# JelleAalbers/blueice

Hardware: AMD Instinct MI355X
Metric: likelihood evals/sec (and GB/s vs HBM peak), 4-src 5^3-anchor 100^3-bin model (higher is better)
Workload: dtype f64; 1 GPU; C2: 4 sources, 3 shape params (5^3 anchors), 100^3 bins; step = one batched call (one kernel launch) of 8 independent dense evaluations, each against its own dataset, in grid cells that share no anchor (no byte re-used), tensor replicated per GPU; device=gfx950:sramecc+:xnack-, gather=none (one process), backend_requested=rccl, backend_explicit=False, gather_kind=none (one process)

## Files before the change

blueice_amd/_capi.py:

```python
import ctypes as C
import os

import numpy as np

from .exceptions import DeviceError

_HERE = os.path.dirname(os.path.abspath(__file__))
LIB_PATH = os.environ.get('BLUEICE_AMD_LIB') or os.path.join(_HERE, 'lib', 'libblueice_hip.so')

ST_OUT_OF_BOUNDS, ST_UNPHYSICAL, ST_BB_ROOT1, ST_BB_NEG, ST_BAD_DATASET, ST_INTERNAL = 1, 2, 4, 8, 16, 32
ERR_INVALID, ERR_HIP, ERR_STATE, ERR_NOMEM = -1, -2, -3, -4

_p = C.c_void_p
_i32, _i64, _f64 = C.c_int32, C.c_int64, C.c_double
_pd = C.POINTER(C.c_double)

SIGNATURES = {
    'bi_create': (C.c_int, [C.c_int, C.POINTER(_p)]),
    'bi_destroy': (None, [_p]),
    'bi_last_error': (C.c_char_p, [_p]),
    'bi_version': (C.c_char_p, []),
    'bi_device_info': (C.c_int, [_p, C.c_char_p, C.c_char_p, C.c_int, C.POINTER(C.c_int), C.POINTER(_i64)]),
    'bi_upload_model': (C.c_int, [_p, C.c_int, _p, _p, C.c_int, _i64, _p, _p, _p, C.c_int]),
    'bi_model_begin': (C.c_int, [_p, C.c_int, _p, _p, C.c_int, _i64, C.c_int]),
# ... 4 lines not shown
    'bi_set_allow_negative': (C.c_int, [_p, _p]),
    'bi_upload_counts': (C.c_int, [_p, _i64, _p]),
    'bi_set_analysis_space': (C.c_int, [_p, C.c_int, _p, _p]),
    'bi_upload_events': (C.c_int, [_p, _i64, _p]),
    'bi_histogram_events': (C.c_int, [_p, C.c_int, _p, _p, _i64, _p, _p]),
    'bi_score_events': (C.c_int, [_p, _p, C.c_int, C.c_int, _p, _p, _i64, _p, C.c_double]),
    'bi_set_unbinned': (C.c_int, [_p, _f64]),
    'bi_simulate_events': (C.c_int, [_p, _p, _p, _p, C.c_int, C.c_int, _p, _p, C.c_uint64, C.c_double, _p]),
    'bi_score_event_sets': (C.c_int, [_p, _p, C.c_int, C.c_int, _p, _p, _i64, _p, _p, C.c_double]),
    'bi_simulate_event_toys': (C.c_int, [_p, _p, _p, _p, C.c_int, C.c_int, _p, _p, _i64, C.c_uint64, C.c_double, _p]),
    'bi_set_event_sets': (C.c_int, [_p, _i64, _p]),
    'bi_event_set_offsets': (C.c_int, [_p, _p]),
    'bi_event_set_counts': (C.c_int, [_p, _p]),
    'bi_event_set_count': (_i64, [_p]),
    'bi_download_event_set': (C.c_int, [_p, _i64, _p]),
    'bi_download_events': (C.c_int, [_p, _p, _p]),
    'bi_simulated_event_count': (_i64, [_p]),
    'bi_generate_toys': (C.c_int, [_p, _p, _p, _i64, C.c_uint64]),
    'bi_generate_toys_points': (C.c_int, [_p, _i64, _p, _p, _p, C.c_uint64, _p]),
    'bi_download_counts': (C.c_int, [_p, _i64, _p]),
    'bi_eval': (C.c_int, [_p, _i64, _p, _p, _p, _p, _p]),
    'bi_eval_grad': (C.c_int, [_p, _i64, _p, _p, _p, _p, _p, _p]),
    'bi_eval_hess': (C.c_int, [_p, _i64, _p, _p, _p, _p, _p, _p, _p]),
    'bi_eval_gof': (C.c_int, [_p, _i64, _p, _p, _p, _p, _p, _p]),
    'bi_expected_counts': (C.c_int, [_p, _i64, _p, _p, C.c_int, _p]),
    'bi_set_coarse_binning': (C.c_int, [_p, C.c_int, _p, _p, _p, C.POINTER(_i64)]),
    'bi_expected_coarse': (C.c_int, [_p, _i64, _p, _p, C.c_int, _p, _p]),
    'bi_expected_coarse_jacobian': (C.c_int, [_p, _i64, _p, _p, _p, _p, _p]),
    'bi_coarse_counts': (C.c_int, [_p, _i64, _p, _p]),
    'bi_set_real_counts': (C.c_int, [_p, _i64, _p]),
    'bi_set_asimov_counts': (C.c_int, [_p, _i64, _p, _p]),
    'bi_real_count_sets': (_i64, [_p]),
    'bi_download_real_counts': (C.c_int, [_p, _i64, _p]),
    'bi_eval_real': (C.c_int, [_p, _i64, _p, _p, _p, _p, _p, _p]),
    'bi_eval_fisher': (C.c_int, [_p, _i64, _p, _p, _p, _p, _p, _p]),
    'bi_fisher_variant': (C.c_int, [C.c_int, C.POINTER(C.c_int), C.POINTER(C.c_int)]),
    'bi_minimize_batched': (C.c_int, [_p, _p, _i64, C.c_int, _p, _p, _p, _p, _p, C.c_double, C.c_int, _p, _p, _p, _p]),
    'bi_fit_batched': (C.c_int, [_p, _i64, C.c_int, _p, _p, _p, _p, _p, _p, _p, _p, _p, _p, _p, C.c_double, C.c_int, _p, _p, _p, _p]),
    'bi_fit_batched_gauss': (C.c_int, [_p, _i64, C.c_int, _p, _p, _p, _p, _p, _p, _p, _p, _p, _p, _p, C.c_double, C.c_int, _p, _p, _p,
                                       _p, _p, _p, _p]),
    'bi_fit_batched_real': (C.c_int, [_p, _i64, C.c_int, _p, _p, _p, _p, _p, _p, _p, _p, _p, _p, _p, C.c_double, C.c_int, _p, _p, _p,
                                      _p, _p, _p, _p]),
    'bi_factored_begin': (C.c_int, [_p, C.c_int, _p, _p, C.c_int, _i64, _p, _p]),
    'bi_factored_set_anchor': (C.c_int, [_p, C.c_int, _i64, _p, C.c_double]),
    'bi_factored_end': (C.c_int, [_p]),
    'bi_factored_set_counts': (C.c_int, [_p, _i64, _p]),
    'bi_eval_factored': (C.c_int, [_p, _i64, _p, _p, _p, _p, _p, _p]),
    'bi_eval_sourcewise_hess': (C.c_int, [_p, _i64, _p, _p, _p, _p, _p, _p, _p]),
    'bi_eval_sourcewise_fisher': (C.c_int, [_p, _i64, _p, _p, _p, _p, _p, _p]),
    'bi_fit_batched_factored': (C.c_int, [_p, _i64, C.c_int, _p, _p, _p, _p, _p, _p, _p, _p, _p, _p, _p, C.c_double, C.c_int, _p, _p, _p,
                                          _p, _p, _p, _p]),
    'bi_sample_stretch': (C.c_int, [_p, _i64, C.c_int, C.c_int, _p, _p, _p, _p, _p, _p, _p, _p, _p, _i64, C.c_double, C.c_uint64, _i64,
                                    _p, _p, _p, _p]),
    'bi_sample_stretch_gauss': (C.c_int, [_p, _i64, C.c_int, C.c_int, _p, _p, _p, _p, _p, _p, _p, _p, _p, _i64, C.c_double, C.c_uint64, _i64,
                                          _p, _p, _p, _p, _p, _p, _p]),
    'bi_grid_reduce': (C.c_int, [_p, _i64, _p, C.c_int, C.c_int, _p, _p, _p, _p, _p, _p, _p, _p, _p, _i64, _p, _p, _p, _p]),
    'bi_eval_datasets': (C.c_int, [_p, _p, _p, _i64, _i64, _p, _p]),
    'bi_eval_datasets_points': (C.c_int, [_p, _i64, _p, _p, _i64, _i64, _p, _p]),
    'bi_eval_datasets_points_device': (C.c_int, [_p, _i64, _p, _p, _i64, _i64, _p, _p]),
    'bi_interpolate': (C.c_int, [_p, C.c_int, _p, _p]),
    'bi_eval_full': (C.c_int, [_p, _p, _p, _i64, _p, _p, _p, _p]),
    'bi_plan_points': (C.c_int, [_p, _i64, _p, _p, _p, C.POINTER(_p)]),
    'bi_run_plan': (C.c_int, [_p, _p, _p]),
    'bi_plan_points_share': (C.c_int, [_p, _i64, _p, _p, _p, C.c_int, C.c_int, C.POINTER(_p)]),
    'bi_plan_points_resident': (C.c_int, [_p, _i64, _p, _p, _p, C.c_int, C.c_int, C.POINTER(_p)]),
    'bi_plan_share_info': (C.c_int, [_p, C.POINTER(_i64), C.POINTER(_i64), C.POINTER(_i64)]),
    'bi_plan_unsort': (C.c_int, [_p, _p, _p, _i64, _p]),
    'bi_plan_read': (C.c_int, [_p, _p, _p, _p]),
    'bi_plan_status': (C.c_int, [_p, _p, C.POINTER(_i32)]),
    'bi_plan_bytes': (_i64, [_p]),
    'bi_plan_launches': (_i64, [_p]),
    'bi_plan_destroy': (None, [_p, _p]),
    'bi_sync': (C.c_int, [_p]),
    'bi_stream': (_p, [_p]),
    'bi_eval_begin': (C.c_int, [_p, _p, _p, _i64]),
    'bi_eval_end': (C.c_int, [_p, _p, _p]),
    'bi_eval_datasets_device': (C.c_int, [_p, _p, _p, _i64, _i64, _p, _p]),
    'bi_counts_to_dense': (C.c_int, [_p]),
    'bi_device_alloc': (C.c_int, [_p, _i64, C.POINTER(_p)]),
    'bi_device_free': (C.c_int, [_p, _p]),
    'bi_memcpy_to_host': (C.c_int, [_p, _p, _p, _i64]),
    'bi_memcpy_to_device': (C.c_int, [_p, _p, _p, _i64]),
    'bi_selftest_log': (C.c_int, [_p, _i64, _p, _p]),
    'bi_selftest_sort': (C.c_int, [_p, C.c_int, _i64, _p, _p, C.c_int, C.c_int, _p, _p]),
    'bi_selftest_scan': (C.c_int, [_p, C.c_int, _i64, _p, _i64, _p]),
    'bi_selftest_grid_reduce': (C.c_int, [_p, _i64, _i64, _i64, _p, _p, _p, _p, _p]),
    'bi_measure_read_bandwidth': (C.c_int, [_p, C.c_int, C.c_int, C.c_int, _p]),
    'bi_measure_stream_bandwidth': (C.c_int, [_p, C.c_int, C.c_int, C.c_int, C.c_int, C.c_int, _p]),
    'bi_measure_copy_bandwidth': (C.c_int, [_p, _i64, C.c_int, _p]),
    'bi_profile_enable': (C.c_int, [_p, C.c_int]),
    'bi_profile_read': (C.c_int, [_p, C.POINTER(_i64), C.POINTER(_f64)]),
    'bi_set_param': (C.c_int, [_p, C.c_char_p, _i64]),
    'bi_get_param': (_i64, [_p, C.c_char_p]),
    'bi_list_params': (C.c_int, [C.c_char_p, C.c_int]),
}

OBJECTIVE_FN = C.CFUNCTYPE(C.c_int, _p, _i64, C.c_int, _pd, C.POINTER(_i64), _pd, _pd)

_lib = None


def load():
    global _lib
    if _lib is not None:
        return _lib
    if not os.path.exists(LIB_PATH):
        raise DeviceError("%s is missing: build it first (python -m blueice_amd.build). "
                          "blueice_amd has no CPU fallback." % LIB_PATH)
    try:
        lib = C.CDLL(LIB_PATH)
    except OSError as e:
        raise DeviceError("cannot load %s: %s" % (LIB_PATH, e))
    for name, (res, args) in SIGNATURES.items():
        try:
            fn = getattr(lib, name)
        except AttributeError:
            raise DeviceError("%s does not export %s (stale build?)" % (LIB_PATH, name))
        fn.restype = res
        fn.argtypes = args
    version = (lib.bi_version() or b'').decode()
    if not version.startswith('blueice_hip') or '(gfx950)' not in version or 'not the product' in version:
        raise DeviceError("%s is not a gfx950 build of libblueice_hip (bi_version: %r)" % (LIB_PATH, version))
    _lib = lib
    return lib


def ptr(a):
    if a is None:
        return None
    return a.ctypes.data_as(C.c_void_p)


def as_f64(a, shape=None):
    a = np.ascontiguousarray(a, dtype=np.float64)
    if shape is not None and tuple(a.shape) != tuple(shape):
        raise ValueError("expected array of shape %s, got %s" % (tuple(shape), a.shape))
    return a
```

blueice_amd/csrc/bi_context.h:

```cpp
#pragma once

struct bi_ctx;

constexpr int kThreads = 256;
constexpr int kBinsPerThread = 2;
constexpr int kTile = kThreads * kBinsPerThread;
constexpr int kMaxDim = 8;
constexpr int kMaxG = 16;
constexpr int kFacMaxDim = 32;
constexpr int kFacMaxSources = 8;
constexpr int kFacMaxOwn = 3;

inline thread_local std::string g_create_error;

struct DevBuf {
    void* p = nullptr;
    size_t bytes = 0;
    struct bi_ctx* owner = nullptr;
    bool view = false;
};

struct bi_plan {
    int64_t P = 0;
    struct Class {
// ... 2 lines not shown
        int nbx = 0;
        DevBuf rowoff, coef, aux, item_cnt, item_tiles, perm, slot_lg, partial, pflags;
        DevBuf rowoff_full;
    };
    std::vector<Class> classes;
    DevBuf bad_idx;
    int64_t n_bad = 0;
    DevBuf nan_idx;
    int64_t n_nan = 0;
    DevBuf out, status;
    std::vector<int32_t> h_status;
    int64_t epoch = 0;
    DevBuf slab;
    bool host_results = false;
    bool use_scan = false;
    int64_t n_groups = 0;
    int scan_cb = 4;
    DevBuf grp_first, grp_items;
    std::vector<int64_t> h_grp_first;
    std::vector<int32_t> h_grp_items;
    int bb_kgt = 0;
    bool valid = false;
    int valid_nslots = 0;
    DevBuf bad;
    bool shared = false;
    int share_world = 1;
    int64_t share_lo = 0, share_hi = 0, n_valid = 0;
    DevBuf sorted_idx;
    DevBuf keep_z, keep_rs;
    int64_t max_group_items = 0;
    int max_item_tiles = 0;
    bool device_planned = false;
    bool no_reuse = false;
    bool sparse = false;
    bool narrow = false;
    bool sorted = false;
    bool by_count = false;
    int64_t bytes = 0;
    int64_t launches = 0;
};

struct bi_ctx {
    int device = 0;
    hipStream_t stream = nullptr;
    hipDeviceProp_t prop{};
    std::string err;

    bool model_ready = false, model_open = false;
    int d = 0, S = 0;
    int64_t B = 0, Bp = 0, A = 0;
    std::vector<int> n_anchor;
    std::vector<std::vector<double>> grid;
    std::vector<int64_t> astride;
    std::vector<int> eff_axes;
    int bb_source = -1;
    std::vector<int32_t> allow_neg;
    DevBuf ps, nm, nm_tot;
    std::vector<double> h_mus;
    std::vector<double> h_nm_tot;
    std::vector<char> anchor_set;

    int space_k = 0;
    std::vector<int32_t> space_n_edges;
    DevBuf space_edges;

    bool unbinned = false;
    double outlier = 0.0;
    bool ps_finite = true;
    bool data_ready = false;
    bool dense_counts = false;
    int64_t T = 0;
    int64_t n_sets = 1;
    std::vector<int64_t> set_first, set_n;
    int64_t n_set_launches = 0;
    DevBuf counts, lgsum;
    std::vector<double> h_lgsum;
    DevBuf cnt8, cnt8_bad;
    std::vector<uint32_t> h_cnt8_bad;
    bool cnt8_valid = false;
    int cnt8_all = -1;
    int64_t narrow_counts = 1;
    int64_t last_streamed_bytes = 0;
    int64_t n_narrow_launches = 0;
    int64_t last_morph_nbx = 0, last_morph_items = 0, last_morph_fused = 0;

    DevBuf real_counts;
    int64_t real_T = 0;

    struct Factored {
        bool ready = false, open = false;
        int d = 0, S = 0;
        int64_t B = 0, Bp = 0;
        std::vector<std::vector<double>> grid;
        std::vector<int> n_own;
        std::vector<int> own;
        std::vector<int64_t> row_first;
        std::vector<int64_t> own_stride;
        std::vector<double> h_mus;
        std::vector<char> row_set;
        DevBuf ps;
        int64_t T = 0;
        DevBuf counts;
        std::vector<double> h_lgsum;
        int n_rows_point = 0;
        int max_own = 0;
    } fac;

    struct Coarse {
        bool set = false;
        int64_t C = 0, CR = 0, Cx = 0;
        int64_t L = 0, NR = 0;
        int64_t x_lo = 0, Lx = 0;
        int64_t max_rows = 0;
        int64_t max_width = 0;
        DevBuf row_off, row_list;
        DevBuf xb;
        DevBuf row_map, x_map;
    } coarse;

    std::vector<double> h_rowsum;
    std::vector<double> h_rowmin;
    bool ps_nonneg = false;

    bool csr_ready = false, compact_ready = false;
    bool compact_sorted = false;
    DevBuf nz_idx, nz_n, nz_off, ps_c, cnt_c;
    DevBuf tm_entries, tm_off;
    int64_t nz_tile_epoch = -1;
    bool tm_ok = false;
    DevBuf tmm_entries, tmm_off;
    int64_t tmm_epoch = -1;
    bool tmm_ok = false;
    int tmm_width = 4;
    int64_t toy_points_pp = 0;
    int64_t toy_points_lanes = 0;
    int64_t toy_points_overlap = 0;
    hipStream_t stream2 = nullptr;
    hipEvent_t tp_ev[7] = {nullptr, nullptr, nullptr, nullptr, nullptr, nullptr, nullptr};
    int64_t n_toy_points_passes = 0;
    int64_t dot_tiled = 1;
    int64_t score_sorted = 1;
    DevBuf ev_perm;
    bool ev_sorted = false;
    int64_t toy_fast_call = 7;
    DevBuf toy_blocks_done;
    bool toy_blocks_done_zeroed = false;
    unsigned long long toy_seq = 0;
    int64_t n_toy_polled = 0;
    int64_t dot_entry16 = 1;
    int tm_width = 4;
    int64_t dot_blocks_per_cu = 0;
    int64_t dot_lanes = 0;
    int64_t toy_events = 1;
    int64_t last_toy_method = 0;
    std::vector<int64_t> h_nz_off;
    std::vector<int64_t> h_c_off, h_cnt_off;
    std::vector<int64_t> h_c_np;
    std::vector<double> h_Tz;

    DevBuf slot_dev, slot_partial, slot_pflags, slot_counter;
    DevBuf mail, mail_flags;
    void* pack_host = nullptr;
    void* bounce_host = nullptr;
    size_t pack_host_bytes = 0;
    DevBuf pack_dev;
    void* plan_host = nullptr;
// ... 242 lines not shown
```

blueice_amd/csrc/bi_dev_common.h:

```cpp
#pragma once


constexpr long long kMailTicksPerMs = 100000;

struct LaunchArgs {
    const double* ps;
    const double* nm;
    const double* counts;
    const int64_t* rowoff;
    const double* coef;
    const double* aux;
    const int64_t* item_cnt;
    const int32_t* item_tiles;
    double* partial;
    unsigned* pflags;
    int64_t B, Bp;
    double outlier;
    int n0, n1, n2;
    int n_tiles;
    int chunks;
    int n_keep;
    double* fin_mail;
    unsigned* fin_flags;
    const int64_t* fin_perm;
    const double* fin_slot_lg;
    double* fin_out;
    int32_t* fin_status;
    int nan_S;
    long long mail_timeout = 2000 * kMailTicksPerMs;
    int skip_post = -1, late_post = -1;
    const uint8_t* cnt8 = nullptr;
};

constexpr int kMaxSingleStreams = 128;

struct SingleDesc {
    int64_t rowoff[kMaxSingleStreams];
    double coef[kMaxSingleStreams];
    double aux[2];
    double slot_lg;
    unsigned* flags;
    double* out;
    int32_t* status;
    unsigned long long* done;
    unsigned long long seq;
};

typedef double bi_double4 __attribute__((ext_vector_type(4)));

struct ScanArgs {
    const double* ps;
    const double* counts;
    const int64_t* rowoff;
    const double* coef;
    const int64_t* item_cnt;
    const int32_t* item_tiles;
    const int64_t* grp_first;
    const int32_t* grp_items;
    double* partial;
    int NS;
    int nslots;
    int n_groups;
    int xcd_mode;
    int share_slow;
};

struct ValidArgs {
    const double* ps;
    const int64_t* rowoff;
    const double* coef;
    const int64_t* grp_first;
    const int32_t* grp_items;
    unsigned* bad;
    int NS;
    int nslots;
    int n_strips;
};

struct BbScanArgs {
    const double* ps;
    const double* nm;
    const double* counts;
    const int64_t* rowoff;
    const double* coef;
    const double* aux;
    const int64_t* item_cnt;
    const int64_t* grp_first;
    const int32_t* grp_items;
    double* partial;
    unsigned* pflags;
    int64_t B;
    int n0, nc;
    int n_tiles;
};

struct GradMfmaArgs {
    const double* ps;
    const double* counts;
    const int64_t* rowoff;
    const double* coef;
    const int64_t* item_cnt;
    const int32_t* item_tiles;
    const int64_t* grp_first;
    const int32_t* grp_items;
    double* part_ll;
    double* part_g;
    int NS, n_slices;
};

struct HessArgs {
    const double* ps;
    const double* counts;
    const int64_t* rowoff;
    const double* coef;
    const int64_t* item_cnt;
// ... 228 lines not shown
    return v;
}

#define BI_SWAP_MUL(SWAP, a, b, out)                                                                               \
    do {                                                                                                           \
        const unsigned long long ua = __double_as_longlong(a), ub = __double_as_longlong(b);                       \
        const auto lo = SWAP((unsigned)ua, (unsigned)ub, false, false);                                            \
        const auto hi = SWAP((unsigned)(ua >> 32), (unsigned)(ub >> 32), false, false);                            \
        out = __longlong_as_double(((unsigned long long)hi[0] << 32) | lo[0]) *                                    \
              __longlong_as_double(((unsigned long long)hi[1] << 32) | lo[1]);                                     \
    } while (0)

__device__ __forceinline__ double lane_value(double v, int src_lane) {
    const unsigned long long u = __double_as_longlong(v);
    return __longlong_as_double(((unsigned long long)(unsigned)__builtin_amdgcn_readlane((int)(u >> 32), src_lane) << 32) |
                                (unsigned)__builtin_amdgcn_readlane((int)u, src_lane));
}

__device__ __forceinline__ unsigned wave_or(unsigned v) {
#pragma unroll
    for (int off = 32; off > 0; off >>= 1) v |= __shfl_down(v, off, 64);
    return v;
}

__shared__ double4 s_log_table[128];

__device__ __forceinline__ void log_table_load() {
    if (threadIdx.x < 128) s_log_table[threadIdx.x] = kLogTable[threadIdx.x];
    __syncthreads();
}

__device__ __forceinline__ bool pos_normal(double x) { return __builtin_amdgcn_class(x, 0x100); }
constexpr double kProdFloor = 0x1p-127;

__device__ __forceinline__ double log_core(double x, int k_adjust) {
    const unsigned long long ix = __double_as_longlong(x);
    const int hi = (int)(ix >> 32);
    const int t = hi - 0x3FE60000;
    const int k0 = t >> 20;
    const int k = k0 + k_adjust;
    int zhi;
    asm("v_mad_i32_i24 %0, %1, %2, %3" : "=v"(zhi) : "v"(k0), "s"(-(1 << 20)), "v"(hi));
    const double z = __longlong_as_double(((unsigned long long)(unsigned)zhi << 32) | (ix & 0xFFFFFFFFull));
    const double4 e = s_log_table[(t >> 13) & 127];
    const double kd = (double)k;
    const double r = fma(z, e.x, -1.0);
    const double w = fma(kd, kLn2Hi, e.y);
    const double tail = fma(kd, kLn2Lo, e.z);
    double p = fma(r, -1.0 / 8.0, e.w);
    p = fma(r, p, -1.0 / 6.0);
    p = fma(r, p, 1.0 / 5.0);
    p = fma(r, p, -1.0 / 4.0);
    p = fma(r, p, 1.0 / 3.0);
    p = fma(r, p, -0.5);
    const double q = fma(r * r, p, tail);
    const double h = w + r;
    const double err = (w - h) + r;
    return h + (err + q);
}

__device__ __forceinline__ double bin_log_fast(double x) { return log_core(x, 0); }

__device__ __forceinline__ double bin_log(double x) {
    const bool tiny = x < 2.2250738585072014e-308;
    double y = log_core(tiny ? x * 18014398509481984.0 : x, tiny ? -54 : 0);
    if (x == 0.0) y = -__builtin_inf();
    if (!(x >= 0.0)) y = __builtin_nan("");
    if (x == __builtin_inf()) y = x;
    return y;
}

template <bool NT>
__device__ __forceinline__ double2 stream_load(const double* p) {
    if constexpr (NT) {
        double2 v;
        v.x = __builtin_nontemporal_load(p);
        v.y = __builtin_nontemporal_load(p + 1);
        return v;
    } else {
        return *reinterpret_cast<const double2*>(p);
    }
}

__device__ __forceinline__ double poisson_term(double n, double mu) {
    double t;
    if (n > 0.0) {
        t = n * bin_log(mu) - mu;
    } else {
        t = -mu;
    }
    if (!(mu >= 0.0) || n != n) t = __builtin_nan("");
    else if (n < 0.0 || n != floor(n)) t = -__builtin_inf();
    return t;
}

__device__ __forceinline__ bool needs_checked_term(double n, double mu) { return n > 0.0 && !pos_normal(mu); }

__device__ __forceinline__ double poisson_term_fast(double n, double mu) {
    const double lg = bin_log_fast(mu);
    double t = (n > 0.0) ? n * lg - mu : -mu;
    if (!(mu >= 0.0) || n != n) t = __builtin_nan("");
    else if (n < 0.0 || n != floor(n)) t = -__builtin_inf();
    return t;
}

__device__ __forceinline__ double poisson_term_nolog(double n, double mu) {
    double t = -mu;
    if (!(mu >= 0.0) || n != n) t = __builtin_nan("");
    else if (n < 0.0 || n != floor(n)) t = -__builtin_inf();
    return t;
}

__device__ __forceinline__ void bb_roots(double a, double p, double U, double d, double& r1, double& r2) {
#pragma clang fp contract(off)
    double U2 = U * U, p2 = p * p, a2 = a * a, d2 = d * d;
    double disc = U2 * p2 + 2 * U2 * p + U2 + 2 * U * a * p2 + 2 * U * a * p - 2 * U * d * p2 - 2 * U * d * p +
                  a2 * p2 + 2 * a * d * p2 + d2 * p2;
    double lead = -U * p - U + a * p + d * p;
    double den = 2 * p * (p + 1);
    double sq = sqrt(disc);
    r1 = (lead - sq) / den;
    r2 = (lead + sq) / den;
}

constexpr unsigned long long kMailEmpty = 0x7FF4B10E1CE00001ull;

__device__ __forceinline__ void mail_post(double* slot, double v) {
    if (v != v) v = __builtin_nan("");
    __hip_atomic_store(slot, v, __ATOMIC_RELAXED, __HIP_MEMORY_SCOPE_SYSTEM);
}

__device__ __forceinline__ double mail_take(double* slot, long long deadline, bool* late) {
    unsigned long long bits;
    for (;;) {
        bits = __hip_atomic_load(reinterpret_cast<unsigned long long*>(slot), __ATOMIC_RELAXED, __HIP_MEMORY_SCOPE_SYSTEM);
        if (bits != kMailEmpty) break;
        if ((long long)wall_clock64() > deadline) { *late = true; return __builtin_nan(""); }
        __builtin_amdgcn_s_sleep(4);
    }
    __hip_atomic_store(reinterpret_cast<unsigned long long*>(slot), kMailEmpty, __ATOMIC_RELAXED, __HIP_MEMORY_SCOPE_SYSTEM);
    return __longlong_as_double(bits);
}

__device__ __forceinline__ double mail_take4(double* mail, int q0, int stride, int total, double s, long long deadline, bool* late) {
    unsigned long long bits[4];
#pragma unroll
    for (int u = 0; u < 4; ++u) {
        const int q = q0 + u * stride;
        bits[u] = q < total ? __hip_atomic_load(reinterpret_cast<unsigned long long*>(mail + q), __ATOMIC_RELAXED, __HIP_MEMORY_SCOPE_SYSTEM)
                            : 0ull;
    }
#pragma unroll
    for (int u = 0; u < 4; ++u) {
        const int q = q0 + u * stride;
        if (q >= total) break;
        if (bits[u] == kMailEmpty) {
            s += mail_take(mail + q, deadline, late);
        } else {
            __hip_atomic_store(reinterpret_cast<unsigned long long*>(mail + q), kMailEmpty, __ATOMIC_RELAXED, __HIP_MEMORY_SCOPE_SYSTEM);
            s += __longlong_as_double(bits[u]);
        }
    }
    return s;
}

__device__ __forceinline__ void flags_post(unsigned* word, unsigned f) {
// ... 35 lines not shown
```

blueice_amd/csrc/bi_events.h:

```cpp
#pragma once

namespace {


struct AxisWords {
    const char* with;
    const char* few;
    const char* values;
};
constexpr AxisWords kSpaceWords{"edges", "axis %d needs at least two edges", "bin edges"};
constexpr AxisWords kHistWords{"edges, and a counts buffer", "axis %d needs at least two edges", "bin edges"};
constexpr AxisWords kGridWords{"grid values", "axis %d needs at least two grid values", "grid values"};
constexpr AxisWords kSimWords{"bin edges", "axis %d has too few bin edges", "bin edges"};

struct AxisWalk {
    int k = 0;
    int flat = 0;
    int64_t bins = 1;
    int n[kMaxDim] = {}, off[kMaxDim] = {};
    int64_t stride[kMaxDim] = {};
    void put(int* n_out, int* off_out, int64_t* stride_out = nullptr) const {
        for (int i = 0; i < k; ++i) {
            n_out[i] = n[i];
            off_out[i] = off[i];
// ... 35 lines not shown
    return BI_OK;
}


int score_events_impl(bi_ctx* tp, bi_ctx* c, int method, int k, const int32_t* n_grid, const double* grid, int64_t N,
                      const double* coords, const double* coords_dev, double outlier_likelihood,
                      const std::vector<int64_t>* pad_cols = nullptr) {
    if (!c) return BI_ERR_INVALID;
    if (!tp || tp == c) return fail(c, BI_ERR_INVALID, "need a templates context different from the target");
    if (c->pending || tp->pending) return fail(c, BI_ERR_STATE, "a bi_eval_begin is outstanding: call bi_eval_end first");
    if (!tp->model_ready) return fail(c, BI_ERR_STATE, "the templates context holds no model");
    if (tp->device != c->device) return fail(c, BI_ERR_INVALID, "templates and target live on different devices");
    if (tp->bb_source >= 0) return fail(c, BI_ERR_INVALID, "Beeston-Barlow applies to binned likelihoods only");
    if (method != 0 && method != 1) return fail(c, BI_ERR_INVALID, "method must be 0 (piecewise) or 1 (linear)");
    AxisWalk ax;
    int rc = walk_axes(c, k, n_grid, grid, 2, method == 1, kGridWords, ax);
    if (rc) return rc;
    if (N < 0 || (N > 0 && !coords && !coords_dev)) return fail(c, BI_ERR_INVALID, "bad N / coords");
    if (ax.bins != tp->B) return fail(c, BI_ERR_INVALID, "the grid describes %lld bins, the templates have %lld", (long long)ax.bins, (long long)tp->B);
    ScoreArgs a{};
    a.k = k;
    a.method = method;
    a.clip = coords_dev ? 1 : 0;
    ax.put(a.n_grid, a.grid_off, a.stride);
    std::vector<int32_t> na(tp->n_anchor.begin(), tp->n_anchor.end());
    std::vector<double> az;
    for (int i = 0; i < tp->d; ++i) az.insert(az.end(), tp->grid[(size_t)i].begin(), tp->grid[(size_t)i].end());
    if ((rc = bi_model_begin(c, tp->d, na.data(), az.data(), tp->S, N, -1))) return rc;
    if (N > 0) {
        ScratchBuf d_ev, d_grid, d_base, d_t, d_keys, d_iota, d_tmp, d_pad;
        const bool sorted = !pad_cols && c->score_sorted && N >= 4096 && N < ((int64_t)1 << 31);
        if (pad_cols && !pad_cols->empty() && (rc = dev_upload(c, d_pad, *pad_cols))) return rc;
        size_t sort_bytes = 0;
        if (sorted) (void)prim_sort_pairs(nullptr, sort_bytes, (const int64_t*)nullptr, (int64_t*)nullptr, (const int32_t*)nullptr,
                                                    (int32_t*)nullptr, (size_t)N, 0u, 64u, c->stream);
        if ((!coords_dev && (rc = dev_alloc(c, d_ev, (size_t)N * k * sizeof(double)))) || (rc = dev_alloc(c, d_grid, (size_t)ax.flat * sizeof(double))) ||
            (rc = dev_alloc(c, d_base, (size_t)N * sizeof(int64_t))) || (method == 1 && (rc = dev_alloc(c, d_t, (size_t)N * k * sizeof(double)))) ||
            (sorted && ((rc = dev_alloc(c, d_keys, (size_t)N * sizeof(int64_t))) || (rc = dev_alloc(c, d_iota, (size_t)N * sizeof(int32_t))) ||
                        (rc = dev_alloc(c, d_tmp, std::max<size_t>(sort_bytes, 256))) || (rc = dev_alloc(c, c->ev_perm, (size_t)N * sizeof(int32_t))))))
            return rc;
        hipError_t e = coords_dev ? hipSuccess : hipMemcpyAsync(d_ev.p, coords, (size_t)N * k * sizeof(double), hipMemcpyHostToDevice, c->stream);
        if (e == hipSuccess) e = hipMemcpyAsync(d_grid.p, grid, (size_t)ax.flat * sizeof(double), hipMemcpyHostToDevice, c->stream);
        if (e == hipSuccess) e = hipStreamSynchronize(tp->stream);
        if (e == hipSuccess) {
            const int n_rows = (int)(tp->A * tp->S);
            hipLaunchKernelGGL(k_score_locate, dim3((unsigned)((N + kThreads - 1) / kThreads)), dim3(kThreads), 0, c->stream,
                               coords_dev ? coords_dev : (const double*)d_ev.p, N, a, (const double*)d_grid.p, (int64_t*)d_base.p, (double*)d_t.p);
            const int64_t* base_used = (const int64_t*)d_base.p;
            if (sorted) {
                hipLaunchKernelGGL(k_iota32, dim3((unsigned)((N + 255) / 256)), dim3(256), 0, c->stream, (int32_t*)d_iota.p, N);
                size_t tb = d_tmp.bytes;
                unsigned bits = 1;
                while (bits < 63 && ((int64_t)1 << bits) < tp->B) ++bits;
                e = prim_sort_pairs(d_tmp.p, tb, (const int64_t*)d_base.p, (int64_t*)d_keys.p, (const int32_t*)d_iota.p,
                                              (int32_t*)c->ev_perm.p, (size_t)N, 0u, bits, c->stream);
                base_used = (const int64_t*)d_keys.p;
            }
            const int per_block = kThreads * score_events_per_thread(method == 0 ? 0 : k);
            const unsigned bx = (unsigned)((N + per_block - 1) / per_block);
#define BI_ROWS(K)                                                                                                 \
    hipLaunchKernelGGL((k_score_rows<K>), dim3(bx, (unsigned)std::min(n_rows, 65535)), dim3(kThreads), 0, c->stream, \
                       base_used, (const double*)d_t.p, N, a, (const double*)tp->ps.p, tp->Bp, n_rows, (double*)c->ps.p, c->Bp,        \
                       sorted ? (const int32_t*)c->ev_perm.p : (const int32_t*)nullptr)
            if (e == hipSuccess) switch (method == 0 ? 0 : k) {
                case 0: BI_ROWS(0); break; case 1: BI_ROWS(1); break; case 2: BI_ROWS(2); break; case 3: BI_ROWS(3); break;
                case 4: BI_ROWS(4); break; case 5: BI_ROWS(5); break; case 6: BI_ROWS(6); break; case 7: BI_ROWS(7); break;
                default: BI_ROWS(8); break;
            }
#undef BI_ROWS
            if (e == hipSuccess && pad_cols && !pad_cols->empty()) {
                const int64_t n_fill = (int64_t)n_rows * (int64_t)pad_cols->size();
                hipLaunchKernelGGL(k_fill_columns, dim3((unsigned)((n_fill + 255) / 256)), dim3(256), 0, c->stream, (double*)c->ps.p, c->Bp,
                                   (int64_t)n_rows, (const int64_t*)d_pad.p, (int64_t)pad_cols->size(), 1.0);
            }
            if (e == hipSuccess) e = hipGetLastError();
        }
        if (e == hipSuccess) e = hipStreamSynchronize(c->stream);
        else (void)hipStreamSynchronize(c->stream);
        c->ev_sorted = e == hipSuccess && sorted;
        if (e != hipSuccess) return fail(c, BI_ERR_HIP, "bi_score_events: %s", hipGetErrorString(e));
    }
    c->h_mus = tp->h_mus;
    std::fill(c->anchor_set.begin(), c->anchor_set.end(), 1);
    if ((rc = bi_model_end(c))) return rc;
    c->allow_neg = tp->allow_neg;
    return bi_set_unbinned(c, outlier_likelihood);
}


struct SimSetup {
    SimArgs a{};
    PointGeom g;
    std::vector<double> r, h_edges;
    std::vector<int64_t> rowoff;
    ScratchBuf row, w, edges, rates, dens, cdf, tmp;
};

int sim_setup(bi_ctx* tp, bi_ctx* c, const double* z, const double* rate_scale, int method, int k, const int32_t* n_edges,
              const double* edges, size_t scan_items, const char* who, SimSetup& s) {
    if (!c) return BI_ERR_INVALID;
    if (!tp || tp == c) return fail(c, BI_ERR_INVALID, "need a templates context different from the target");
    if (c->pending || tp->pending) return fail(c, BI_ERR_STATE, "a bi_eval_begin is outstanding: call bi_eval_end first");
    if (!tp->model_ready) return fail(c, BI_ERR_STATE, "the templates context holds no model");
    if (tp->device != c->device) return fail(c, BI_ERR_INVALID, "templates and target live on different devices");
    if (method != 0 && method != 1) return fail(c, BI_ERR_INVALID, "method must be 0 (piecewise) or 1 (linear)");
    AxisWalk ax;
    int rc = walk_axes(c, k, n_edges, edges, method == 1 ? 3 : 2, false, kSimWords, ax);
    if (rc) return rc;
    if (tp->d > 0 && !z) return fail(c, BI_ERR_INVALID, "z is NULL");
    if (ax.bins != tp->B) return fail(c, BI_ERR_INVALID, "the edges describe %lld bins, the templates have %lld", (long long)ax.bins, (long long)tp->B);
    s.a.k = k; s.a.S = tp->S;
    ax.put(s.a.n_edges, s.a.edge_off, s.a.stride);
    HIP_TRY(c, hipSetDevice(c->device));
    PointGeom& g = s.g;
    std::vector<double>& r = s.r;
    if ((rc = rates_at(c, tp, z, rate_scale, "simulation", "event simulation", g, r))) return rc;
    const int S = tp->S;
    for (int q = 0; q < S; ++q)
        if (r[(size_t)q] >= kSimMaxRate)
            return fail(c, BI_ERR_INVALID, "event simulation draws at most 2^30 expected events per source: source %d has %g", q, r[(size_t)q]);
    const int nc = (int)g.w.size();
    const int64_t B = tp->B;
    s.rowoff.assign((size_t)S * nc, 0);
    for (int q = 0; q < S; ++q)
        for (int corner = 0; corner < nc; ++corner)
            s.rowoff[(size_t)q * nc + corner] = ((g.cell_anchor + corner_offset(tp, corner)) * S + q) * tp->Bp;
    size_t scan_bytes = 0, scan2 = 0;
    (void)prim_inclusive_scan_sum(nullptr, scan_bytes, (const double*)nullptr, (double*)nullptr, (size_t)B, c->stream);
    if (scan_items) (void)prim_exclusive_scan_sum(nullptr, scan2, (const int64_t*)nullptr, (int64_t*)nullptr, (int64_t)0, scan_items, c->stream);
    s.h_edges.assign(edges, edges + ax.flat);
    if ((rc = dev_upload(c, s.row, s.rowoff)) || (rc = dev_upload(c, s.w, g.w)) || (rc = dev_upload(c, s.edges, s.h_edges)) ||
        (rc = dev_upload(c, s.rates, r)) || (rc = dev_alloc(c, s.dens, (size_t)S * B * sizeof(double))) ||
        (rc = dev_alloc(c, s.cdf, (size_t)S * B * sizeof(double))) ||
        (rc = dev_alloc(c, s.tmp, std::max<size_t>(std::max(scan_bytes, scan2), 256)))) return rc;
    hipError_t e = hipStreamSynchronize(tp->stream);
    if (e == hipSuccess) {
        hipLaunchKernelGGL(k_morph_store, dim3((unsigned)((B + kThreads - 1) / kThreads), (unsigned)S), dim3(kThreads), 0, c->stream,
                           (const double*)tp->ps.p, (const int64_t*)s.row.p, (const double*)s.w.p, nc, B, (double*)s.dens.p);
        hipLaunchKernelGGL(k_sim_pmf, dim3((unsigned)((B + kThreads - 1) / kThreads), (unsigned)S), dim3(kThreads), 0, c->stream,
                           (const double*)s.dens.p, s.a, (const double*)s.edges.p, B, (double*)s.dens.p);
        e = hipGetLastError();
    }
    for (int q = 0; e == hipSuccess && q < S; ++q) {
        size_t tb = s.tmp.bytes;
        e = prim_inclusive_scan_sum(s.tmp.p, tb, (const double*)s.dens.p + (size_t)q * B, (double*)s.cdf.p + (size_t)q * B, (size_t)B, c->stream);
    }
    if (e != hipSuccess) return fail(c, BI_ERR_HIP, "%s: %s", who, hipGetErrorString(e));
    return BI_OK;
}

void lookup_grid(int method, int k, const int32_t* n_edges, const double* edges, std::vector<int32_t>& n_grid, std::vector<double>& grid) {
    n_grid.assign((size_t)k, 0);
    grid.clear();
    int eo = 0;
    for (int i = 0; i < k; ++i) {
        if (method == 0) {
            n_grid[(size_t)i] = n_edges[i];
            grid.insert(grid.end(), edges + eo, edges + eo + n_edges[i]);
        } else {
            n_grid[(size_t)i] = n_edges[i] - 1;
            for (int j = 0; j + 1 < n_edges[i]; ++j) grid.push_back(0.5 * (edges[eo + j] + edges[eo + j + 1]));
        }
        eo += n_edges[i];
    }
}


// ... 249 lines not shown
```

blueice_amd/csrc/bi_k_misc.h:

```cpp
#pragma once

#include "bi_philox.h"

namespace {

__global__ void k_selftest_log(const double* __restrict__ x, int64_t n, double* __restrict__ out) {
    log_table_load();
    const int64_t i = (int64_t)blockIdx.x * blockDim.x + threadIdx.x;
    if (i < n) out[i] = bin_log(x[i]);
}

template <bool NT>
__global__ __launch_bounds__(kThreads) void k_read_sum(const double* __restrict__ p, int64_t n2, double* __restrict__ sink) {
    double s = 0.0;
    const int64_t stride = (int64_t)gridDim.x * kThreads;
    int64_t i = (int64_t)blockIdx.x * kThreads + threadIdx.x;
    for (; i + 7 * stride < n2; i += 8 * stride) {
        double2 v[8];
#pragma unroll
        for (int u = 0; u < 8; ++u) v[u] = stream_load<NT>(p + 2 * (i + u * stride));
#pragma unroll
        for (int u = 0; u < 8; ++u) s += v[u].x + v[u].y;
    }
    for (; i < n2; i += stride) s += p[2 * i] + p[2 * i + 1];
// ... 83 lines not shown
    f = wave_or(f);
    if (lanes == 64) {
        if ((threadIdx.x & 63) == 0 && p >= 0) {
            out[p] = s - lg;
            if (status) status[p] |= (int32_t)f;
        }
        return;
    }
    if ((threadIdx.x & 63) == 0) { sh[threadIdx.x >> 6] = s; shf[threadIdx.x >> 6] = f; }
    __syncthreads();
    if (threadIdx.x == 0 && p >= 0) {
        double t = sh[0];
        unsigned ff = shf[0];
        for (int w = 1; w < kThreads / 64; ++w) { t += sh[w]; ff |= shf[w]; }
        out[p] = t - lg;
        if (status) status[p] |= (int32_t)ff;
    }
}

__global__ __launch_bounds__(kThreads) void k_status_or(const int32_t* __restrict__ status, int64_t n, int32_t* __restrict__ out) {
    unsigned f = 0u;
    for (int64_t i = (int64_t)blockIdx.x * kThreads + threadIdx.x; i < n; i += (int64_t)gridDim.x * kThreads) f |= (unsigned)status[i];
    f = wave_or(f);
    if ((threadIdx.x & 63) == 0 && f) atomicOr((unsigned*)out, f);
}

__global__ __launch_bounds__(kThreads) void k_status_clear(int32_t* __restrict__ status, int64_t n, int32_t mask) {
    for (int64_t i = (int64_t)blockIdx.x * kThreads + threadIdx.x; i < n; i += (int64_t)gridDim.x * kThreads)
        if (status[i] & mask) status[i] &= ~mask;
}

__global__ void k_fill_value(double* __restrict__ out, int64_t n, double v) {
    const int64_t i = (int64_t)blockIdx.x * blockDim.x + threadIdx.x;
    if (i < n) out[i] = v;
}

__global__ void k_fill_const(double* __restrict__ out, const int64_t* __restrict__ idx, int64_t n, double v) {
    const int64_t i = (int64_t)blockIdx.x * blockDim.x + threadIdx.x;
    if (i < n) out[idx[i]] = v;
}

__global__ __launch_bounds__(kThreads) void k_counts_lgamma(const double* __restrict__ counts, int64_t B, int64_t Bp,
                                                            double* __restrict__ partial, int nblk) {
    const int t = blockIdx.y;
    const double* __restrict__ c = counts + (int64_t)t * Bp;
    double s = 0.0;
    for (int64_t b = (int64_t)blockIdx.x * kThreads + threadIdx.x; b < B; b += (int64_t)nblk * kThreads) {
        const double n = c[b];
        if (n > 1.0 && n == floor(n)) s += lgamma(n + 1.0);
    }
    __shared__ double sh[kThreads / 64];
    s = wave_sum(s);
    if ((threadIdx.x & 63) == 0) sh[threadIdx.x >> 6] = s;
    __syncthreads();
    if (threadIdx.x == 0) {
        double r = sh[0];
        for (int w = 1; w < kThreads / 64; ++w) r += sh[w];
        partial[(int64_t)t * nblk + blockIdx.x] = r;
    }
}

constexpr int kNarrowPerThread = 8;
__global__ __launch_bounds__(kThreads) void k_counts_narrow(const double* __restrict__ counts, int64_t B, int64_t Bp,
                                                            uint8_t* __restrict__ narrow, unsigned* __restrict__ bad) {
    const int t = blockIdx.y;
    const int64_t b0 = ((int64_t)blockIdx.x * kThreads + threadIdx.x) * kNarrowPerThread;
    bool lossy = false;
    if (b0 < Bp) {
        const double* __restrict__ src = counts + (int64_t)t * Bp + b0;
        unsigned long long packed = 0ull;
#pragma unroll
        for (int j = 0; j < kNarrowPerThread; ++j) {
            const double v = b0 + j < B ? src[j] : 0.0;
            const bool in_range = v >= 0.0 && v <= 255.0;
            const unsigned q = in_range ? (unsigned)(int)v : 0u;
            lossy |= __double_as_longlong((double)q) != __double_as_longlong(v);
            packed |= (unsigned long long)q << (8 * j);
        }
        *reinterpret_cast<unsigned long long*>(narrow + (int64_t)t * Bp + b0) = packed;
    }
    if (__ballot(lossy) != 0ull && (threadIdx.x & 63) == 0) atomicOr(bad + t, 1u);
}

__global__ void k_rows_sum(const double* __restrict__ partial, int nblk, double* __restrict__ out, int64_t T) {
    const int64_t t = (int64_t)blockIdx.x * blockDim.x + threadIdx.x;
    if (t >= T) return;
    double s = 0.0;
    for (int b = 0; b < nblk; ++b) s += partial[t * nblk + b];
    out[t] = s;
}

__global__ __launch_bounds__(kThreads) void k_morph_store(const double* __restrict__ src,
                                                          const int64_t* __restrict__ rowoff,
                                                          const double* __restrict__ w,
                                                          int nc, int64_t B, double* __restrict__ out,
                                                          const int32_t* __restrict__ place = nullptr) {
    const int r = blockIdx.y;
    const int64_t b = (int64_t)blockIdx.x * kThreads + threadIdx.x;
    if (b >= B) return;
    double v = 0.0;
    for (int c = 0; c < nc; ++c) {
        const double term = __dmul_rn(src[rowoff[(int64_t)r * nc + c] + b], w[c]);
        v = __dadd_rn(v, term);
    }
    out[(int64_t)r * B + (place ? (int64_t)place[b] : b)] = v;
}

__global__ __launch_bounds__(kThreads) void k_row_total(const double* __restrict__ rows, int64_t B, int64_t Bp,
                                                        double* __restrict__ out) {
    const double* __restrict__ r = rows + (int64_t)blockIdx.x * Bp;
    double s = 0.0;
    for (int64_t b = threadIdx.x; b < B; b += kThreads) s += r[b];
    __shared__ double sh[kThreads / 64];
    s = wave_sum(s);
    if ((threadIdx.x & 63) == 0) sh[threadIdx.x >> 6] = s;
    __syncthreads();
    if (threadIdx.x == 0) {
        double t = sh[0];
        for (int w = 1; w < kThreads / 64; ++w) t += sh[w];
        out[blockIdx.x] = t;
    }
}

constexpr int kSumChunk = 8192;

__global__ __launch_bounds__(kThreads) void k_bb_chunk_sums(const double* __restrict__ nm, const int64_t* __restrict__ rowoff_all,
                                                            const double* __restrict__ w_all, int nc, int64_t B,
                                                            double* __restrict__ chunk_sum_all, double* __restrict__ tail_all) {
    __shared__ double a[kSumChunk / 2];
    __shared__ double r[256];
    __shared__ double leaf[64];
    const int64_t q = blockIdx.x;
    const int64_t* __restrict__ rowoff = rowoff_all + q * nc;
    const double* __restrict__ w = w_all + q * nc;
    double* __restrict__ chunk_sum = chunk_sum_all + q * (B / kSumChunk);
    double* __restrict__ tail = tail_all + q * (B % kSumChunk);
    const int64_t b0 = (int64_t)blockIdx.y * kSumChunk;
    const int n = (int)(B - b0 < (int64_t)kSumChunk ? B - b0 : (int64_t)kSumChunk);
    if (n < kSumChunk) {
        for (int i = threadIdx.x; i < n; i += kThreads) {
            double v = 0.0;
            for (int c = 0; c < nc; ++c) v = __dadd_rn(v, __dmul_rn(nm[rowoff[c] + b0 + i], w[c]));
            tail[i] = v;
        }
        return;
    }
    for (int half = 0; half < 2; ++half) {
        __syncthreads();
        for (int i = threadIdx.x; i < kSumChunk / 2; i += kThreads) {
            double v = 0.0;
            for (int c = 0; c < nc; ++c) v = __dadd_rn(v, __dmul_rn(nm[rowoff[c] + b0 + half * (kSumChunk / 2) + i], w[c]));
            a[i] = v;
        }
        __syncthreads();
        {
            const int blk = threadIdx.x >> 3, j = threadIdx.x & 7;
            double t = a[blk * 128 + j];
#pragma unroll
            for (int i = 1; i < 16; ++i) t = __dadd_rn(t, a[blk * 128 + 8 * i + j]);
            r[threadIdx.x] = t;
        }
        __syncthreads();
        if (threadIdx.x < 32) {
            const double* q = r + threadIdx.x * 8;
            leaf[half * 32 + threadIdx.x] = __dadd_rn(__dadd_rn(__dadd_rn(q[0], q[1]), __dadd_rn(q[2], q[3])),
                                                      __dadd_rn(__dadd_rn(q[4], q[5]), __dadd_rn(q[6], q[7])));
// ... 748 lines not shown
```

blueice_amd/csrc/bi_k_morph.h:

```cpp
#pragma once

#ifndef BI_CNT8_NT
#define BI_CNT8_NT 0
#endif

namespace {


template <int G, bool BB, bool NT, int MODE, bool CNT8 = false>
__device__ __forceinline__ void morph_tiles(const LaunchArgs& a, const int64_t* __restrict__ rowoff,
                                            const double* __restrict__ coef, const double* __restrict__ aux_base,
                                            const double* __restrict__ cnt, const uint8_t* __restrict__ cnt8, int n_tiles, int tile0,
                                            int tile_step, double (&sum)[G], unsigned (&flg)[G]) {
    double4 tab = {0.0, 0.0, 0.0, 0.0};
    if (threadIdx.x < 128) tab = kLogTable[threadIdx.x];
    bool tab_pending = true;
    const int chunks = (a.chunks > 1 && n_tiles >= 64 * a.chunks) ? a.chunks : 1;
    const int per_chunk = (n_tiles + chunks - 1) / chunks;
    for (int lt = tile0; lt < per_chunk * chunks; lt += tile_step) {
        const int tile = chunks > 1 ? (lt % chunks) * per_chunk + lt / chunks : lt;
        if (tile >= n_tiles) continue;
        const int64_t bin0 = (int64_t)tile * kTile + threadIdx.x * kBinsPerThread;
        double acc[G][2];
#pragma unroll
        for (int g = 0; g < G; ++g) { acc[g][0] = 0.0; acc[g][1] = 0.0; }
        double2 nv;
        if constexpr (MODE == 2 || MODE == 3) { nv.x = nv.y = 0.0; }
        else if constexpr (CNT8) {
#if BI_CNT8_NT
            const unsigned pair = __builtin_nontemporal_load(reinterpret_cast<const uint16_t*>(cnt8 + bin0));
#else
            const unsigned pair = *reinterpret_cast<const uint16_t*>(cnt8 + bin0);
#endif
            nv.x = (double)(pair & 0xffu);
            nv.y = (double)(pair >> 8);
        } else { nv = *reinterpret_cast<const double2*>(cnt + bin0); }

        int k0 = 0;
        if constexpr (NT && G == 1 && MODE != 2 && MODE != 3) {
            k0 = a.n_keep;
#pragma unroll 8
            for (int k = 0; k < k0; ++k) {
                const double2 v = stream_load<false>(a.ps + rowoff[k] + bin0);
                const double c = coef[k];
                acc[0][0] = fma(c, v.x, acc[0][0]);
                acc[0][1] = fma(c, v.y, acc[0][1]);
            }
        }
        if constexpr (MODE == 2 || MODE == 3) if (a.nan_S > 0) {
            const int S = a.nan_S, nc = a.n0 / S;
            for (int s = 0; s < S; ++s) {
                double part[G][2];
#pragma unroll
                for (int g = 0; g < G; ++g) { part[g][0] = 0.0; part[g][1] = 0.0; }
                for (int c = 0; c < nc; ++c) {
                    const int k = c * S + s;
                    const double2 v = stream_load<NT>(a.ps + rowoff[k] + bin0);
#pragma unroll
                    for (int g = 0; g < G; ++g) {
                        const double cf = coef[k * G + g];
                        part[g][0] = fma(cf, v.x, part[g][0]);
                        part[g][1] = fma(cf, v.y, part[g][1]);
                    }
                }
                if constexpr (MODE == 3) {
#pragma unroll
                    for (int j = 0; j < 2; ++j)
                        if (part[0][j] == part[0][j]) {
#pragma unroll
                            for (int g = 0; g < G; ++g) acc[g][j] += part[g][j];
                        }
                } else {
#pragma unroll
                    for (int g = 0; g < G; ++g) {
                        if (part[g][0] == part[g][0]) acc[g][0] += part[g][0];
                        if (part[g][1] == part[g][1]) acc[g][1] += part[g][1];
                    }
                }
            }
            k0 = a.n0;
        }
#pragma unroll 8
        for (int k = k0; k < a.n0; ++k) {
            const double2 v = stream_load<NT>(a.ps + rowoff[k] + bin0);
#pragma unroll
            for (int g = 0; g < G; ++g) {
                const double c = coef[k * G + g];
                acc[g][0] = fma(c, v.x, acc[g][0]);
                acc[g][1] = fma(c, v.y, acc[g][1]);
            }
        }
        if (tab_pending) {
            if (threadIdx.x < 128) s_log_table[threadIdx.x] = tab;
            __syncthreads();
            tab_pending = false;
        }

        if constexpr (MODE == 2) {
            bool checked = false;
#pragma unroll
            for (int g = 0; g < G; ++g) {
#pragma unroll
                for (int j = 0; j < 2; ++j) {
                    if (a.outlier != 0.0 && !(acc[g][j] > 0.0)) acc[g][j] = a.outlier;
                    checked |= bin0 + j < a.B && !pos_normal(acc[g][j]);
                }
            }
            const bool fast = __ballot(checked) == 0ull;
#pragma unroll
            for (int g = 0; g < G; ++g) {
#pragma unroll
                for (int j = 0; j < 2; ++j) {
                    const double lg = fast ? bin_log_fast(acc[g][j]) : bin_log(acc[g][j]);
                    if (bin0 + j < a.B) sum[g] += lg;
                }
            }
        } else if constexpr (MODE == 3) {
#pragma unroll
            for (int j = 0; j < 2; ++j) {
                double lam = acc[0][j];
                const bool clamped = a.outlier != 0.0 && !(lam > 0.0);
                if (clamped) lam = a.outlier;
                const double lg = bin_log(lam);
                if (bin0 + j < a.B) {
                    sum[0] += lg;
                    const double inv = clamped ? 0.0 : 1.0 / lam;
#pragma unroll
                    for (int g = 1; g < G; ++g) sum[g] += acc[g][j] * inv;
                }
            }
        } else if constexpr (MODE == 1) {
            sum[0] += poisson_term(nv.x, acc[0][0]) + poisson_term(nv.y, acc[0][1]);
            const double f0 = (nv.x != 0.0 ? nv.x / acc[0][0] : 0.0) - 1.0;
            const double f1 = (nv.y != 0.0 ? nv.y / acc[0][1] : 0.0) - 1.0;
#pragma unroll
            for (int g = 1; g < G; ++g) sum[g] += f0 * acc[g][0] + f1 * acc[g][1];
        } else if constexpr (!BB) {
#pragma unroll
            for (int j = 0; j < 2; ++j) {
                const double n = j ? nv.y : nv.x;
                bool checked = false;
#pragma unroll
                for (int g = 0; g < G; ++g) checked |= needs_checked_term(n, acc[g][j]);
                if (__ballot(n > 0.0) == 0ull) {
#pragma unroll
                    for (int g = 0; g < G; ++g) sum[g] += poisson_term_nolog(n, acc[g][j]);
                } else if (__ballot(checked) == 0ull) {
#pragma unroll
                    for (int g = 0; g < G; ++g) sum[g] += poisson_term_fast(n, acc[g][j]);
                } else {
#pragma unroll
                    for (int g = 0; g < G; ++g) sum[g] += poisson_term(n, acc[g][j]);
                }
            }
        } else {
            double pi[G][2], ai[G][2];
#pragma unroll
            for (int g = 0; g < G; ++g) { pi[g][0] = pi[g][1] = ai[g][0] = ai[g][1] = 0.0; }
#pragma unroll 8
            for (int k = 0; k < a.n1; ++k) {
                const double2 v = stream_load<NT>(a.ps + rowoff[a.n0 + k] + bin0);
#pragma unroll
                for (int g = 0; g < G; ++g) {
                    const double c = coef[(a.n0 + k) * G + g];
                    pi[g][0] = __dadd_rn(pi[g][0], __dmul_rn(v.x, c));
                    pi[g][1] = __dadd_rn(pi[g][1], __dmul_rn(v.y, c));
                }
            }
#pragma unroll 8
            for (int k = 0; k < a.n2; ++k) {
                const double2 v = stream_load<NT>(a.nm + rowoff[a.n0 + a.n1 + k] + bin0);
#pragma unroll
                for (int g = 0; g < G; ++g) {
                    const double c = coef[(a.n0 + a.n1 + k) * G + g];
                    ai[g][0] = __dadd_rn(ai[g][0], __dmul_rn(v.x, c));
                    ai[g][1] = __dadd_rn(ai[g][1], __dmul_rn(v.y, c));
                }
            }
            const double* __restrict__ aux = aux_base;
#pragma unroll
            for (int g = 0; g < G; ++g) {
                const double p_cal = aux[g * 2 + 0];
                const double Ntot = aux[g * 2 + 1];
#pragma unroll
                for (int j = 0; j < 2; ++j) {
                    if (bin0 + j < a.B) {
                        const double n = j ? nv.y : nv.x;
                        const double U = acc[g][j];
                        const double ab = ai[g][j];
                        const double w = pi[g][j] / ab * Ntot;
                        double r1, r2;
                        bb_roots(ab, w * p_cal, U, n, r1, r2);
                        if (!(r1 <= 0.0)) flg[g] |= BI_ST_BB_ROOT1;
                        const double A = (U == 0.0) ? (n + ab) / (1.0 + p_cal) : r2;
                        if (!(0.0 <= A)) flg[g] |= BI_ST_BB_NEG;
                        const double mu = U + (A * w) * p_cal;
                        sum[g] += poisson_term(n, mu);
                    }
                }
            }
        }
    }

}

template <int G, bool BB, bool NT, int MODE = 0, bool CNT8 = false>
__global__ __launch_bounds__(kThreads) void k_morph_reduce(LaunchArgs a) {
    const int item = blockIdx.y;
    const int NS = a.n0 + a.n1 + a.n2;
    const int64_t* __restrict__ rowoff = a.rowoff + (int64_t)item * NS;
    const double* __restrict__ coef = a.coef + (int64_t)item * NS * G;
    const int64_t cnt_off = a.item_cnt[item];
    const double* __restrict__ cnt = a.counts + cnt_off;
    const uint8_t* __restrict__ cnt8 = CNT8 ? a.cnt8 + cnt_off : nullptr;
    const int n_tiles = a.item_tiles ? a.item_tiles[item] : a.n_tiles;

    double sum[G];
    unsigned flg[G];
#pragma unroll
    for (int g = 0; g < G; ++g) { sum[g] = 0.0; flg[g] = 0u; }

    morph_tiles<G, BB, NT, MODE, CNT8>(a, rowoff, coef, a.aux + (int64_t)item * G * 2, cnt, cnt8, n_tiles, (int)blockIdx.x, (int)gridDim.x, sum, flg);

    __shared__ double s_sum[kThreads / 64][G];
    __shared__ unsigned s_flg[kThreads / 64][G];
    const int lane = threadIdx.x & 63, wave = threadIdx.x >> 6;
#pragma unroll
    for (int g = 0; g < G; ++g) {
        const double s = wave_sum(sum[g]);
        const unsigned f = BB ? wave_or(flg[g]) : 0u;
        if (lane == 0) { s_sum[wave][g] = s; s_flg[wave][g] = f; }
    }
    __syncthreads();
    const bool fuse = a.fin_mail != nullptr;
    const int nbx = gridDim.x;
    if (threadIdx.x < G) {
        const int g = threadIdx.x;
        double s = s_sum[0][g];
        unsigned f = s_flg[0][g];
#pragma unroll
        for (int w = 1; w < kThreads / 64; ++w) { s += s_sum[w][g]; f |= s_flg[w][g]; }
        const int64_t o = ((int64_t)item * nbx + blockIdx.x) * G + g;
        if (fuse) {
            if (BB) flags_post(a.fin_flags + (int64_t)item * G + g, f);
            mail_post_checked(a, a.fin_mail + o, s);
        } else {
            a.partial[o] = s;
            a.pflags[o] = f;
        }
    }
    if (!fuse || (int)blockIdx.x != nbx - 1) return;

    const long long deadline = (long long)wall_clock64() + a.mail_timeout;
    double* __restrict__ mail = a.fin_mail + (int64_t)item * nbx * G;
    bool late = false;
    if (nbx <= 64) {
        for (int g = wave; g < G; g += kThreads / 64) {
            double s = lane < nbx ? mail_take(mail + (int64_t)lane * G + g, deadline, &late) : 0.0;
            s = wave_sum(s);
            const bool any_late = __ballot(late) != 0ull;
            const int64_t p = a.fin_perm[(int64_t)item * G + g];
            if (lane == 0) {
                const unsigned f = (BB ? flags_take(a.fin_flags + (int64_t)item * G + g) : 0u) | (any_late ? (unsigned)BI_ST_INTERNAL : 0u);
                if (p >= 0) {
                    a.fin_out[p] = s - a.fin_slot_lg[(int64_t)item * G + g];
                    if (a.fin_status) a.fin_status[p] |= (int32_t)f;
                }
            }
        }
        return;
    }
    {
        const int total = nbx * G;
        double s = 0.0;
        for (int q0 = threadIdx.x; q0 < total; q0 += 4 * kThreads) s = mail_take4(mail, q0, kThreads, total, s, deadline, &late);
        __shared__ double s_part[kThreads];
        __shared__ unsigned s_late[kThreads / 64];
        const unsigned lt = __ballot(late) != 0ull ? 1u : 0u;
        if constexpr (G == 1) s = wave_sum(s);
        __syncthreads();
        s_part[threadIdx.x] = s;
        if (lane == 0) s_late[wave] = lt;
        __syncthreads();
        if (threadIdx.x < G) {
            const int g = threadIdx.x;
            double t = 0.0;
            if constexpr (G == 1) {
                t = s_part[0];
#pragma unroll
                for (int w = 1; w < kThreads / 64; ++w) t += s_part[w * 64];
            } else {
                for (int j = 0; j < kThreads / G; ++j) t += s_part[g + G * j];
            }
            unsigned any_late = 0u;
#pragma unroll
            for (int w = 0; w < kThreads / 64; ++w) any_late |= s_late[w];
            const int64_t p = a.fin_perm[(int64_t)item * G + g];
            const unsigned f = (BB ? flags_take(a.fin_flags + (int64_t)item * G + g) : 0u) | (any_late ? (unsigned)BI_ST_INTERNAL : 0u);
            if (p >= 0) {
                a.fin_out[p] = t - a.fin_slot_lg[(int64_t)item * G + g];
                if (a.fin_status) a.fin_status[p] |= (int32_t)f;
            }
        }
    }
}

template <bool BB, bool NT, int MODE, bool FUSE, bool CNT8 = false>
__global__ __launch_bounds__(kThreads) void k_morph_single(LaunchArgs a, SingleDesc d) {
    double sum[1] = {0.0};
    unsigned flg[1] = {0u};
    morph_tiles<1, BB, NT, MODE, CNT8>(a, d.rowoff, d.coef, d.aux, a.counts, a.cnt8, a.n_tiles, (int)blockIdx.x, (int)gridDim.x, sum, flg);

    __shared__ double s_sum[kThreads / 64];
    __shared__ unsigned s_flg[kThreads / 64];
    const int lane = threadIdx.x & 63, wave = threadIdx.x >> 6;
    {
        const double s = wave_sum(sum[0]);
        const unsigned f = BB ? wave_or(flg[0]) : 0u;
        if (lane == 0) { s_sum[wave] = s; s_flg[wave] = f; }
    }
    __syncthreads();
    if (threadIdx.x == 0) {
        double s = s_sum[0];
        unsigned f = s_flg[0];
#pragma unroll
        for (int w = 1; w < kThreads / 64; ++w) { s += s_sum[w]; f |= s_flg[w]; }
        if constexpr (FUSE) {
            if (BB) flags_post(d.flags, f);
            mail_post_checked(a, a.partial + blockIdx.x, s);
        } else {
            a.partial[blockIdx.x] = s;
            a.pflags[blockIdx.x] = f;
        }
    }
    if constexpr (!FUSE) return;
    if (blockIdx.x != gridDim.x - 1) return;
    const long long deadline = (long long)wall_clock64() + a.mail_timeout;
    bool late = false;
    double s = 0.0;
    for (int b = threadIdx.x; b < (int)gridDim.x; b += 4 * kThreads) s = mail_take4(a.partial, b, kThreads, (int)gridDim.x, s, deadline, &late);
    s = wave_sum(s);
    const unsigned lt = __ballot(late) != 0ull ? 1u : 0u;
    __syncthreads();
    if (lane == 0) { s_sum[wave] = s; s_flg[wave] = lt; }
    __syncthreads();
    if (threadIdx.x == 0) {
        double t = s_sum[0];
        unsigned any_late = s_flg[0];
#pragma unroll
        for (int w = 1; w < kThreads / 64; ++w) { t += s_sum[w]; any_late |= s_flg[w]; }
        const unsigned ff = (BB ? flags_take(d.flags) : 0u) | (any_late ? (unsigned)BI_ST_INTERNAL : 0u);
        *d.out = t - d.slot_lg;
        *d.status = (int32_t)ff;
        __hip_atomic_store(d.done, d.seq, __ATOMIC_RELEASE, __HIP_MEMORY_SCOPE_SYSTEM);
    }
}

}
```

blueice_amd/csrc/bi_launch.h:

```cpp
#pragma once

namespace {

constexpr int64_t kMailSlots = (int64_t)1 << 20;
constexpr int64_t kMailFlagWords = (int64_t)1 << 16;

int ensure_mail(bi_ctx* c) {
    if (c->mail.p) return BI_OK;
    void* p = nullptr;
    void* f = nullptr;
    if (hipMalloc(&p, (size_t)kMailSlots * sizeof(double)) != hipSuccess) return BI_ERR_NOMEM;
    if (hipMalloc(&f, (size_t)kMailFlagWords * sizeof(unsigned)) != hipSuccess) { (void)hipFree(p); return BI_ERR_NOMEM; }
    hipLaunchKernelGGL(k_mail_init, dim3((unsigned)((kMailSlots + 255) / 256)), dim3(256), 0, c->stream, (unsigned long long*)p, kMailSlots);
    if (hipGetLastError() != hipSuccess || hipMemsetAsync(f, 0, (size_t)kMailFlagWords * sizeof(unsigned), c->stream) != hipSuccess) {
        (void)hipFree(p);
        (void)hipFree(f);
        return BI_ERR_HIP;
    }
    c->mail.p = p; c->mail.bytes = (size_t)kMailSlots * sizeof(double); c->mail.owner = nullptr;
    c->mail_flags.p = f; c->mail_flags.bytes = (size_t)kMailFlagWords * sizeof(unsigned); c->mail_flags.owner = nullptr;
    return BI_OK;
}

void arm_mail(bi_ctx* c, LaunchArgs& a) {
    a.mail_timeout = c->mail_timeout_ms * kMailTicksPerMs;
    a.skip_post = (int)c->debug_skip_post;
    a.late_post = (int)c->debug_late_post;
    c->debug_skip_post = c->debug_late_post = -1;
}

void reset_mail(bi_ctx* c) {
    if (!c->mail.p) return;
    ++c->n_mail_resets;
    (void)hipStreamSynchronize(c->stream);
    hipLaunchKernelGGL(k_mail_init, dim3((unsigned)((kMailSlots + 255) / 256)), dim3(256), 0, c->stream, (unsigned long long*)c->mail.p, kMailSlots);
    (void)hipMemsetAsync(c->mail_flags.p, 0, (size_t)kMailFlagWords * sizeof(unsigned), c->stream);
    (void)hipStreamSynchronize(c->stream);
}

int check_ready(bi_ctx* c, bool need_data) {
    if (!c) return BI_ERR_INVALID;
    if (c->pending) return fail(c, BI_ERR_STATE, "a bi_eval_begin is outstanding on this context: call bi_eval_end first");
    if (!c->model_ready) return fail(c, BI_ERR_STATE, "no model uploaded (prepare() first)");
    if (need_data && !c->data_ready) return fail(c, BI_ERR_STATE, "no data uploaded (set_data() first)");
    return BI_OK;
}

int n_tiles_of(const bi_ctx* c) { return (int)(c->Bp / kTile); }

void build_narrow_counts(bi_ctx* c, int64_t T) {
    c->cnt8_valid = false;
    c->cnt8_all = -1;
    if (c->unbinned || T < 1 || !c->counts.p) return;
    const std::string keep = c->err;
    if (dev_alloc(c, c->cnt8, (size_t)T * c->Bp) || dev_alloc(c, c->cnt8_bad, (size_t)T * sizeof(unsigned))) {
        (void)hipGetLastError();
        c->err = keep;
        return;
    }
    if (hipMemsetAsync(c->cnt8_bad.p, 0, (size_t)T * sizeof(unsigned), c->stream) != hipSuccess) { (void)hipGetLastError(); return; }
    const unsigned nbx = (unsigned)((c->Bp + (int64_t)kThreads * kNarrowPerThread - 1) / ((int64_t)kThreads * kNarrowPerThread));
    const int64_t chunk = 32768;
    for (int64_t t0 = 0; t0 < T; t0 += chunk)
        hipLaunchKernelGGL(k_counts_narrow, dim3(nbx, (unsigned)std::min(chunk, T - t0)), dim3(kThreads), 0, c->stream,
                           (const double*)c->counts.p + t0 * c->Bp, c->B, c->Bp, (uint8_t*)c->cnt8.p + t0 * c->Bp, (unsigned*)c->cnt8_bad.p + t0);
    c->h_cnt8_bad.assign((size_t)T, 1u);
    if (hipGetLastError() != hipSuccess ||
        hipMemcpyAsync(c->h_cnt8_bad.data(), c->cnt8_bad.p, (size_t)T * sizeof(unsigned), hipMemcpyDeviceToHost, c->stream) != hipSuccess) {
        (void)hipGetLastError();
        return;
    }
    c->cnt8_valid = true;
}

bool narrow_on(const bi_ctx* c) { return c->narrow_counts && c->cnt8_valid && !c->unbinned && c->dense_counts; }
bool narrow_has(const bi_ctx* c, int64_t ds) {
    return c->cnt8_valid && ds >= 0 && ds < (int64_t)c->h_cnt8_bad.size() && c->h_cnt8_bad[(size_t)ds] == 0u;
}
bool narrow_has_all(bi_ctx* c) {
    if (!c->cnt8_valid) return false;
    if (c->cnt8_all < 0) c->cnt8_all = std::all_of(c->h_cnt8_bad.begin(), c->h_cnt8_bad.end(), [](uint32_t f) { return f == 0u; }) ? 1 : 0;
    return c->cnt8_all == 1;
}

void launch_finish(bi_ctx* c, const double* partial, const unsigned* pflags, int nbx, int G, int64_t n_slots, const int64_t* perm,
                   const double* slot_lg, double* out, int32_t* status) {
    const int lanes = nbx > 64 ? kThreads : 64;
    const int per_block = kThreads / lanes;
    hipLaunchKernelGGL(k_finish, dim3((unsigned)((n_slots + per_block - 1) / per_block)), dim3(kThreads), 0, c->stream, partial, pflags,
                       nbx, G, lanes, n_slots, perm, slot_lg, out, status);
}

}
```

blueice_amd/csrc/bi_params.h:

```cpp
#pragma once

namespace {

enum : int { kParamRead = 1, kParamWrite = 2, kParamRW = 3 };

struct ParamDef {
    const char* name;
    int access;
    int64_t (*get)(bi_ctx*);
    int (*set)(bi_ctx*, int64_t);
};

#define BI_P_GET(expr) [](bi_ctx* c) -> int64_t { return (int64_t)(expr); }
#define BI_P_SET(stmt) [](bi_ctx* c, int64_t v) -> int { stmt; return BI_OK; }
#define BI_P_RANGE(lo, hi, field, what)                                                                           \
    [](bi_ctx* c, int64_t v) -> int {                                                                             \
        if (v < (lo) || v > (hi)) return fail(c, BI_ERR_INVALID, what);                                           \
        c->field = v;                                                                                             \
        return BI_OK;                                                                                             \
    }
#define BI_P_FLAG(field) BI_P_SET(c->field = v ? 1 : 0)
#define BI_P_RO(nm, expr) {nm, kParamRead, BI_P_GET(expr), nullptr}

const ParamDef kParams[] = {
    {"sparse", kParamRW, BI_P_GET(c->sparse), BI_P_RANGE(0, 2, sparse, "sparse: 0 = off, 1 = auto, 2 = whenever exact")},
    {"max_group", kParamRW, BI_P_GET(c->max_group),
     [](bi_ctx* c, int64_t v) -> int {
         if (v < 1 || v > kMaxG || (v & (v - 1))) return fail(c, BI_ERR_INVALID, "max_group must be a power of two in [1,%d]", kMaxG);
         c->max_group = v;
         return BI_OK;
     }},
    {"bb_max_group", kParamRW, BI_P_GET(c->bb_max_group), BI_P_SET(c->bb_max_group = v >= 16 ? 16 : (v >= 8 ? 8 : (v >= 4 ? 4 : (v >= 2 ? 2 : 1))))},
    {"blocks_per_cu", kParamRW, BI_P_GET(c->blocks_per_cu), BI_P_RANGE(1, 32, blocks_per_cu, "blocks_per_cu in [1,32]")},
    {"nt_loads", kParamRW, BI_P_GET(c->nt_loads), BI_P_RANGE(0, 2, nt_loads, "nt_loads: 0 = never, 1 = always, 2 = auto")},
    {"tile_chunks", kParamRW, BI_P_GET(c->tile_chunks), BI_P_SET(c->tile_chunks = v < 1 ? 1 : v)},
    {"single_kernel", kParamRW, BI_P_GET(c->single_kernel), BI_P_FLAG(single_kernel)},
    {"fuse_max_blocks", kParamRW, BI_P_GET(c->fuse_max_blocks), BI_P_SET(c->fuse_max_blocks = v)},
    {"single_blocks_per_cu", kParamRW, BI_P_GET(c->single_blocks_per_cu),
     BI_P_RANGE(1, 32, single_blocks_per_cu, "single_blocks_per_cu in [1,32]")},
    {"fuse_finish", kParamRW, BI_P_GET(c->fuse_finish), BI_P_FLAG(fuse_finish)},
    {"keep_rows", kParamRW, BI_P_GET(c->keep_rows), BI_P_SET(c->keep_rows = v < 0 ? -1 : v)},
    {"poll_result", kParamRW, BI_P_GET(c->poll_result), BI_P_FLAG(poll_result)},
    {"xcd_affine", kParamRW, BI_P_GET(c->xcd_affine), BI_P_FLAG(xcd_affine)},
    {"device_plan_min", kParamRW, BI_P_GET(c->device_plan_min), BI_P_SET(c->device_plan_min = v)},
    {"scan_mfma", kParamRW, BI_P_GET(c->scan_mfma), BI_P_FLAG(scan_mfma)},
    {"scan_min_items", kParamRW, BI_P_GET(c->scan_min_items), BI_P_SET(c->scan_min_items = v < 1 ? 1 : v)},
    {"scan_cb", kParamRW, BI_P_GET(c->scan_cb), BI_P_SET(c->scan_cb = (v == 2 || v == 4) ? v : 0)},
    {"scan_waves_per_cu", kParamRW, BI_P_GET(c->scan_waves_per_cu), BI_P_SET(c->scan_waves_per_cu = v < 0 ? 0 : v)},
    {"host_threads", kParamRW, [](bi_ctx*) -> int64_t { return host_threads(); },
     [](bi_ctx* c, int64_t v) -> int { if (v < 0 || v > 256) return fail(c, BI_ERR_INVALID, "host_threads in [0, 256] (0 = by the process's affinity, at most 16)"); host_threads_setting().store((int)v); return BI_OK; }},
    {"toy_points_pp", kParamRW, BI_P_GET(c->toy_points_pp),
     [](bi_ctx* c, int64_t v) -> int {
         if (v != 0 && v != 1 && v != 2 && v != 4) return fail(c, BI_ERR_INVALID, "toy_points_pp: 0 = by the batch, 1 = point by point, 2 or 4 points per pass");
         c->toy_points_pp = v;
         return BI_OK;
     }},
    {"toy_points_overlap", kParamRW, BI_P_GET(c->toy_points_overlap), BI_P_FLAG(toy_points_overlap)},
    {"toy_points_lanes", kParamRW, BI_P_GET(c->toy_points_lanes),
     [](bi_ctx* c, int64_t v) -> int {
         if (v != 0 && v != 2 && v != 4 && v != 8) return fail(c, BI_ERR_INVALID, "toy_points_lanes: 0 = default, or 2 / 4 / 8");
         c->toy_points_lanes = v;
         return BI_OK;
     }},
    {"grad_mfma", kParamRW, BI_P_GET(c->grad_mfma), BI_P_FLAG(grad_mfma)},
    {"grad_mfma_min", kParamRW, BI_P_GET(c->grad_mfma_min), BI_P_RANGE(1, (int64_t)1 << 40, grad_mfma_min, "grad_mfma_min >= 1")},
    {"grad_slices", kParamRW, BI_P_GET(c->grad_slices), BI_P_RANGE(0, 4096, grad_slices, "grad_slices in [0, 4096]")},
    {"scan_xcd", kParamRW, BI_P_GET(c->scan_xcd), BI_P_RANGE(0, 2, scan_xcd, "scan_xcd: 0 launch order, 1 contiguous ranges, 2 one XCD per group")},
    {"scan_share_slow", kParamRW, BI_P_GET(c->scan_share_slow), BI_P_FLAG(scan_share_slow)},
    {"scan_chunk", kParamRW, BI_P_GET(c->scan_chunk), BI_P_FLAG(scan_chunk)},
    {"plan_tables", kParamRW, BI_P_GET(c->plan_tables), BI_P_FLAG(plan_tables)},
    {"plan_count_sort", kParamRW, BI_P_GET(c->plan_count_sort), BI_P_FLAG(plan_count_sort)},
    {"scan_bb", kParamRW, BI_P_GET(c->scan_bb), BI_P_FLAG(scan_bb)},
    {"scan_bb_min", kParamRW, BI_P_GET(c->scan_bb_min), BI_P_RANGE(1, (int64_t)1 << 40, scan_bb_min, "scan_bb_min >= 1")},
    {"scan_sparse_max_items", kParamRW, BI_P_GET(c->scan_sparse_max_items), BI_P_SET(c->scan_sparse_max_items = v < 0 ? 0 : v)},
    {"scan_split", kParamRW, BI_P_GET(c->scan_split), BI_P_FLAG(scan_split)},
    {"scan_pow", kParamRW, BI_P_GET(c->scan_pow), BI_P_SET(c->scan_pow = v ? 1 : 0; c->sorted_epoch = -1)},
    {"bb_exact", kParamRW, BI_P_GET(c->bb_exact), BI_P_RANGE(0, 2, bb_exact, "bb_exact: 0 never, 1 always, 2 auto")},
    {"toy_events", kParamRW, BI_P_GET(c->toy_events), BI_P_FLAG(toy_events)},
    {"dot_tiled", kParamRW, BI_P_GET(c->dot_tiled), BI_P_FLAG(dot_tiled)},
    {"score_sorted", kParamRW, BI_P_GET(c->score_sorted), BI_P_FLAG(score_sorted)},
    {"toy_fast_call", kParamRW, BI_P_GET(c->toy_fast_call), BI_P_RANGE(0, 7, toy_fast_call, "toy_fast_call: bits 1 | 2 | 4")},
    {"dot_entry16", kParamRW, BI_P_GET(c->dot_entry16), [](bi_ctx* c, int64_t v) -> int { c->dot_entry16 = v ? 1 : 0; c->nz_tile_epoch = -1; c->tmm_epoch = -1; return BI_OK; }},
    {"dot_blocks_per_cu", kParamRW, BI_P_GET(c->dot_blocks_per_cu), BI_P_RANGE(0, 16, dot_blocks_per_cu, "dot_blocks_per_cu in [0, 16]")},
    {"dot_lanes", kParamRW, BI_P_GET(c->dot_lanes), BI_P_SET(c->dot_lanes = (v == 16 || v == 8 || v == 4) ? v : 0)},
    {"compact_budget", kParamRW, BI_P_GET(c->compact_budget), BI_P_SET(c->compact_budget = v)},
    {"toy_offset", kParamRW, BI_P_GET(c->toy_offset), BI_P_RANGE(0, INT64_MAX, toy_offset, "toy_offset >= 0")},
    {"narrow_counts", kParamRW, BI_P_GET(c->narrow_counts), BI_P_FLAG(narrow_counts)},
    {"mail_timeout_ms", kParamRW, BI_P_GET(c->mail_timeout_ms),
     BI_P_RANGE(1, 60000, mail_timeout_ms, "mail_timeout_ms in [1, 60000]")},
    {"single_timing_reset", kParamWrite, nullptr,
     BI_P_SET(c->single_ns[0] = c->single_ns[1] = c->single_ns[2] = 0; c->single_calls = 0; (void)v)},
    {"drop_recycle_cache", kParamWrite, nullptr, BI_P_SET((void)hipSetDevice(c->device); (void)hipStreamSynchronize(c->stream); drop_recycle_cache(c); (void)v)},
    {"debug_skip_post", kParamWrite, nullptr, BI_P_SET(c->debug_skip_post = v < 0 ? -1 : v)},
    {"debug_late_post", kParamWrite, nullptr, BI_P_SET(c->debug_late_post = v < 0 ? -1 : v)},
    BI_P_RO("tile_bins", kTile),
    BI_P_RO("padded_bins", c->Bp),
    BI_P_RO("n_scan_launches", c->n_scan_launches),
    BI_P_RO("n_toy_polled", c->n_toy_polled),
    BI_P_RO("n_toy_points_passes", c->n_toy_points_passes),
    BI_P_RO("n_bb_scan_launches", c->n_bb_scan_launches),
    BI_P_RO("n_sampler_half_steps", c->n_sampler_half_steps),
    BI_P_RO("n_set_launches", c->n_set_launches),
    BI_P_RO("last_plan_refused", c->plan_refused),
    BI_P_RO("tmm_entry_bytes", c->tmm_ok ? c->tmm_width : 0),
    BI_P_RO("tm_entry_bytes", c->tm_ok ? c->tm_width : 0),
    BI_P_RO("events_sorted", c->ev_sorted ? 1 : 0),
    BI_P_RO("n_grad_mfma_launches", c->n_grad_mfma_launches),
    BI_P_RO("n_valid_launches", c->n_valid_launches),
    BI_P_RO("n_sorted_scans", c->n_sorted_scans),
    BI_P_RO("n_bb_exact", c->n_bb_exact),
    BI_P_RO("n_mail_resets", c->n_mail_resets),
    BI_P_RO("last_streamed_bytes", c->last_streamed_bytes),
    BI_P_RO("n_narrow_launches", c->n_narrow_launches),
    BI_P_RO("last_morph_nbx", c->last_morph_nbx),
    BI_P_RO("last_morph_items", c->last_morph_items),
    BI_P_RO("last_morph_fused", c->last_morph_fused),
    BI_P_RO("narrow_ready", c->cnt8_valid ? 1 : 0),
    BI_P_RO("csr_ready", (c->csr_ready && (c->sparse_at_upload != 0 || !c->dense_counts)) ? 1 : 0),
    BI_P_RO("compact_ready", (c->compact_ready && c->ps_nonneg && (c->sparse_at_upload != 0 || !c->dense_counts)) ? 1 : 0),
    BI_P_RO("split_ready", (c->compact_ready && c->dense_counts) ? 1 : 0),
    BI_P_RO("ps_nonneg", c->ps_nonneg ? 1 : 0),
    BI_P_RO("dense_counts", (c->data_ready && c->dense_counts) ? 1 : 0),
    BI_P_RO("coarse_cells", c->coarse.set ? c->coarse.C : 0),
    BI_P_RO("compact_sorted", (c->compact_ready && c->compact_sorted) ? 1 : 0),
    BI_P_RO("nnz_total", c->csr_ready ? c->h_nz_off.back() : -1),
    BI_P_RO("last_scan_nslots", c->last_scan_nslots),
    BI_P_RO("last_valid_nslots", c->last_valid_nslots),
    BI_P_RO("last_scan_resident", c->last_scan_resident),
    BI_P_RO("last_scan_groups", c->last_scan_groups),
    BI_P_RO("last_scan_max_items", c->last_scan_max_items),
    BI_P_RO("last_scan_cb", c->last_scan_cb),
    BI_P_RO("last_scan_by_count", c->last_scan_by_count),
    BI_P_RO("last_scan_prod", c->last_scan_prod),
    BI_P_RO("last_toy_method", c->last_toy_method),
    BI_P_RO("single_calls", c->single_calls),
    BI_P_RO("single_ns_host", c->single_ns[0]),
    BI_P_RO("single_ns_launch", c->single_ns[1]),
    BI_P_RO("single_ns_wait", c->single_ns[2]),
    BI_P_RO("user_allocations", (int64_t)c->user_allocs.size()),
    BI_P_RO("recycle_cache_bytes", (int64_t)c->cache_bytes),
};

#undef BI_P_GET
#undef BI_P_SET
#undef BI_P_RANGE
#undef BI_P_FLAG
#undef BI_P_RO

const ParamDef* find_param(const char* name) {
    for (const ParamDef& p : kParams)
        if (!strcmp(p.name, name)) return &p;
    return nullptr;
}

}
```

blueice_amd/csrc/bi_single.h:

```cpp
#pragma once

namespace {


int single_wait(bi_ctx* c, unsigned long long seq, double* out, int32_t* status) {
    char* res = (char*)c->slot_host;
    bool arrived = false;
    if (c->poll_result && !c->profiling) {
        const std::chrono::milliseconds limit(20);
        arrived = wait_word((const volatile unsigned long long*)(res + 16), seq, limit, limit, 1024);
    }
    if (!arrived || (seq & 255ull) == 0) HIP_TRY(c, hipStreamSynchronize(c->stream));
    if (*(const volatile unsigned long long*)(res + 16) != seq)
        return fail(c, BI_ERR_HIP, "single-point launch %llu finished without publishing its result", seq);
    *out = *(double*)res;
    if (status) *status = *(int32_t*)(res + 8);
    if (*(int32_t*)(res + 8) & BI_ST_INTERNAL) reset_mail(c);
    return BI_OK;
}

double pairwise_sum_host(const double* a, int64_t n) {
    if (n < 8) {
        double res = 0.0;
        for (int64_t i = 0; i < n; ++i) res += a[i];
// ... 140 lines not shown
    const int64_t row_stride = sparse ? c->h_c_np[(size_t)ds] : c->Bp;
    const int64_t row_base = sparse ? c->h_c_off[(size_t)ds] : 0;
    const int tiles = multi_set(c) ? (int)std::max<int64_t>(1, (c->set_n[(size_t)ds] + kTile - 1) / kTile) : (int)(row_stride / kTile);
    const int64_t slots = (int64_t)c->prop.multiProcessorCount * c->blocks_per_cu;
    const int64_t target = (int64_t)c->prop.multiProcessorCount * c->single_blocks_per_cu;
    const int64_t tiles_per_block = std::max<int64_t>(1, (tiles + target - 1) / target);
    int64_t want = (tiles + tiles_per_block - 1) / tiles_per_block;
    if (want >= 8) want = (want + 7) / 8 * 8;
    const int nbx = (int)std::min<int64_t>(std::min<int64_t>(want, tiles), slots);
    int rc;
    if (!c->slot_host) {
        HIP_TRY(c, hipHostMalloc(&c->slot_host, 4096, hipHostMallocDefault));
        c->slot_host_bytes = 4096;
    }
    const bool fuse = nbx <= c->fuse_max_blocks && nbx <= kMailSlots && !ensure_mail(c);
    if (!fuse && ((rc = dev_alloc(c, c->slot_partial, (size_t)slots * sizeof(double))) ||
                  (rc = dev_alloc(c, c->slot_pflags, (size_t)slots * sizeof(unsigned)))))
        return rc;
    SingleDesc d;
    const int64_t n_rows = c->A * S;
    int k = 0;
    double zsum = 0.0;
    for (int corner = 0; corner < nc; ++corner) {
        const int64_t a = g.cell_anchor + corner_offset(c, corner);
        for (int s = 0; s < S; ++s) {
            if (bb && s == c->bb_source) continue;
            d.rowoff[k] = row_base + (a * S + s) * row_stride;
            d.coef[k] = g.w[(size_t)corner] * rates[s];
            if (sparse) zsum += d.coef[k] * c->h_Tz[(size_t)(ds * n_rows + a * S + s)];
            ++k;
        }
    }
    d.aux[0] = d.aux[1] = 1.0;
    if (bb) {
        double Ntot = 0.0;
        for (int corner = 0; corner < nc; ++corner) {
            const int64_t a = g.cell_anchor + corner_offset(c, corner);
            d.rowoff[n0 + corner] = (a * S + c->bb_source) * c->Bp;
            d.coef[n0 + corner] = g.w[(size_t)corner];
            d.rowoff[n0 + n1 + corner] = a * c->Bp;
            d.coef[n0 + n1 + corner] = g.w[(size_t)corner];
            const double term = c->h_nm_tot[(size_t)a] * g.w[(size_t)corner];
            Ntot = Ntot + term;
        }
        if (c->bb_exact == 1 || (c->bb_exact == 2 && bb_zero_u_possible(c, g, rates))) {
            if ((rc = bb_exact_total(c, g, &Ntot))) return rc;
        }
        d.aux[0] = rates[c->bb_source] / Ntot;
        d.aux[1] = Ntot;
    }
    d.slot_lg = c->h_lgsum[(size_t)ds] + zsum;
    if (c->unbinned) {
        double rsum = 0.0;
        for (int s = 0; s < S; ++s) rsum += rates[s];
        d.slot_lg = rsum;
    }
    char* res = (char*)c->slot_host;
    *(double*)res = 0.0;
    *(int64_t*)(res + 8) = 0;
    *(unsigned long long*)(res + 16) = 0ull;
    d.flags = fuse ? (unsigned*)c->mail_flags.p : nullptr;
    d.out = (double*)res;
    d.status = (int32_t*)(res + 8);
    d.done = (unsigned long long*)(res + 16);
    d.seq = ++c->slot_seq;
    LaunchArgs a{};
    a.ps = sparse ? (const double*)c->ps_c.p : (const double*)c->ps.p;
    a.nm = (const double*)c->nm.p;
    a.counts = (sparse ? (const double*)c->cnt_c.p + c->h_cnt_off[(size_t)ds] : (const double*)c->counts.p + ds * c->Bp);
    a.partial = fuse ? (double*)c->mail.p : (double*)c->slot_partial.p;
    a.pflags = (unsigned*)c->slot_pflags.p;
    a.B = c->B; a.Bp = c->Bp; a.n0 = n0; a.n1 = n1; a.n2 = n2; a.n_tiles = tiles; a.chunks = (int)c->tile_chunks;
    if (multi_set(c)) {
        a.ps += c->set_first[(size_t)ds];
        a.B = c->set_n[(size_t)ds];
    }
    a.outlier = c->outlier;
    a.nan_S = (c->unbinned && !c->ps_finite) ? c->S : 0;
    if (fuse) arm_mail(c, a);
    if (!sparse && narrow_on(c) && narrow_has(c, ds)) {
        a.cnt8 = (const uint8_t*)c->cnt8.p + ds * c->Bp;
        ++c->n_narrow_launches;
    }
    const bool nt = !sparse && c->nt_loads != 0;
    a.n_keep = 0;
    if (nt && !bb && c->keep_rows != 0) {
        const bool same_cell = c->last_single_cell == g.cell_anchor && c->last_single_ds == ds;
        const int64_t fit = (int64_t)(0.85 * 256.0 * 1048576.0 / ((double)row_stride * sizeof(double)));
        if (same_cell) a.n_keep = (int)std::min<int64_t>(c->keep_rows > 0 ? c->keep_rows : fit, n0);
    }
    c->last_single_cell = g.cell_anchor;
    c->last_single_ds = ds;
    const dim3 grid((unsigned)nbx), block(kThreads);
    const auto t_launch = bi_clock::now();
    {
        EventScope ev(c);
        launch_morph_single(c, bb, nt, fuse, grid, a, d);
    }
    c->last_morph_nbx = nbx; c->last_morph_items = 1; c->last_morph_fused = fuse ? 1 : 0;
    if (!fuse)
        hipLaunchKernelGGL(k_finish_single, dim3(1), block, 0, c->stream, (const double*)a.partial, (const unsigned*)a.pflags,
                           nbx, d.slot_lg, d.out, d.status, d.done, d.seq);
    HIP_TRY(c, hipGetLastError());
    const auto t_wait = bi_clock::now();
    c->single_ns[0] += ns_between(t_entry, t_launch);
    c->single_ns[1] += ns_between(t_launch, t_wait);
    ++c->single_calls;
    if (!wait) {
        c->pending = 1;
        c->pending_seq = d.seq;
        return BI_OK;
    }
    rc = single_wait(c, d.seq, out, status);
    c->single_ns[2] += ns_between(t_wait, bi_clock::now());
    return rc;
}

int eval_single(bi_ctx* c, const double* z, const double* rate_scale, int64_t ds, double* out, int32_t* status, bool wait = true) {
    const auto t_entry = bi_clock::now();
    double parked_ll = 0.0;
    int32_t parked_st = 0;
    if (!wait) { out = &parked_ll; status = &parked_st; c->pending = 2; }
    struct Park {
        bi_ctx* c; const bool on; double* ll; int32_t* st;
        ~Park() { if (on && c->pending == 2) { c->pending_ll = *ll; c->pending_status = *st; } }
    } park{c, !wait, &parked_ll, &parked_st};
    const int S = c->S;
    const double ninf = -std::numeric_limits<double>::infinity();
    PointGeom g;
    double r[64];
    std::vector<double> rbig;
    double* rates = r;
    if (S > 64) { rbig.resize((size_t)S); rates = rbig.data(); }
    if (const int32_t bit = screen_point(c, z, rate_scale, ds, g, rates)) { *out = ninf; if (status) *status = bit; return BI_OK; }
    if (has_infinite_rate(rates, S) && c->bb_source < 0 && !c->unbinned && c->ps_finite && c->dense_counts)
        return inf_rate_value(c, g, rates, ds, out);

    const bool bb = c->bb_source >= 0;
    const int nc = (int)g.w.size();
    const int n0 = bb ? nc * (S - 1) : nc * S, n1 = bb ? nc : 0, n2 = bb ? nc : 0, NS = n0 + n1 + n2;
    const bool sparse = ItemRoute(c).compact;
    if (!sparse && !c->dense_counts) return fail(c, BI_ERR_STATE, "dataset counts are not resident in dense form");
    const int64_t row_stride = sparse ? c->h_c_np[(size_t)ds] : c->Bp;
    const int64_t row_base = sparse ? c->h_c_off[(size_t)ds] : 0;
    const int tiles = multi_set(c) ? (int)std::max<int64_t>(1, (c->set_n[(size_t)ds] + kTile - 1) / kTile) : (int)(row_stride / kTile);
    const int64_t slots = (int64_t)c->prop.multiProcessorCount * c->blocks_per_cu;
    const int nbx = (int)std::min<int64_t>(tiles, slots);

    if (NS <= kMaxSingleStreams && c->single_kernel) return eval_single_fused(c, g, rates, ds, sparse, out, status, wait, t_entry);

    const size_t n_words = (size_t)NS * 2 + 2 + 4 + 2;
    const size_t bytes = n_words * 8;
    int rc;
    if (c->slot_host_bytes < bytes) {
        if (c->slot_host) (void)hipHostFree(c->slot_host);
        c->slot_host = nullptr;
        HIP_TRY(c, hipHostMalloc(&c->slot_host, bytes * 2, hipHostMallocDefault));
        c->slot_host_bytes = bytes * 2;
    }
    if ((rc = dev_alloc(c, c->slot_dev, bytes)) || (rc = dev_alloc(c, c->slot_partial, (size_t)slots * sizeof(double))) ||
        (rc = dev_alloc(c, c->slot_pflags, (size_t)slots * sizeof(unsigned))))
        return rc;
    int64_t* w64 = (int64_t*)c->slot_host;
    double* wd = (double*)c->slot_host;
    int64_t* rowoff = w64;
    double* coef = wd + NS;
    double* aux = wd + 2 * NS;
    int k = 0;
    double zsum = 0.0;
    const int64_t n_rows = c->A * S;
    for (int corner = 0; corner < nc; ++corner) {
        const int64_t a = g.cell_anchor + corner_offset(c, corner);
        for (int s = 0; s < S; ++s) {
            if (bb && s == c->bb_source) continue;
            rowoff[k] = row_base + (a * S + s) * row_stride;
            coef[k] = g.w[(size_t)corner] * rates[s];
            if (sparse) zsum += coef[k] * c->h_Tz[(size_t)(ds * n_rows + a * S + s)];
            ++k;
        }
    }
    aux[0] = 1.0; aux[1] = 1.0;
    if (bb) {
        double Ntot = 0.0;
        for (int corner = 0; corner < nc; ++corner) {
            const int64_t a = g.cell_anchor + corner_offset(c, corner);
            rowoff[n0 + corner] = (a * S + c->bb_source) * c->Bp;
            coef[n0 + corner] = g.w[(size_t)corner];
            rowoff[n0 + n1 + corner] = a * c->Bp;
            coef[n0 + n1 + corner] = g.w[(size_t)corner];
            const double term = c->h_nm_tot[(size_t)a] * g.w[(size_t)corner];
            Ntot = Ntot + term;
        }
        if (c->bb_exact == 1 || (c->bb_exact == 2 && bb_zero_u_possible(c, g, rates))) {
            if ((rc = bb_exact_total(c, g, &Ntot))) return rc;
        }
        aux[0] = rates[c->bb_source] / Ntot;
        aux[1] = Ntot;
    }
    const size_t o = (size_t)2 * NS + 2;
    w64[o + 0] = sparse ? c->h_cnt_off[(size_t)ds] : ds * c->Bp;
    ((int32_t*)(w64 + o + 1))[0] = tiles;
    ((int32_t*)(w64 + o + 1))[1] = 0;
    w64[o + 2] = 0;
    wd[o + 3] = c->h_lgsum[(size_t)ds] + zsum;
    if (c->unbinned) {
        double rsum = 0.0;
        for (int s = 0; s < S; ++s) rsum += rates[s];
        wd[o + 3] = rsum;
    }
    char* res = (char*)c->slot_host + bytes;
    *(double*)res = 0.0;
    *(int64_t*)(res + 8) = 0;

    char* dev = (char*)c->slot_dev.p;
    HIP_TRY(c, hipMemcpyAsync(dev, c->slot_host, bytes, hipMemcpyHostToDevice, c->stream));
    LaunchArgs a{};
    a.ps = sparse ? (const double*)c->ps_c.p : (const double*)c->ps.p;
    a.nm = (const double*)c->nm.p;
    a.counts = sparse ? (const double*)c->cnt_c.p : (const double*)c->counts.p;
    a.rowoff = (const int64_t*)dev;
    a.coef = (const double*)(dev + (size_t)NS * 8);
    a.aux = (const double*)(dev + (size_t)NS * 16);
    a.item_cnt = (const int64_t*)(dev + (o + 0) * 8);
    a.item_tiles = (const int32_t*)(dev + (o + 1) * 8);
    a.partial = (double*)c->slot_partial.p;
    a.pflags = (unsigned*)c->slot_pflags.p;
    a.B = c->B; a.Bp = c->Bp; a.n0 = n0; a.n1 = n1; a.n2 = n2; a.n_tiles = tiles; a.chunks = (int)c->tile_chunks;
    if (multi_set(c)) {
        a.ps += c->set_first[(size_t)ds];
        a.B = c->set_n[(size_t)ds];
    }
    a.outlier = c->outlier;
    a.nan_S = (c->unbinned && !c->ps_finite) ? c->S : 0;
    if (!sparse && narrow_on(c) && narrow_has(c, ds)) {
        a.cnt8 = (const uint8_t*)c->cnt8.p;
        ++c->n_narrow_launches;
    }
    launch_morph_g(c, 1, a, dim3((unsigned)nbx, 1), bb, !sparse && c->nt_loads != 0);
    c->last_morph_nbx = nbx; c->last_morph_items = 1; c->last_morph_fused = 0;
    launch_finish(c, a.partial, a.pflags, nbx, 1, 1, (const int64_t*)(dev + (o + 2) * 8), (const double*)(dev + (o + 3) * 8),
                  (double*)res, (int32_t*)(res + 8));
    HIP_TRY(c, hipGetLastError());
    HIP_TRY(c, hipStreamSynchronize(c->stream));
    *out = *(double*)res;
    if (status) *status = *(int32_t*)(res + 8);
    return BI_OK;
}

}
```

blueice_amd/csrc/blueice_hip.hip:

```cpp

#include "bi_common.h"
#include "bi_prim.h"
#include "bi_k_misc.h"
#include "bi_geometry.h"
#include "bi_launch.h"
#include "bi_items.h"
#include "bi_sparse.h"
#include "bi_single.h"
#include "bi_planning.h"
#include "bi_planning_device.h"
#include "bi_grad_mfma.h"
#include "bi_grad.h"
#include "bi_params.h"
#include "bi_events.h"
#include "bi_toys.h"

namespace {

int finish_counts(bi_ctx* c, int64_t T) {
    int rc;
    const int nblk = (int)std::min<int64_t>(256, (c->B + kThreads - 1) / kThreads);
    if ((rc = dev_alloc(c, c->lgsum, (size_t)T * sizeof(double)))) return rc;
    const int64_t chunk = 32768;
    if ((rc = dev_alloc(c, c->scratch, (size_t)std::min(T, chunk) * nblk * sizeof(double)))) return rc;
    for (int64_t t0 = 0; t0 < T; t0 += chunk) {
        const int64_t n = std::min(chunk, T - t0);
        hipLaunchKernelGGL(k_counts_lgamma, dim3(nblk, (unsigned)n), dim3(kThreads), 0, c->stream,
                           (const double*)c->counts.p + t0 * c->Bp, c->B, c->Bp, (double*)c->scratch.p, nblk);
        hipLaunchKernelGGL(k_rows_sum, dim3((unsigned)((n + 255) / 256)), dim3(256), 0, c->stream,
                           (const double*)c->scratch.p, nblk, (double*)c->lgsum.p + t0, n);
    }
    HIP_TRY(c, hipGetLastError());
    build_narrow_counts(c, T);
    c->h_lgsum.assign((size_t)T, 0.0);
    HIP_TRY(c, hipMemcpyAsync(c->h_lgsum.data(), c->lgsum.p, (size_t)T * sizeof(double), hipMemcpyDeviceToHost, c->stream));
    HIP_TRY(c, hipStreamSynchronize(c->stream));
    c->T = T;
    c->dense_counts = true;
    if ((rc = build_sparse_forms(c))) return rc;
    c->data_ready = true;
    return BI_OK;
}

}

extern "C" {

const char* bi_version(void) { return BI_VERSION; }

const char* bi_last_error(const bi_ctx* ctx) { return ctx ? ctx->err.c_str() : g_create_error.c_str(); }

int bi_create(int device, bi_ctx** out) {
    if (!out) return fail(nullptr, BI_ERR_INVALID, "out is NULL");
    *out = nullptr;
    int n = 0;
    hipError_t e = hipGetDeviceCount(&n);
    if (e != hipSuccess || n == 0)
        return fail(nullptr, BI_ERR_HIP, "no HIP device available (%s); this library has no CPU fallback",
                    e == hipSuccess ? "device count is 0" : hipGetErrorString(e));
    if (device < 0 || device >= n) return fail(nullptr, BI_ERR_INVALID, "device %d out of range [0,%d)", device, n);
    bi_ctx* c = new bi_ctx();
    c->device = device;
    if ((e = hipSetDevice(device)) != hipSuccess || (e = hipGetDeviceProperties(&c->prop, device)) != hipSuccess ||
        (e = hipStreamCreateWithFlags(&c->stream, hipStreamNonBlocking)) != hipSuccess) {
        fail(nullptr, BI_ERR_HIP, "device init failed: %s", hipGetErrorString(e));
        delete c;
        return BI_ERR_HIP;
    }
    *out = c;
    return BI_OK;
}

void bi_destroy(bi_ctx* c) {
    if (!c) return;
    (void)hipSetDevice(c->device);
    (void)hipStreamSynchronize(c->stream);
    dev_free(c->ps); dev_free(c->nm); dev_free(c->nm_tot); dev_free(c->counts); dev_free(c->lgsum); dev_free(c->cnt8); dev_free(c->cnt8_bad);
    dev_free(c->scratch); dev_free(c->scratch2); dev_free(c->logmu); dev_free(c->toy_blocks_done); dev_free(c->ev_perm);
    dev_free(c->slot_dev); dev_free(c->slot_partial); dev_free(c->slot_pflags); dev_free(c->slot_counter); dev_free(c->space_edges);
    dev_free(c->mail); dev_free(c->mail_flags);
    dev_free(c->ps_sorted); dev_free(c->cnt_sorted);
    dev_free(c->sim_coords); dev_free(c->sim_source);
    dev_free(c->real_counts);
    dev_free(c->fac.ps); dev_free(c->fac.counts);
    release_coarse(c);
    if (c->slot_host) (void)hipHostFree(c->slot_host);
    if (c->pack_host) (void)hipHostFree(c->pack_host);
    if (c->bounce_host) (void)hipHostFree(c->bounce_host);
    if (c->plan_host) (void)hipHostFree(c->plan_host);
    dev_free(c->pack_dev);
    dev_free(c->nz_idx); dev_free(c->nz_n); dev_free(c->nz_off); dev_free(c->ps_c); dev_free(c->cnt_c); dev_free(c->tm_entries); dev_free(c->tm_off); dev_free(c->tmm_entries); dev_free(c->tmm_off);
    dev_free(c->pt_grid); dev_free(c->pt_mus); dev_free(c->pt_coff); dev_free(c->pt_allow); dev_free(c->pt_c_off);
    dev_free(c->pt_cnt_off); dev_free(c->pt_c_np); dev_free(c->pt_Tz); dev_free(c->pt_rowsum); dev_free(c->pt_rowmin); dev_free(c->pt_nm_tot);
    for (void* q : c->user_allocs) (void)hipFree(q);
    c->user_allocs.clear();
    for (auto& q : c->cache) (void)hipFree(q.p);
    c->cache.clear();
    for (auto& ev : c->ev_pool) { (void)hipEventDestroy(ev.first); (void)hipEventDestroy(ev.second); }
    for (hipEvent_t ev : c->tp_ev)
        if (ev) (void)hipEventDestroy(ev);
    if (c->stream2) (void)hipStreamDestroy(c->stream2);
    (void)hipStreamDestroy(c->stream);
    delete c;
}

int bi_device_info(bi_ctx* c, char* name, char* arch, int len, int* n_cu, int64_t* hbm_bytes) {
    if (!c) return BI_ERR_INVALID;
    if (name && len > 0) { strncpy(name, c->prop.name, len - 1); name[len - 1] = 0; }
    if (arch && len > 0) { strncpy(arch, c->prop.gcnArchName, len - 1); arch[len - 1] = 0; }
    if (n_cu) *n_cu = c->prop.multiProcessorCount;
    if (hbm_bytes) *hbm_bytes = (int64_t)c->prop.totalGlobalMem;
    return BI_OK;
}

void* bi_stream(bi_ctx* c) { return c ? (void*)c->stream : nullptr; }

int bi_sync(bi_ctx* c) {
    if (!c) return BI_ERR_INVALID;
    HIP_TRY(c, hipStreamSynchronize(c->stream));
    return BI_OK;
}

int bi_set_param(bi_ctx* c, const char* name, int64_t v) {
    if (!c || !name) return BI_ERR_INVALID;
    const ParamDef* p = find_param(name);
    if (!p) return fail(c, BI_ERR_INVALID, "unknown parameter %s", name);
    if (!p->set) return fail(c, BI_ERR_INVALID, "parameter %s is read-only", name);
    return p->set(c, v);
}

int64_t bi_get_param(bi_ctx* c, const char* name) {
    if (!c || !name) return INT64_MIN;
    const ParamDef* p = find_param(name);
    if (!p || !p->get) {
        fail(c, BI_ERR_INVALID, p ? "parameter %s is write-only" : "unknown parameter %s", name);
        return INT64_MIN;
    }
    return p->get(c);
}

int bi_list_params(char* buf, int len) {
    std::string all;
    for (const ParamDef& p : kParams) {
        all += p.name;
        all += p.access == kParamRW ? " rw\n" : (p.access == kParamRead ? " r\n" : " w\n");
    }
    if (buf && len > 0) {
        const size_t n = std::min<size_t>(all.size(), (size_t)len - 1);
        memcpy(buf, all.data(), n);
        buf[n] = 0;
    }
    return (int)all.size() + 1;
}


int bi_model_begin(bi_ctx* c, int d, const int32_t* n_anchor, const double* anchor_z, int S, int64_t B,
                   int bb_source) {
    if (!c) return BI_ERR_INVALID;
    HIP_TRY(c, hipSetDevice(c->device));
    if (d < 0 || d > kMaxDim) return fail(c, BI_ERR_INVALID, "d=%d outside [0,%d]", d, kMaxDim);
    if (S < 1 || B < 0) return fail(c, BI_ERR_INVALID, "need S >= 1 and B >= 0 (got S=%d B=%lld)", S, (long long)B);
    if (bb_source < -1 || bb_source >= S) return fail(c, BI_ERR_INVALID, "bb_source %d outside [-1,%d)", bb_source, S);
    if (d > 0 && (!n_anchor || !anchor_z)) return fail(c, BI_ERR_INVALID, "anchor arrays are NULL");
    c->model_ready = false;
    c->data_ready = false;
    c->cnt8_valid = false;
    dev_free(c->real_counts);
    c->real_T = 0;
    release_coarse(c);
    ++c->epoch;
    c->d = d; c->S = S; c->B = B; c->bb_source = bb_source;
    c->Bp = std::max<int64_t>(kTile, (B + kTile - 1) / kTile * kTile);
    c->unbinned = false;
    c->ev_sorted = false;
    c->n_sets = 1;
    c->set_first.clear();
    c->set_n.clear();
    c->n_anchor.assign(d, 0);
    c->grid.assign(d, {});
    c->A = 1;
    const double* zp = anchor_z;
    for (int i = 0; i < d; ++i) {
        if (n_anchor[i] < 1) return fail(c, BI_ERR_INVALID, "axis %d has %d anchors", i, n_anchor[i]);
        c->n_anchor[i] = n_anchor[i];
        c->grid[i].assign(zp, zp + n_anchor[i]);
        for (int j = 1; j < n_anchor[i]; ++j)
            if (!(c->grid[i][j] > c->grid[i][j - 1]))
                return fail(c, BI_ERR_INVALID, "anchor z values of axis %d are not strictly ascending", i);
        zp += n_anchor[i];
        c->A *= n_anchor[i];
    }
    c->astride.assign(d, 1);
    for (int i = d - 2; i >= 0; --i) c->astride[i] = c->astride[i + 1] * c->n_anchor[i + 1];
    c->eff_axes.clear();
    for (int i = 0; i < d; ++i)
        if (c->n_anchor[i] >= 2) c->eff_axes.push_back(i);
    c->allow_neg.assign(S, 0);
    c->h_mus.assign((size_t)c->A * S, 0.0);
    c->h_nm_tot.assign((size_t)c->A, 0.0);
    c->anchor_set.assign((size_t)c->A, 0);
    const size_t ps_bytes = ((size_t)c->A * S * c->Bp + kTile) * sizeof(double);
    int rc = dev_alloc(c, c->ps, ps_bytes);
    if (rc) return rc;
    HIP_TRY(c, hipMemsetAsync(c->ps.p, 0, ps_bytes, c->stream));
    if (bb_source >= 0) {
        const size_t nm_bytes = (size_t)c->A * c->Bp * sizeof(double);
        if ((rc = dev_alloc(c, c->nm, nm_bytes))) return rc;
        HIP_TRY(c, hipMemsetAsync(c->nm.p, 0, nm_bytes, c->stream));
        if ((rc = dev_alloc(c, c->nm_tot, (size_t)c->A * sizeof(double)))) return rc;
    }
    c->model_open = true;
    return BI_OK;
}

int bi_model_set_anchor(bi_ctx* c, int64_t ai, const double* ps, const double* mus, const double* nm_row) {
    if (!c || !c->model_open) return fail(c, BI_ERR_STATE, "bi_model_begin first");
    if (ai < 0 || ai >= c->A) return fail(c, BI_ERR_INVALID, "anchor index %lld outside [0,%lld)", (long long)ai, (long long)c->A);
    if (!ps || !mus) return fail(c, BI_ERR_INVALID, "ps / mus are NULL");
    if (c->bb_source >= 0 && !nm_row) return fail(c, BI_ERR_INVALID, "Beeston-Barlow model needs the n_model row");
    HIP_TRY(c, hipSetDevice(c->device));
    double* dst = (double*)c->ps.p + (size_t)ai * c->S * c->Bp;
    if (c->B > 0) HIP_TRY(c, hipMemcpy2DAsync(dst, c->Bp * sizeof(double), ps, c->B * sizeof(double), c->B * sizeof(double), c->S,
                                hipMemcpyHostToDevice, c->stream));
    for (int s = 0; s < c->S; ++s) c->h_mus[(size_t)ai * c->S + s] = mus[s];
    if (c->bb_source >= 0 && c->B > 0) {
        double* nd = (double*)c->nm.p + (size_t)ai * c->Bp;
        HIP_TRY(c, hipMemcpyAsync(nd, nm_row, c->B * sizeof(double), hipMemcpyHostToDevice, c->stream));
    }
    HIP_TRY(c, hipStreamSynchronize(c->stream));
    c->anchor_set[(size_t)ai] = 1;
    return BI_OK;
}

int bi_model_end(bi_ctx* c) {
    if (!c || !c->model_open) return fail(c, BI_ERR_STATE, "bi_model_begin first");
    for (int64_t a = 0; a < c->A; ++a)
        if (!c->anchor_set[(size_t)a]) return fail(c, BI_ERR_STATE, "anchor %lld was never set", (long long)a);
    HIP_TRY(c, hipSetDevice(c->device));
    if (c->bb_source >= 0) {
        hipLaunchKernelGGL(k_row_total, dim3((unsigned)c->A), dim3(kThreads), 0, c->stream, (const double*)c->nm.p, c->B,
                           c->Bp, (double*)c->nm_tot.p);
        HIP_TRY(c, hipGetLastError());
        HIP_TRY(c, hipMemcpyAsync(c->h_nm_tot.data(), c->nm_tot.p, (size_t)c->A * sizeof(double), hipMemcpyDeviceToHost,
                                  c->stream));
    }
    {
        const int64_t rows = c->A * c->S;
        int rc = dev_alloc(c, c->scratch, (size_t)rows * 3 * sizeof(double));
        if (rc) return rc;
        hipLaunchKernelGGL(k_row_stats, dim3((unsigned)rows), dim3(kThreads), 0, c->stream, (const double*)c->ps.p, c->B,
                           c->Bp, (double*)c->scratch.p);
        HIP_TRY(c, hipGetLastError());
        std::vector<double> st((size_t)rows * 3);
        HIP_TRY(c, hipMemcpyAsync(st.data(), c->scratch.p, st.size() * sizeof(double), hipMemcpyDeviceToHost, c->stream));
        HIP_TRY(c, hipStreamSynchronize(c->stream));
        c->h_rowsum.assign((size_t)rows, 0.0);
        c->h_rowmin.assign((size_t)rows, 0.0);
        c->ps_nonneg = true;
        c->ps_finite = true;
        for (int64_t r = 0; r < rows; ++r) {
            c->h_rowsum[(size_t)r] = st[(size_t)r * 3];
            c->h_rowmin[(size_t)r] = st[(size_t)r * 3 + 1];
            if (!(st[(size_t)r * 3 + 1] >= 0.0) || st[(size_t)r * 3 + 2] != 0.0) c->ps_nonneg = false;
            if (st[(size_t)r * 3 + 2] != 0.0) c->ps_finite = false;
        }
    }
    HIP_TRY(c, hipStreamSynchronize(c->stream));
    c->model_open = false;
    c->model_ready = true;
    return BI_OK;
}

int bi_upload_model(bi_ctx* c, int d, const int32_t* n_anchor, const double* anchor_z, int S, int64_t B,
                    const double* ps, const double* mus, const double* n_model, int bb_source) {
    if (!c) return BI_ERR_INVALID;
    if (!ps || !mus) return fail(c, BI_ERR_INVALID, "ps / mus are NULL");
    if (bb_source >= 0 && !n_model) return fail(c, BI_ERR_INVALID, "bb_source given but n_model is NULL");
    int rc = bi_model_begin(c, d, n_anchor, anchor_z, S, B, bb_source);
    if (rc) return rc;
    if (B > 0) HIP_TRY(c, hipMemcpy2DAsync(c->ps.p, c->Bp * sizeof(double), ps, B * sizeof(double), B * sizeof(double),
                                (size_t)c->A * S, hipMemcpyHostToDevice, c->stream));
    std::copy(mus, mus + (size_t)c->A * S, c->h_mus.begin());
    if (bb_source >= 0) {
        if (B > 0) HIP_TRY(c, hipMemcpy2DAsync(c->nm.p, c->Bp * sizeof(double), n_model + (size_t)bb_source * B,
                                    (size_t)S * B * sizeof(double), B * sizeof(double), (size_t)c->A,
                                    hipMemcpyHostToDevice, c->stream));
    }
    HIP_TRY(c, hipStreamSynchronize(c->stream));
    std::fill(c->anchor_set.begin(), c->anchor_set.end(), 1);
    return bi_model_end(c);
}

int bi_set_allow_negative(bi_ctx* c, const int32_t* allow) {
    int rc = check_ready(c, false);
    if (rc) return rc;
    if (!allow) return fail(c, BI_ERR_INVALID, "allow is NULL");
    c->allow_neg.assign(allow, allow + c->S);
    return BI_OK;
}

int bi_set_bb_totals(bi_ctx* c, const double* totals) {
    int rc = check_ready(c, false);
    if (rc) return rc;
    if (c->bb_source < 0) return fail(c, BI_ERR_INVALID, "the model has no Beeston-Barlow source");
    if (!totals) return fail(c, BI_ERR_INVALID, "totals is NULL");
    c->h_nm_tot.assign(totals, totals + c->A);
    ++c->epoch;
    return BI_OK;
}

int bi_get_bb_totals(bi_ctx* c, double* totals) {
    int rc = check_ready(c, false);
    if (rc) return rc;
    if (c->bb_source < 0 || !totals) return fail(c, BI_ERR_INVALID, "no Beeston-Barlow source / totals is NULL");
    std::copy(c->h_nm_tot.begin(), c->h_nm_tot.end(), totals);
    return BI_OK;
}


int bi_upload_counts(bi_ctx* c, int64_t T, const double* counts) {
    int rc = check_ready(c, false);
    if (rc) return rc;
    if (T < 1 || !counts) return fail(c, BI_ERR_INVALID, "need T >= 1 datasets and a counts pointer");
    if (c->unbinned) return fail(c, BI_ERR_STATE, "the context holds an unbinned likelihood: it has no binned counts");
    if (c->B < 1) return fail(c, BI_ERR_INVALID, "a binned likelihood needs at least one bin");
    HIP_TRY(c, hipSetDevice(c->device));
    c->data_ready = false;
    ++c->epoch;
    const size_t bytes = (size_t)T * c->Bp * sizeof(double);
    if ((rc = dev_alloc(c, c->counts, bytes))) return rc;
    HIP_TRY(c, hipMemsetAsync(c->counts.p, 0, bytes, c->stream));
    HIP_TRY(c, hipMemcpy2DAsync(c->counts.p, c->Bp * sizeof(double), counts, c->B * sizeof(double),
                                c->B * sizeof(double), (size_t)T, hipMemcpyHostToDevice, c->stream));
    return finish_counts(c, T);
}



int bi_set_analysis_space(bi_ctx* c, int k, const int32_t* n_edges, const double* edges) {
    int rc = check_ready(c, false);
    if (rc) return rc;
    AxisWalk ax;
    if ((rc = walk_axes(c, k, n_edges, edges, 2, false, kSpaceWords, ax))) return rc;
    if (ax.bins != c->B) return fail(c, BI_ERR_INVALID, "analysis space has %lld bins, the model %lld", (long long)ax.bins, (long long)c->B);
    HIP_TRY(c, hipSetDevice(c->device));
    c->space_k = k;
    c->space_n_edges.assign(n_edges, n_edges + k);
    const std::vector<double> flat(edges, edges + ax.flat);
    if ((rc = dev_upload(c, c->space_edges, flat))) return rc;
    HIP_TRY(c, hipStreamSynchronize(c->stream));
// ... 102 lines not shown
    if (P < 0 || P > (int64_t)1 << 30) return fail(c, BI_ERR_INVALID, "P outside [0, 2^30]");
    if (share_world < 1 || share_rank < 0 || share_rank >= share_world)
        return fail(c, BI_ERR_INVALID, "share %d outside [0,%d)", share_rank, share_world);
    if (c->d > 0 && P > 0 && !z_dev) return fail(c, BI_ERR_INVALID, "z_dev is NULL");
    HIP_TRY(c, hipSetDevice(c->device));
    if (P == 0) return plan_points(c, 0, nullptr, nullptr, nullptr, out);
    const void* ptrs[3] = {c->d > 0 ? (const void*)z_dev : nullptr, rate_scale_dev, dataset_dev};
    const char* names[3] = {"z_dev", "rate_scale_dev", "dataset_dev"};
    for (int i = 0; i < 3 && check_pointers; ++i) {
        if (!ptrs[i]) continue;
        hipPointerAttribute_t at;
        const hipError_t e = hipPointerGetAttributes(&at, ptrs[i]);
        if (e != hipSuccess || (at.type != hipMemoryTypeDevice && at.type != hipMemoryTypeManaged) || at.device != c->device) {
            (void)hipGetLastError();
            return fail(c, BI_ERR_INVALID, "%s is not device memory of GPU %d", names[i], c->device);
        }
    }
    const bool sparse = ItemRoute(c).compact;
    if (!sparse && !c->dense_counts)
        return fail(c, BI_ERR_STATE, "the datasets exist only as non-empty-bin lists (device-generated toys): point "
                                     "evaluations need the compacted templates (sparse mode, budget) or bi_eval_datasets");
    c->plan_refused = 0;
    rc = plan_points_device(c, P, z_dev, rate_scale_dev, dataset_dev, sparse, out, share_rank, share_world, true, false);
    if (rc == kPlanNeedsHost && (c->plan_refused = 1))
        return fail(c, BI_ERR_INVALID, "resident points are planned on the device: this Beeston-Barlow batch has points at which some bin can "
                                       "have U_b == 0 (or bb_exact = 1) and needs the host planner's exact totals (bi_plan_points)");
    return rc;
}

}

extern "C" {

int bi_plan_points_resident(bi_ctx* c, int64_t P, const double* z_dev, const double* rate_scale_dev, const int64_t* dataset_dev,
                            int share_rank, int share_world, bi_plan** out) {
    if (c && multi_set(c)) return refuse_sets(c, "bi_plan_points_resident");
    return plan_points_resident_impl(c, P, z_dev, rate_scale_dev, dataset_dev, share_rank, share_world, out, true);
}

int bi_plan_share_info(const bi_plan* p, int64_t* n_valid, int64_t* lo, int64_t* hi) {
    if (!p || !p->shared) return BI_ERR_INVALID;
    if (n_valid) *n_valid = p->n_valid;
    if (lo) *lo = p->share_lo;
    if (hi) *hi = p->share_hi;
    return BI_OK;
}

int bi_plan_unsort(bi_ctx* c, bi_plan* plan, const double* gathered_dev, int64_t stride, double* full_dev) {
    if (!c || !plan) return BI_ERR_INVALID;
    if (!plan->shared) return fail(c, BI_ERR_INVALID, "bi_plan_unsort: not a share of a dealt scan (bi_plan_points_share)");
    const int64_t per_rank = (plan->n_valid + plan->share_world - 1) / plan->share_world;
    if (!gathered_dev || !full_dev || stride < per_rank) return fail(c, BI_ERR_INVALID, "bi_plan_unsort: NULL buffer or stride %lld < %lld", (long long)stride, (long long)per_rank);
    HIP_TRY(c, hipSetDevice(c->device));
    if (plan->P > 0)
        hipLaunchKernelGGL(k_unsort_share, dim3((unsigned)((plan->P + kThreads - 1) / kThreads)), dim3(kThreads), 0, c->stream, gathered_dev,
                           stride, plan->share_world, plan->n_valid, plan->P, (const int64_t*)plan->sorted_idx.p, full_dev);
    HIP_TRY(c, hipGetLastError());
    return BI_OK;
}

int bi_run_plan(bi_ctx* c, bi_plan* plan, double* out_dev) {
    int rc = check_ready(c, true);
    if (rc) return rc;
    if (!plan) return fail(c, BI_ERR_INVALID, "plan is NULL");
    if (plan->epoch != c->epoch) return fail(c, BI_ERR_STATE, "plan is stale: model or data were uploaded after it was made");
    HIP_TRY(c, hipSetDevice(c->device));
    double* out = out_dev ? out_dev : (double*)plan->out.p;
    const bool bb = c->bb_source >= 0;
    const int nc = 1 << (int)c->eff_axes.size();
    LaunchArgs a{};
    a.ps = plan->sparse ? (const double*)c->ps_c.p : (const double*)c->ps.p;
    a.nm = (const double*)c->nm.p;
    a.counts = plan->sparse ? (const double*)c->cnt_c.p : (const double*)c->counts.p;
    a.B = c->B; a.Bp = c->Bp;
    a.outlier = c->outlier;
    a.nan_S = (c->unbinned && !c->ps_finite) ? c->S : 0;
    a.n0 = bb ? nc * (c->S - 1) : nc * c->S;
    a.n1 = bb ? nc : 0; a.n2 = bb ? nc : 0;
    a.n_tiles = n_tiles_of(c);
    a.chunks = (int)c->tile_chunks;
    const int NS = a.n0 + a.n1 + a.n2;
    c->last_streamed_bytes = plan->bytes;
    const bool narrow = plan->narrow && !plan->sparse && narrow_on(c);
    if (plan->use_scan) {
        bi_plan::Class& k = plan->classes[0];
        ScanArgs sa{};
        sa.ps = a.ps; sa.counts = a.counts;
        if (plan->sorted) {
            if (c->sorted_epoch != c->epoch || !c->sorted_ok) return fail(c, BI_ERR_STATE, "plan is stale: the count-sorted rows are gone");
            sa.ps = (const double*)c->ps_sorted.p; sa.counts = (const double*)c->cnt_sorted.p;
            ++c->n_sorted_scans;
        }
        sa.rowoff = (const int64_t*)k.rowoff.p; sa.coef = (const double*)k.coef.p;
        sa.item_cnt = (const int64_t*)k.item_cnt.p; sa.item_tiles = (const int32_t*)k.item_tiles.p;
        sa.grp_first = (const int64_t*)plan->grp_first.p; sa.grp_items = (const int32_t*)plan->grp_items.p;
        sa.partial = (double*)k.partial.p; sa.NS = NS; sa.nslots = k.nbx;
        HIP_TRY(c, hipMemsetAsync(k.partial.p, 0, (size_t)k.n_items * k.nbx * k.G * sizeof(double), c->stream));
        {
            EventScope ev(c);
            ++c->n_scan_launches;
            const dim3 sgrid((unsigned)(k.nbx / 4), (unsigned)plan->n_groups);
            c->last_scan_groups = plan->n_groups; c->last_scan_max_items = plan->max_group_items;
            c->last_scan_cb = plan->by_count ? 4 : (plan->scan_cb == 2 ? 2 : 4);
            c->last_scan_by_count = plan->by_count ? 1 : 0;
            c->last_scan_prod = 0;
            if (plan->by_count) {
                sa.n_groups = (int)plan->n_groups;
                sa.xcd_mode = (int)c->scan_xcd;
                sa.share_slow = (int)c->scan_share_slow;
                const int64_t scan_blocks = (int64_t)(k.nbx / 4) * (c->scan_xcd == 2 ? (plan->n_groups + 7) / 8 * 8 : plan->n_groups);
                launch_scan_sorted(c, NS, dim3((unsigned)((scan_blocks + 7) / 8 * 8)), sa);
            } else
                launch_scan_mfma(c, plan->scan_cb == 2 ? 2 : 4, plan->sparse, NS, sgrid, sa);
        }
        hipLaunchKernelGGL(k_finish_scan, dim3((unsigned)((k.n_items + kThreads / 64 - 1) / (kThreads / 64))), dim3(kThreads), 0,
                           c->stream, (const double*)k.partial.p, k.nbx, k.n_items, (const int64_t*)k.perm.p,
                           (const double*)k.slot_lg.p, out);
    }
    if (plan->bb_kgt && !plan->classes.empty()) {
        bi_plan::Class& k = plan->classes[0];
        BbScanArgs ba{};
        ba.ps = a.ps; ba.nm = a.nm; ba.counts = a.counts;
        ba.rowoff = (const int64_t*)k.rowoff.p; ba.coef = (const double*)k.coef.p; ba.aux = (const double*)k.aux.p;
        ba.item_cnt = (const int64_t*)k.item_cnt.p;
        ba.grp_first = (const int64_t*)plan->grp_first.p; ba.grp_items = (const int32_t*)plan->grp_items.p;
        ba.partial = (double*)k.partial.p; ba.pflags = (unsigned*)k.pflags.p;
        ba.B = c->B; ba.n0 = a.n0; ba.nc = a.n1; ba.n_tiles = (int)((c->B + 15) / 16);
        const int64_t quads = std::max<int64_t>(1, (plan->max_group_items + 3) / 4);
        {
            EventScope ev(c);
            ++c->n_bb_scan_launches;
            launch_scan_bb(c, plan->bb_kgt, dim3((unsigned)k.nbx, (unsigned)plan->n_groups, (unsigned)quads), ba);
        }
        launch_finish(c, (const double*)k.partial.p, (const unsigned*)k.pflags.p, k.nbx, k.G, k.n_items * k.G, (const int64_t*)k.perm.p,
                      (const double*)k.slot_lg.p, out, (int32_t*)plan->status.p);
    }
    for (auto& k : plan->classes) {
        if (plan->use_scan || plan->bb_kgt) break;
        for (int64_t i0 = 0; i0 < k.n_items; i0 += 65535) {
            const int64_t ni = std::min<int64_t>(65535, k.n_items - i0);
            LaunchArgs b = a;
            b.rowoff = (const int64_t*)k.rowoff.p + i0 * NS;
            b.coef = (const double*)k.coef.p + i0 * NS * k.G;
            b.aux = (const double*)k.aux.p + i0 * k.G * 2;
            b.item_cnt = (const int64_t*)k.item_cnt.p + i0;
            b.item_tiles = (const int32_t*)k.item_tiles.p + i0;
            b.partial = (double*)k.partial.p + i0 * k.nbx * k.G;
            b.pflags = (unsigned*)k.pflags.p + i0 * k.nbx * k.G;
            const bool huge_items = (int64_t)sizeof(double) * (NS + 1) * c->Bp > ((int64_t)1 << 30);
            const bool nt = !plan->sparse && (c->nt_loads == 1 || (c->nt_loads == 2 && (plan->no_reuse || huge_items)));
            const bool fuse = c->fuse_finish && k.n_items <= 256 && k.n_items * k.nbx * k.G <= kMailSlots &&
                              k.n_items * k.G <= kMailFlagWords && !ensure_mail(c);
            if (fuse) {
                b.fin_mail = (double*)c->mail.p;
                b.fin_flags = (unsigned*)c->mail_flags.p;
                b.fin_perm = (const int64_t*)k.perm.p;
                b.fin_slot_lg = (const double*)k.slot_lg.p;
                b.fin_out = out;
                b.fin_status = (int32_t*)plan->status.p;
                arm_mail(c, b);
            }
            if (narrow) {
                b.cnt8 = (const uint8_t*)c->cnt8.p;
                c->last_streamed_bytes -= 7 * c->Bp * ni;
                ++c->n_narrow_launches;
            }
            launch_morph_g(c, k.G, b, dim3((unsigned)k.nbx, (unsigned)ni), bb, nt);
            c->last_morph_nbx = k.nbx; c->last_morph_items = ni; c->last_morph_fused = fuse ? 1 : 0;
            if (fuse) continue;
            launch_finish(c, b.partial, b.pflags, k.nbx, k.G, ni * k.G, (const int64_t*)k.perm.p + i0 * k.G,
                          (const double*)k.slot_lg.p + i0 * k.G, out, (int32_t*)plan->status.p);
        }
    }
    if (plan->valid) {
        bi_plan::Class& k = plan->classes[0];
        ValidArgs va{};
        va.ps = (const double*)c->ps.p;
        va.rowoff = (const int64_t*)k.rowoff_full.p; va.coef = (const double*)k.coef.p;
        va.grp_first = (const int64_t*)plan->grp_first.p; va.grp_items = (const int32_t*)plan->grp_items.p;
        va.bad = (unsigned*)plan->bad.p; va.NS = NS; va.nslots = plan->valid_nslots;
        va.n_strips = n_tiles_of(c) * (kTile / 64);
        HIP_TRY(c, hipMemsetAsync(plan->bad.p, 0, (size_t)k.n_items * k.G * sizeof(unsigned), c->stream));
        {
            EventScope ev(c);
            ++c->n_valid_launches;
            c->last_scan_groups = plan->n_groups; c->last_scan_max_items = plan->max_group_items;
            const dim3 vgrid((unsigned)(plan->valid_nslots / 4), (unsigned)plan->n_groups);
            launch_scan_valid(c, NS, vgrid, va);
        }
        const int64_t n_slots = k.n_items * k.G;
        hipLaunchKernelGGL(k_apply_bad, dim3((unsigned)((n_slots + kThreads - 1) / kThreads)), dim3(kThreads), 0, c->stream,
                           (const unsigned*)plan->bad.p, (const int64_t*)k.perm.p, n_slots, out);
    }
    if (plan->shared) {
    } else if (plan->n_bad > 0 && plan->device_planned)
        hipLaunchKernelGGL(k_fill_bad_by_status, dim3((unsigned)((plan->P + kThreads - 1) / kThreads)), dim3(kThreads), 0, c->stream,
                           (const int32_t*)plan->status.p, plan->P, out);
    else if (plan->n_bad > 0)
        hipLaunchKernelGGL(k_fill_const, dim3((unsigned)((plan->n_bad + 255) / 256)), dim3(256), 0, c->stream, out,
                           (const int64_t*)plan->bad_idx.p, plan->n_bad, -std::numeric_limits<double>::infinity());
    if (plan->n_nan > 0)
        hipLaunchKernelGGL(k_fill_const, dim3((unsigned)((plan->n_nan + 255) / 256)), dim3(256), 0, c->stream, out,
                           (const int64_t*)plan->nan_idx.p, plan->n_nan, std::numeric_limits<double>::quiet_NaN());
    HIP_TRY(c, hipGetLastError());
    return BI_OK;
}

static void internal_reported(bi_ctx* c, bi_plan* plan) {
    reset_mail(c);
    if (!plan->P) return;
    if (plan->host_results) {
        int32_t* st = (int32_t*)plan->status.p;
        for (int64_t p = 0; p < plan->P; ++p) st[p] &= ~BI_ST_INTERNAL;
    } else {
        hipLaunchKernelGGL(k_status_clear, dim3((unsigned)std::min<int64_t>(1024, (plan->P + kThreads - 1) / kThreads)), dim3(kThreads), 0,
                           c->stream, (int32_t*)plan->status.p, plan->P, (int32_t)BI_ST_INTERNAL);
        (void)hipStreamSynchronize(c->stream);
    }
}

int bi_plan_read(bi_ctx* c, bi_plan* plan, double* out, int32_t* status) {
    if (!c || !plan) return BI_ERR_INVALID;
    if (out && plan->shared) return fail(c, BI_ERR_INVALID, "bi_plan_read: a share's results are in sorted order: gather them and call bi_plan_unsort");
    HIP_TRY(c, hipSetDevice(c->device));
    if (out && plan->P)
        HIP_TRY(c, hipMemcpyAsync(out, plan->out.p, (size_t)plan->P * sizeof(double), hipMemcpyDeviceToHost, c->stream));
    if (status && plan->P)
        HIP_TRY(c, hipMemcpyAsync(status, plan->status.p, (size_t)plan->P * sizeof(int32_t), hipMemcpyDeviceToHost, c->stream));
    HIP_TRY(c, hipStreamSynchronize(c->stream));
    if (status) {
        for (int64_t p = 0; p < plan->P; ++p)
            if (status[p] & BI_ST_INTERNAL) { internal_reported(c, plan); break; }
        return BI_OK;
    }
    int32_t any = 0;
    return bi_plan_status(c, plan, &any);
}

int bi_plan_status(bi_ctx* c, bi_plan* plan, int32_t* status_or) {
    if (!c || !plan) return BI_ERR_INVALID;
    HIP_TRY(c, hipSetDevice(c->device));
    int32_t any = 0;
    if (plan->P) {
        if (plan->host_results) {
            HIP_TRY(c, hipStreamSynchronize(c->stream));
            const int32_t* st = (const int32_t*)plan->status.p;
            for (int64_t p = 0; p < plan->P; ++p) any |= st[p];
        } else {
            ScratchBuf d_or;
// ... 318 lines not shown
    c->dense_counts = false;
    c->csr_ready = c->compact_ready = false;
    ++c->epoch;
    dev_free(c->counts);
    c->cnt8_valid = false;
    std::vector<int32_t> meth;
    if ((rc = draw_toy_lists(c, truths, n_toys, T, seed, meth))) return rc;
    if (method_out) std::copy(meth.begin(), meth.end(), method_out);
    c->T = T;
    c->csr_ready = true;
    if ((rc = build_compact_templates(c))) return rc;
    c->data_ready = true;
    return BI_OK;
}

int bi_generate_toys(bi_ctx* c, const double* z, const double* rate_scale, int64_t T, uint64_t seed) {
    if (!c) return BI_ERR_INVALID;
    return generate_toys_impl(c, 1, z, rate_scale, &T, seed, nullptr, true);
}

int bi_generate_toys_points(bi_ctx* c, int64_t H, const double* z, const double* rate_scale, const int64_t* n_toys, uint64_t seed,
                            int32_t* method_out) {
    if (!c) return BI_ERR_INVALID;
    return generate_toys_impl(c, H, z, rate_scale, n_toys, seed, method_out, false);
}

int bi_download_counts(bi_ctx* c, int64_t t, double* out) {
    int rc = check_ready(c, true);
    if (rc) return rc;
    if (t < 0 || t >= c->T || !out) return fail(c, BI_ERR_INVALID, "dataset %lld outside [0,%lld) or out is NULL", (long long)t, (long long)c->T);
    HIP_TRY(c, hipSetDevice(c->device));
    if (c->dense_counts) {
        HIP_TRY(c, hipMemcpyAsync(out, (const double*)c->counts.p + t * c->Bp, (size_t)c->B * sizeof(double), hipMemcpyDeviceToHost, c->stream));
        HIP_TRY(c, hipStreamSynchronize(c->stream));
        return BI_OK;
    }
    if (!c->csr_ready) return fail(c, BI_ERR_STATE, "no counts resident");
    if ((rc = dev_alloc(c, c->logmu, (size_t)c->Bp * sizeof(double)))) return rc;
    const int64_t lo = c->h_nz_off[(size_t)t], nnz = c->h_nz_off[(size_t)t + 1] - lo;
    HIP_TRY(c, hipMemsetAsync(c->logmu.p, 0, (size_t)c->B * sizeof(double), c->stream));
    if (nnz > 0)
        hipLaunchKernelGGL(k_csr_to_dense, dim3((unsigned)((nnz + 255) / 256)), dim3(256), 0, c->stream,
                           (const int32_t*)c->nz_idx.p + lo, (const double*)c->nz_n.p + lo, nnz, (double*)c->logmu.p);
    HIP_TRY(c, hipGetLastError());
    HIP_TRY(c, hipMemcpyAsync(out, c->logmu.p, (size_t)c->B * sizeof(double), hipMemcpyDeviceToHost, c->stream));
    HIP_TRY(c, hipStreamSynchronize(c->stream));
    return BI_OK;
}


int bi_counts_to_dense(bi_ctx* c) {
    int rc = check_ready(c, true);
    if (rc) return rc;
    if (c->dense_counts) return BI_OK;
    if (!c->csr_ready) return fail(c, BI_ERR_STATE, "no counts resident");
    HIP_TRY(c, hipSetDevice(c->device));
    const size_t bytes = (size_t)c->T * c->Bp * sizeof(double);
    if ((rc = dev_alloc(c, c->counts, bytes))) return rc;
    HIP_TRY(c, hipMemsetAsync(c->counts.p, 0, bytes, c->stream));
    for (int64_t t = 0; t < c->T; ++t) {
        const int64_t lo = c->h_nz_off[(size_t)t], nnz = c->h_nz_off[(size_t)t + 1] - lo;
        if (nnz > 0)
            hipLaunchKernelGGL(k_csr_to_dense, dim3((unsigned)((nnz + 255) / 256)), dim3(256), 0, c->stream,
                               (const int32_t*)c->nz_idx.p + lo, (const double*)c->nz_n.p + lo, nnz, (double*)c->counts.p + t * c->Bp);
    }
    HIP_TRY(c, hipGetLastError());
    build_narrow_counts(c, c->T);
    HIP_TRY(c, hipStreamSynchronize(c->stream));
    c->dense_counts = true;
    ++c->epoch;
    return BI_OK;
}



int bi_set_unbinned(bi_ctx* c, double outlier_likelihood) {
    int rc = check_ready(c, false);
    if (rc) return rc;
    if (c->bb_source >= 0) return fail(c, BI_ERR_INVALID, "Beeston-Barlow applies to binned likelihoods only");
    HIP_TRY(c, hipSetDevice(c->device));
    ++c->epoch;
    c->unbinned = true;
    c->cnt8_valid = false;
    c->outlier = outlier_likelihood;
    c->csr_ready = c->compact_ready = false;
    if ((rc = dev_alloc(c, c->counts, (size_t)c->Bp * sizeof(double)))) return rc;
    HIP_TRY(c, hipMemsetAsync(c->counts.p, 0, (size_t)c->Bp * sizeof(double), c->stream));
    HIP_TRY(c, hipStreamSynchronize(c->stream));
    c->T = 1;
    c->h_lgsum.assign(1, 0.0);
    c->n_sets = 1;
    c->set_first.assign(1, 0);
    c->set_n.assign(1, c->B);
    c->dense_counts = true;
    c->data_ready = true;
    return BI_OK;
}

}


static int interpolate_set(bi_ctx* c, int which, const double* z, double* out, int64_t set) {
    int rc = check_ready(c, false);
    if (rc) return rc;
    if (!out) return fail(c, BI_ERR_INVALID, "out is NULL");
    if (c->d > 0 && !z) return fail(c, BI_ERR_INVALID, "z is NULL");
    if (which < 0 || which > 2) return fail(c, BI_ERR_INVALID, "which must be 0 (ps), 1 (mus) or 2 (n_model row)");
    if (which == 2 && c->bb_source < 0) return fail(c, BI_ERR_INVALID, "model has no n_model tensor");
    PointGeom g;
    if (!point_geometry(c, z, g))
        return fail(c, BI_ERR_INVALID, "One of the requested xi is out of bounds");
    if (which == 1) { interp_mus(c, g, out); return BI_OK; }
    HIP_TRY(c, hipSetDevice(c->device));
    const int nc = (int)g.w.size();
    const int R = which == 0 ? c->S : 1;
    const bool of_set = which == 0 && multi_set(c);
    const int64_t col0 = of_set ? c->set_first[(size_t)set] : 0, nB = of_set ? c->set_n[(size_t)set] : c->B;
    if (of_set && nB == 0) return BI_OK;
    std::vector<int64_t> rowoff((size_t)R * nc);
    for (int r = 0; r < R; ++r)
        for (int corner = 0; corner < nc; ++corner) {
            const int64_t a = g.cell_anchor + corner_offset(c, corner);
            rowoff[(size_t)r * nc + corner] = which == 0 ? (a * c->S + r) * c->Bp + col0 : a * c->Bp;
        }
    ScratchBuf d_row, d_w, d_out;
    if ((rc = dev_upload(c, d_row, rowoff)) || (rc = dev_upload(c, d_w, g.w)) ||
        (rc = dev_alloc(c, d_out, (size_t)R * nB * sizeof(double)))) return rc;
    hipLaunchKernelGGL(k_morph_store, dim3((unsigned)((nB + kThreads - 1) / kThreads), (unsigned)R), dim3(kThreads), 0,
                       c->stream, which == 0 ? (const double*)c->ps.p : (const double*)c->nm.p,
                       (const int64_t*)d_row.p, (const double*)d_w.p, nc, nB, (double*)d_out.p,
                       which == 0 && c->ev_sorted ? (const int32_t*)c->ev_perm.p : (const int32_t*)nullptr);
    hipError_t e = hipGetLastError();
    if (e == hipSuccess) e = hipMemcpyAsync(out, d_out.p, (size_t)R * nB * sizeof(double), hipMemcpyDeviceToHost, c->stream);
    if (e == hipSuccess) e = hipStreamSynchronize(c->stream);
    if (e != hipSuccess) return fail(c, BI_ERR_HIP, "bi_interpolate: %s", hipGetErrorString(e));
    return BI_OK;
}

extern "C" {

int bi_interpolate(bi_ctx* c, int which, const double* z, double* out) { return interpolate_set(c, which, z, out, 0); }

int bi_eval_full(bi_ctx* c, const double* z, const double* rate_scale, int64_t dataset, double* ll, double* mus_out,
                 double* ps_out, int32_t* status) {
    int rc = check_ready(c, true);
    if (rc) return rc;
    if (!ll || !mus_out || !ps_out) return fail(c, BI_ERR_INVALID, "output pointers are NULL");
    if (c->bb_source >= 0 && !c->dense_counts) return fail(c, BI_ERR_STATE, "dataset counts are not resident in dense form");
    int32_t st = 0;
    rc = bi_eval(c, 1, z, rate_scale, &dataset, ll, &st);
    if (rc) return rc;
    if (status) *status = st;
    if (st & (BI_ST_OUT_OF_BOUNDS | BI_ST_UNPHYSICAL | BI_ST_BAD_DATASET)) return BI_OK;
    PointGeom g;
    point_geometry(c, z, g);
    interp_mus(c, g, mus_out);
    if (rate_scale) for (int s = 0; s < c->S; ++s) mus_out[s] *= rate_scale[s];
    if ((rc = interpolate_set(c, 0, z, ps_out, dataset))) return rc;
    if (c->bb_source < 0) return BI_OK;
    HIP_TRY(c, hipSetDevice(c->device));
    const int i = c->bb_source;
    const int64_t B = c->B;
    double Ntot = 0.0;
    for (size_t corner = 0; corner < g.w.size(); ++corner) {
        const double term = c->h_nm_tot[(size_t)(g.cell_anchor + corner_offset(c, (int)corner))] * g.w[corner];
        Ntot = Ntot + term;
// ... 40 lines not shown
        drop_recycle_cache(c);
        e = hipMalloc(out, (size_t)std::max<int64_t>(bytes, 16));
    }
    if (e != hipSuccess) return fail(c, BI_ERR_NOMEM, "hipMalloc(%lld bytes) failed: %s", (long long)bytes, hipGetErrorString(e));
    c->user_allocs.push_back(*out);
    return BI_OK;
}

int bi_device_free(bi_ctx* c, void* p) {
    if (!c) return BI_ERR_INVALID;
    if (!p) return BI_OK;
    HIP_TRY(c, hipSetDevice(c->device));
    auto it = std::find(c->user_allocs.begin(), c->user_allocs.end(), p);
    if (it == c->user_allocs.end()) return fail(c, BI_ERR_INVALID, "bi_device_free: %p was not allocated by bi_device_alloc on this context", p);
    HIP_TRY(c, hipStreamSynchronize(c->stream));
    c->user_allocs.erase(it);
    HIP_TRY(c, hipFree(p));
    return BI_OK;
}

constexpr int64_t kBounceBytes = (int64_t)4 << 20;

static int bounce_of(bi_ctx* c) {
    if (!c->bounce_host) HIP_TRY(c, hipHostMalloc(&c->bounce_host, (size_t)kBounceBytes, hipHostMallocDefault));
    return BI_OK;
}

int bi_memcpy_to_host(bi_ctx* c, void* dst, const void* src, int64_t bytes) {
    if (!c || bytes < 0 || (bytes > 0 && (!dst || !src))) return BI_ERR_INVALID;
    HIP_TRY(c, hipSetDevice(c->device));
    if (bytes > 0 && bytes <= kBounceBytes) {
        int rc = bounce_of(c);
        if (rc) return rc;
        if (bytes % 4 == 0 && ((uintptr_t)src & 3) == 0) {
            const int64_t n_words = bytes / 4;
            hipLaunchKernelGGL(k_copy_words, dim3((unsigned)std::min<int64_t>(1024, (n_words + 255) / 256)), dim3(256), 0, c->stream,
                               (const uint32_t*)src, (uint32_t*)c->bounce_host, n_words);
            HIP_TRY(c, hipGetLastError());
        } else {
            HIP_TRY(c, hipMemcpyAsync(c->bounce_host, src, (size_t)bytes, hipMemcpyDeviceToHost, c->stream));
        }
        HIP_TRY(c, hipStreamSynchronize(c->stream));
        memcpy(dst, c->bounce_host, (size_t)bytes);
        return BI_OK;
    }
    if (bytes) HIP_TRY(c, hipMemcpyAsync(dst, src, (size_t)bytes, hipMemcpyDeviceToHost, c->stream));
    HIP_TRY(c, hipStreamSynchronize(c->stream));
    return BI_OK;
}

int bi_memcpy_to_device(bi_ctx* c, void* dst, const void* src, int64_t bytes) {
    if (!c || bytes < 0 || (bytes > 0 && (!dst || !src))) return BI_ERR_INVALID;
    HIP_TRY(c, hipSetDevice(c->device));
    if (bytes > 0 && bytes <= kBounceBytes) {
        int rc = bounce_of(c);
        if (rc) return rc;
        HIP_TRY(c, hipStreamSynchronize(c->stream));
        memcpy(c->bounce_host, src, (size_t)bytes);
        HIP_TRY(c, hipMemcpyAsync(dst, c->bounce_host, (size_t)bytes, hipMemcpyHostToDevice, c->stream));
        HIP_TRY(c, hipStreamSynchronize(c->stream));
        return BI_OK;
    }
    if (bytes) HIP_TRY(c, hipMemcpyAsync(dst, src, (size_t)bytes, hipMemcpyHostToDevice, c->stream));
    HIP_TRY(c, hipStreamSynchronize(c->stream));
    return BI_OK;
}


int bi_selftest_log(bi_ctx* c, int64_t n, const double* x, double* out) {
    if (!c || n < 0 || (n > 0 && (!x || !out))) return BI_ERR_INVALID;
    HIP_TRY(c, hipSetDevice(c->device));
    ScratchBuf dx, dy;
    int rc;
    if ((rc = dev_alloc(c, dx, (size_t)std::max<int64_t>(n, 1) * sizeof(double))) ||
        (rc = dev_alloc(c, dy, (size_t)std::max<int64_t>(n, 1) * sizeof(double)))) return rc;
    hipError_t e = n ? hipMemcpyAsync(dx.p, x, (size_t)n * sizeof(double), hipMemcpyHostToDevice, c->stream) : hipSuccess;
    if (e == hipSuccess && n) {
        hipLaunchKernelGGL(k_selftest_log, dim3((unsigned)((n + 255) / 256)), dim3(256), 0, c->stream, (const double*)dx.p, n, (double*)dy.p);
        e = hipGetLastError();
    }
    if (e == hipSuccess && n) e = hipMemcpyAsync(out, dy.p, (size_t)n * sizeof(double), hipMemcpyDeviceToHost, c->stream);
    if (e == hipSuccess) e = hipStreamSynchronize(c->stream);
    if (e != hipSuccess) return fail(c, BI_ERR_HIP, "bi_selftest_log: %s", hipGetErrorString(e));
    return BI_OK;
}

int bi_selftest_sort(bi_ctx* c, int kind, int64_t n, const void* keys, const void* vals, int begin_bit, int end_bit, void* keys_out, void* vals_out) {
    if (!c || n < 0 || kind < 0 || kind > 3 || begin_bit < 0 || end_bit > (kind == 3 ? 1024 : 64) || begin_bit > end_bit || (kind == 3 && end_bit < 1) ||
        (n > 0 && (!keys || !vals || !keys_out || !vals_out)))
        return BI_ERR_INVALID;
    HIP_TRY(c, hipSetDevice(c->device));
    const size_t vb = (kind == 0 || kind == 3) ? 8 : 4, nn = (size_t)std::max<int64_t>(n, 1);
    ScratchBuf dk, dv, dk2, dv2, dt;
    size_t tb = 0;
    if (kind == 0) (void)prim_sort_pairs(nullptr, tb, (const uint64_t*)nullptr, (uint64_t*)nullptr, (const int64_t*)nullptr, (int64_t*)nullptr, (size_t)n, 0u, 64u, c->stream);
    else if (kind == 3) (void)prim_count_sort_pairs(nullptr, tb, (const uint64_t*)nullptr, (uint64_t*)nullptr, (const int64_t*)nullptr, (int64_t*)nullptr, (size_t)n, (uint64_t)end_bit, c->stream);
    else if (kind == 1) (void)prim_sort_pairs(nullptr, tb, (const int64_t*)nullptr, (int64_t*)nullptr, (const int32_t*)nullptr, (int32_t*)nullptr, (size_t)n, 0u, 64u, c->stream);
    else (void)prim_sort_pairs(nullptr, tb, (const double*)nullptr, (double*)nullptr, (const int32_t*)nullptr, (int32_t*)nullptr, (size_t)n, 0u, 64u, c->stream);
    int rc;
    if ((rc = dev_alloc(c, dk, nn * 8)) || (rc = dev_alloc(c, dv, nn * vb)) || (rc = dev_alloc(c, dk2, nn * 8)) || (rc = dev_alloc(c, dv2, nn * vb)) ||
        (rc = dev_alloc(c, dt, std::max<size_t>(tb, 256)))) return rc;
    hipError_t e = n ? hipMemcpyAsync(dk.p, keys, (size_t)n * 8, hipMemcpyHostToDevice, c->stream) : hipSuccess;
    if (e == hipSuccess && n) e = hipMemcpyAsync(dv.p, vals, (size_t)n * vb, hipMemcpyHostToDevice, c->stream);
    size_t t2 = dt.bytes;
    if (e == hipSuccess) {
        if (kind == 0) e = prim_sort_pairs(dt.p, t2, (const uint64_t*)dk.p, (uint64_t*)dk2.p, (const int64_t*)dv.p, (int64_t*)dv2.p, (size_t)n, (unsigned)begin_bit, (unsigned)end_bit, c->stream);
        else if (kind == 3) e = prim_count_sort_pairs(dt.p, t2, (const uint64_t*)dk.p, (uint64_t*)dk2.p, (const int64_t*)dv.p, (int64_t*)dv2.p, (size_t)n, (uint64_t)end_bit, c->stream);
        else if (kind == 1) e = prim_sort_pairs(dt.p, t2, (const int64_t*)dk.p, (int64_t*)dk2.p, (const int32_t*)dv.p, (int32_t*)dv2.p, (size_t)n, (unsigned)begin_bit, (unsigned)end_bit, c->stream);
        else e = prim_sort_pairs(dt.p, t2, (const double*)dk.p, (double*)dk2.p, (const int32_t*)dv.p, (int32_t*)dv2.p, (size_t)n, (unsigned)begin_bit, (unsigned)end_bit, c->stream);
    }
    if (e == hipSuccess && n) e = hipMemcpyAsync(keys_out, dk2.p, (size_t)n * 8, hipMemcpyDeviceToHost, c->stream);
    if (e == hipSuccess && n) e = hipMemcpyAsync(vals_out, dv2.p, (size_t)n * vb, hipMemcpyDeviceToHost, c->stream);
    if (e == hipSuccess) e = hipStreamSynchronize(c->stream); else (void)hipStreamSynchronize(c->stream);
    if (e != hipSuccess) return fail(c, BI_ERR_HIP, "bi_selftest_sort: %s", hipGetErrorString(e));
    return BI_OK;
}

int bi_selftest_scan(bi_ctx* c, int kind, int64_t n, const void* in, int64_t init, void* out) {
    if (!c || n < 0 || kind < 0 || kind > 3 || (n > 0 && (!in || !out))) return BI_ERR_INVALID;
    HIP_TRY(c, hipSetDevice(c->device));
    const size_t nn = (size_t)std::max<int64_t>(n, 1);
    ScratchBuf di, dout, dt;
    size_t tb = 0;
    (void)prim_exclusive_scan_sum(nullptr, tb, (const int64_t*)nullptr, (int64_t*)nullptr, (int64_t)0, (size_t)n, c->stream);
    int rc;
    if ((rc = dev_alloc(c, di, nn * 8)) || (rc = dev_alloc(c, dout, nn * 8)) || (rc = dev_alloc(c, dt, std::max<size_t>(tb, 256)))) return rc;
    hipError_t e = n ? hipMemcpyAsync(di.p, in, (size_t)n * 8, hipMemcpyHostToDevice, c->stream) : hipSuccess;
    size_t t2 = dt.bytes;
    if (e == hipSuccess) {
        if (kind == 0) e = prim_inclusive_scan_max(dt.p, t2, (const int64_t*)di.p, (int64_t*)dout.p, (size_t)n, c->stream);
        else if (kind == 1) e = prim_inclusive_scan_sum(dt.p, t2, (const int64_t*)di.p, (int64_t*)dout.p, (size_t)n, c->stream);
        else if (kind == 2) e = prim_inclusive_scan_sum(dt.p, t2, (const double*)di.p, (double*)dout.p, (size_t)n, c->stream);
        else e = prim_exclusive_scan_sum(dt.p, t2, (const int64_t*)di.p, (int64_t*)dout.p, init, (size_t)n, c->stream);
    }
    if (e == hipSuccess && n) e = hipMemcpyAsync(out, dout.p, (size_t)n * 8, hipMemcpyDeviceToHost, c->stream);
    if (e == hipSuccess) e = hipStreamSynchronize(c->stream); else (void)hipStreamSynchronize(c->stream);
    if (e != hipSuccess) return fail(c, BI_ERR_HIP, "bi_selftest_scan: %s", hipGetErrorString(e));
    return BI_OK;
}


int bi_measure_read_bandwidth(bi_ctx* c, int nontemporal, int blocks_per_cu, int reps, double* gb_per_s) {
    if (!c || !gb_per_s || reps < 1 || blocks_per_cu < 1) return BI_ERR_INVALID;
    if (!c->model_ready || !c->ps.p) return fail(c, BI_ERR_STATE, "bi_measure_read_bandwidth: no model resident");
    HIP_TRY(c, hipSetDevice(c->device));
    ScratchBuf sink;
    int rc = dev_alloc(c, sink, 8);
    if (rc) return rc;
    const int64_t n2 = c->A * c->S * c->Bp / 2;
    const dim3 grid((unsigned)(c->prop.multiProcessorCount * blocks_per_cu));
    hipEvent_t e0 = nullptr, e1 = nullptr;
    hipError_t e = hipEventCreate(&e0);
    if (e == hipSuccess) e = hipEventCreate(&e1);
    double best = 0.0;
    for (int r = 0; e == hipSuccess && r <= reps; ++r) {
        e = hipEventRecord(e0, c->stream);
        if (nontemporal) hipLaunchKernelGGL(k_read_sum<true>, grid, dim3(kThreads), 0, c->stream, (const double*)c->ps.p, n2, (double*)sink.p);
        else hipLaunchKernelGGL(k_read_sum<false>, grid, dim3(kThreads), 0, c->stream, (const double*)c->ps.p, n2, (double*)sink.p);
        if (e == hipSuccess) e = hipEventRecord(e1, c->stream);
        if (e == hipSuccess) e = hipEventSynchronize(e1);
        float ms = 0.f;
        if (e == hipSuccess) e = hipEventElapsedTime(&ms, e0, e1);
        if (e == hipSuccess && r > 0 && ms > 0.f) best = std::max(best, (double)n2 * 16.0 / (ms * 1e6));
    }
    if (e0) (void)hipEventDestroy(e0);
    if (e1) (void)hipEventDestroy(e1);
// ... 113 lines not shown
```

blueice_amd/csrc/tu_morph.hip:

```cpp
#include "bi_common.h"
#include "bi_k_morph.h"
#include "bi_k_sets.h"

namespace {

template <int G>
void launch_morph(bi_ctx* c, const LaunchArgs& a, dim3 grid, bool bb, bool nt) {
    if (c->unbinned) {
        if (nt) hipLaunchKernelGGL((k_morph_reduce<G, false, true, 2>), grid, dim3(kThreads), 0, c->stream, a);
        else hipLaunchKernelGGL((k_morph_reduce<G, false, false, 2>), grid, dim3(kThreads), 0, c->stream, a);
        return;
    }
    if (a.cnt8) {
        if (bb && nt) hipLaunchKernelGGL((k_morph_reduce<G, true, true, 0, true>), grid, dim3(kThreads), 0, c->stream, a);
        else if (bb) hipLaunchKernelGGL((k_morph_reduce<G, true, false, 0, true>), grid, dim3(kThreads), 0, c->stream, a);
        else if (nt) hipLaunchKernelGGL((k_morph_reduce<G, false, true, 0, true>), grid, dim3(kThreads), 0, c->stream, a);
        else hipLaunchKernelGGL((k_morph_reduce<G, false, false, 0, true>), grid, dim3(kThreads), 0, c->stream, a);
        return;
    }
    if (bb && nt) hipLaunchKernelGGL((k_morph_reduce<G, true, true>), grid, dim3(kThreads), 0, c->stream, a);
    else if (bb) hipLaunchKernelGGL((k_morph_reduce<G, true, false>), grid, dim3(kThreads), 0, c->stream, a);
    else if (nt) hipLaunchKernelGGL((k_morph_reduce<G, false, true>), grid, dim3(kThreads), 0, c->stream, a);
    else hipLaunchKernelGGL((k_morph_reduce<G, false, false>), grid, dim3(kThreads), 0, c->stream, a);
}

}

void launch_morph_grad(bi_ctx* c, int G, const LaunchArgs& a, dim3 grid, bool nt) {
    EventScope ev(c);
#define BI_GRAD_CASE(GG)                                                                                          \
    case GG:                                                                                                      \
        if (c->unbinned) {                                                                                        \
            if (nt) hipLaunchKernelGGL((k_morph_reduce<GG, false, true, 3>), grid, dim3(kThreads), 0, c->stream, a); \
            else hipLaunchKernelGGL((k_morph_reduce<GG, false, false, 3>), grid, dim3(kThreads), 0, c->stream, a); \
        } else if (nt) hipLaunchKernelGGL((k_morph_reduce<GG, false, true, 1>), grid, dim3(kThreads), 0, c->stream, a); \
        else hipLaunchKernelGGL((k_morph_reduce<GG, false, false, 1>), grid, dim3(kThreads), 0, c->stream, a);   \
        break;
    switch (G) {
        BI_GRAD_CASE(2)
        BI_GRAD_CASE(4)
        BI_GRAD_CASE(8)
        default:
            BI_GRAD_CASE(16)
    }
#undef BI_GRAD_CASE
}

void launch_morph_g(bi_ctx* c, int G, const LaunchArgs& a, dim3 grid, bool bb, bool nt) {
    EventScope ev(c);
    switch (G) {
        case 1: launch_morph<1>(c, a, grid, bb, nt); break;
        case 2: launch_morph<2>(c, a, grid, bb, nt); break;
        case 4: launch_morph<4>(c, a, grid, bb, nt); break;
        case 8: launch_morph<8>(c, a, grid, bb, nt); break;
        default: launch_morph<16>(c, a, grid, bb, nt); break;
    }
}


void launch_morph_single(bi_ctx* c, bool bb, bool nt, bool fuse, dim3 grid, const LaunchArgs& a, const SingleDesc& d) {
    const dim3 block(kThreads);
#define BI_SINGLE(BBv, MODEv, C8v)                                                                                          \
    do {                                                                                                               \
        if (nt && fuse) hipLaunchKernelGGL((k_morph_single<BBv, true, MODEv, true, C8v>), grid, block, 0, c->stream, a, d);    \
        else if (nt) hipLaunchKernelGGL((k_morph_single<BBv, true, MODEv, false, C8v>), grid, block, 0, c->stream, a, d);      \
        else if (fuse) hipLaunchKernelGGL((k_morph_single<BBv, false, MODEv, true, C8v>), grid, block, 0, c->stream, a, d);    \
        else hipLaunchKernelGGL((k_morph_single<BBv, false, MODEv, false, C8v>), grid, block, 0, c->stream, a, d);             \
    } while (0)
    if (c->unbinned) BI_SINGLE(false, 2, false);
    else if (a.cnt8 && bb) BI_SINGLE(true, 0, true);
    else if (a.cnt8) BI_SINGLE(false, 0, true);
    else if (bb) BI_SINGLE(true, 0, false);
    else BI_SINGLE(false, 0, false);
#undef BI_SINGLE
}

void launch_morph_sets(bi_ctx* c, int G, const LaunchArgs& a, dim3 grid) {
    EventScope ev(c);
    switch (G) {
        case 1: hipLaunchKernelGGL((k_morph_sets<1, 2>), grid, dim3(kThreads), 0, c->stream, a); break;
        case 2: hipLaunchKernelGGL((k_morph_sets<2, 3>), grid, dim3(kThreads), 0, c->stream, a); break;
        case 4: hipLaunchKernelGGL((k_morph_sets<4, 3>), grid, dim3(kThreads), 0, c->stream, a); break;
        case 8: hipLaunchKernelGGL((k_morph_sets<8, 3>), grid, dim3(kThreads), 0, c->stream, a); break;
        default: hipLaunchKernelGGL((k_morph_sets<16, 3>), grid, dim3(kThreads), 0, c->stream, a); break;
    }
}
```

blueice_amd/device.py:

```python
import ctypes as C
import os

import numpy as np

from . import _capi
from ._capi import as_f64, ptr
from .exceptions import DeviceError, NotPreparedException, PlannerRefused

__all__ = ['DeviceContext', 'DeviceBuffer', 'EvalPlan', 'default_device']


def default_device():
    return int(os.environ.get('BLUEICE_AMD_DEVICE', os.environ.get('LOCAL_RANK', 0)))


class DeviceContext:

    def __init__(self, device=None):
        self._lib = _capi.load()
        self._h = C.c_void_p()
        device = default_device() if device is None else int(device)
        rc = self._lib.bi_create(device, C.byref(self._h))
        if rc != 0:
            raise DeviceError("bi_create(device=%d) failed: %s" % (
# ... 190 lines not shown
                                                    ptr(cols), float(outlier_likelihood)))
        self._made_unbinned(target, sets[0].shape[1], len(sets))

    def simulate_event_toys(self, target, method, edges, z, rate_scale=None, n_toys=1, seed=0, outlier_likelihood=1e-12):
        code, k, n_edges, flat = self._axes_args(method, edges)
        z = as_f64(z).reshape(self.d) if self.d else None
        if rate_scale is not None:
            rate_scale = as_f64(rate_scale, (self.S,))
        counts = np.zeros((int(n_toys), self.S), dtype=np.int64)
        target._check(self._lib.bi_simulate_event_toys(self._h, target._h, ptr(z), ptr(rate_scale), code, k, ptr(n_edges),
                                                       ptr(flat), int(n_toys), int(seed) & (2**64 - 1), float(outlier_likelihood),
                                                       ptr(counts)))
        self._made_unbinned(target, counts[0].sum(), n_toys)
        target._sim_dims = k
        return counts

    def adopt_event_sets(self, counts):
        counts = np.ascontiguousarray(counts, dtype=np.int64)
        self._check(self._lib.bi_set_event_sets(self._h, len(counts), ptr(counts)))
        self.T, self.B = len(counts), int(counts[0])

    def event_set_offsets(self):
        T = int(self._lib.bi_event_set_count(self._h))
        if T < 1:
            raise NotPreparedException("the context holds no unbinned data")
        out = np.zeros(T + 1, dtype=np.int64)
        self._check(self._lib.bi_event_set_offsets(self._h, ptr(out)))
        return out

    def event_set_counts(self):
        T = int(self._lib.bi_event_set_count(self._h))
        if T < 1:
            raise NotPreparedException("the context holds no unbinned data")
        out = np.zeros(T, dtype=np.int64)
        self._check(self._lib.bi_event_set_counts(self._h, ptr(out)))
        return out

    def download_event_set(self, t=0):
        n = int(self.event_set_counts()[t])
        A = int(np.prod([len(a) for a in self.anchor_z], dtype=np.int64)) if self.d else 1
        out = np.empty((A, self.S, n), dtype=np.float64)
        self._check(self._lib.bi_download_event_set(self._h, int(t), ptr(out)))
        return out

    def download_events(self):
        n = int(self._lib.bi_simulated_event_count(self._h))
        if n < 0:
            raise NotPreparedException("no simulated events are resident")
        coords = np.empty((self._sim_dims, n), dtype=np.float64)
        source = np.empty(n, dtype=np.int32)
        self._check(self._lib.bi_download_events(self._h, ptr(coords), ptr(source)))
        return coords, source

    def set_unbinned(self, outlier_likelihood=1e-12):
        self._check(self._lib.bi_set_unbinned(self._h, float(outlier_likelihood)))
        self.T = 1

    def counts_to_dense(self):
        self._check(self._lib.bi_counts_to_dense(self._h))

    def generate_toys(self, z, rate_scale=None, T=1, seed=0):
        z = as_f64(z).reshape(self.d) if self.d else None
        if rate_scale is not None:
            rate_scale = as_f64(rate_scale, (self.S,))
        self._check(self._lib.bi_generate_toys(self._h, ptr(z), ptr(rate_scale), int(T), int(seed) & (2**64 - 1)))
        self.T = int(T)

    def generate_toys_points(self, z, rate_scale=None, n_toys=1, seed=0):
        n_toys = np.ascontiguousarray(np.atleast_1d(n_toys), dtype=np.int64)
        H = len(n_toys)
        z = np.ascontiguousarray(as_f64(z).reshape(H, self.d)) if self.d else None
        if rate_scale is not None:
            rate_scale = np.ascontiguousarray(np.broadcast_to(as_f64(np.atleast_2d(rate_scale)), (H, self.S)))
        methods = np.empty(H, dtype=np.int32)
        self._check(self._lib.bi_generate_toys_points(self._h, H, ptr(z), ptr(rate_scale), ptr(n_toys), int(seed) & (2**64 - 1),
                                                      ptr(methods)))
        self.T = int(n_toys.sum())
        return methods

    def download_counts(self, t=0):
        out = np.empty(self.B, dtype=np.float64)
        self._check(self._lib.bi_download_counts(self._h, int(t), ptr(out)))
        return out

    def _point_args(self, z, rate_scale, dataset):
        if self.d:
            z = as_f64(z).reshape(-1, self.d)
            P = len(z)
        else:
            P = 1 if rate_scale is None else len(np.atleast_2d(rate_scale))
            z = None
        if rate_scale is not None:
            rate_scale = np.ascontiguousarray(np.broadcast_to(as_f64(np.atleast_2d(rate_scale)), (P, self.S)))
        if dataset is not None:
            dataset = np.ascontiguousarray(np.broadcast_to(np.asarray(dataset, dtype=np.int64), (P,)))
        return P, z, rate_scale, dataset

    def eval_one(self, z, rate_scale=None, dataset=0):
        if z is not None and (z.dtype != np.float64 or not z.flags.c_contiguous or z.size != self.d):
            z = as_f64(z).reshape(self.d)
        if rate_scale is not None and (rate_scale.dtype != np.float64 or not rate_scale.flags.c_contiguous
                                       or rate_scale.size != self.S):
            rate_scale = as_f64(rate_scale).reshape(self.S)
        ds = self._one_ds
        ds.value = dataset
        rc = self._lib.bi_eval(self._h, 1, z.ctypes.data if self.d else None,
                               rate_scale.ctypes.data if rate_scale is not None else None, C.addressof(ds),
                               C.addressof(self._one_out), C.addressof(self._one_st))
        if rc:
            self._check(rc)
        return self._one_out.value, self._one_st.value

    def eval(self, z, rate_scale=None, dataset=None):
        P, z, rate_scale, dataset = self._point_args(z, rate_scale, dataset)
        out = np.empty(P, dtype=np.float64)
        status = np.zeros(P, dtype=np.int32)
        self._check(self._lib.bi_eval(self._h, P, ptr(z), ptr(rate_scale), ptr(dataset), ptr(out), ptr(status)))
        return out, status

    def eval_begin(self, z, rate_scale=None, dataset=0):
        z = as_f64(z).reshape(self.d) if self.d else None
        if rate_scale is not None:
            rate_scale = as_f64(rate_scale, (self.S,))
        self._check(self._lib.bi_eval_begin(self._h, ptr(z), ptr(rate_scale), int(dataset)))

    def eval_end(self):
        out = C.c_double()
        status = C.c_int32()
        self._check(self._lib.bi_eval_end(self._h, C.byref(out), C.byref(status)))
        return out.value, status.value

    def eval_grad(self, z, rate_scale=None, dataset=None):
        P, z, rate_scale, dataset = self._point_args(z, rate_scale, dataset)
        ll = np.empty(P, dtype=np.float64)
        grad = np.empty((P, self.d + self.S), dtype=np.float64)
        status = np.zeros(P, dtype=np.int32)
        self._check(self._lib.bi_eval_grad(self._h, P, ptr(z), ptr(rate_scale), ptr(dataset), ptr(ll), ptr(grad),
                                           ptr(status)))
        return ll, grad[:, :self.d], grad[:, self.d:], status

    def eval_hess(self, z, rate_scale=None, dataset=None):
        P, z, rate_scale, dataset = self._point_args(z, rate_scale, dataset)
        F = self.d + self.S
        ll = np.empty(P, dtype=np.float64)
        grad = np.empty((P, F), dtype=np.float64)
        hess = np.empty((P, F, F), dtype=np.float64)
        status = np.zeros(P, dtype=np.int32)
        self._check(self._lib.bi_eval_hess(self._h, P, ptr(z), ptr(rate_scale), ptr(dataset), ptr(ll), ptr(grad), ptr(hess),
                                           ptr(status)))
        return ll, grad[:, :self.d], grad[:, self.d:], hess, status

    def eval_gof(self, z, rate_scale=None, dataset=None):
        P, z, rate_scale, dataset = self._point_args(z, rate_scale, dataset)
        half_deviance = np.empty(P, dtype=np.float64)
        pearson = np.empty(P, dtype=np.float64)
        status = np.zeros(P, dtype=np.int32)
        self._check(self._lib.bi_eval_gof(self._h, P, ptr(z), ptr(rate_scale), ptr(dataset), ptr(half_deviance), ptr(pearson),
                                          ptr(status)))
        return half_deviance, pearson, status

    def expected_counts(self, z, rate_scale=None, per_source=False):
        P, z, rate_scale, _ = self._point_args(z, rate_scale, None)
        out = np.empty((P, self.S, self.B) if per_source else (P, self.B), dtype=np.float64)
        self._check(self._lib.bi_expected_counts(self._h, P, ptr(z), ptr(rate_scale), 1 if per_source else 0, ptr(out)))
        return out

# ... 410 lines not shown
```

include/blueice_hip.h:

```cpp
#ifndef BLUEICE_HIP_H
#define BLUEICE_HIP_H

#include <stdint.h>

#ifdef __cplusplus
extern "C" {
#endif
#if defined(__GNUC__)
#pragma GCC visibility push(default)
#endif

typedef struct bi_ctx bi_ctx;

enum {
    BI_OK = 0,
    BI_ERR_INVALID = -1,
    BI_ERR_HIP = -2,
    BI_ERR_STATE = -3,
    BI_ERR_NOMEM = -4
};

enum {
    BI_ST_OUT_OF_BOUNDS = 1,
    BI_ST_UNPHYSICAL = 2,
// ... 108 lines not shown
                         const double* hi, const int32_t* n_kinks, const double* kinks, double gtol, int max_iter,
                         const double* prior_mean, const double* prior_sigma, const double* prior_const, double* x_out,
                         double* f_out, int32_t* flags_out, int64_t* counters);

int bi_fit_batched_real(bi_ctx* ctx, int64_t P, int F, const int32_t* var_kind, const int32_t* var_index, const double* z0,
                        const double* scale0, const double* unit, const int64_t* dataset, const double* x0, const double* lo,
                        const double* hi, const int32_t* n_kinks, const double* kinks, double gtol, int max_iter,
                        const double* prior_mean, const double* prior_sigma, const double* prior_const, double* x_out,
                        double* f_out, int32_t* flags_out, int64_t* counters);

int bi_factored_begin(bi_ctx* ctx, int d, const int32_t* n_anchor, const double* anchor_z, int S, int64_t B,
                      const int32_t* n_own, const int32_t* own_axes);
int bi_factored_set_anchor(bi_ctx* ctx, int s, int64_t local_index, const double* ps_row, double mu);
int bi_factored_end(bi_ctx* ctx);
int bi_factored_set_counts(bi_ctx* ctx, int64_t T, const double* counts);
int bi_eval_factored(bi_ctx* ctx, int64_t P, const double* z, const double* rate_scale, const int64_t* dataset, double* ll,
                     double* grad, int32_t* status);
int bi_fit_batched_factored(bi_ctx* ctx, int64_t P, int F, const int32_t* var_kind, const int32_t* var_index, const double* z0,
                            const double* scale0, const double* unit, const int64_t* dataset, const double* x0,
                            const double* lo, const double* hi, const int32_t* n_kinks, const double* kinks, double gtol,
                            int max_iter, const double* prior_mean, const double* prior_sigma, const double* prior_const,
                            double* x_out, double* f_out, int32_t* flags_out, int64_t* counters);

int bi_eval_sourcewise_hess(bi_ctx* ctx, int64_t P, const double* z, const double* rate_scale, const int64_t* dataset, double* ll,
                            double* grad, double* hess, int32_t* status);
int bi_eval_sourcewise_fisher(bi_ctx* ctx, int64_t P, const double* z, const double* rate_scale, double* info, double* total,
                              int64_t* unbounded, int32_t* status);

int bi_sample_stretch(bi_ctx* ctx, int64_t E, int W, int F, const int32_t* var_kind, const int32_t* var_index, const double* z0,
                      const double* scale0, const double* unit, const int64_t* dataset, const double* x0, const double* lo,
                      const double* hi, int64_t n_steps, double a, uint64_t seed, int64_t first_ensemble, double* chain, double* ll,
                      int64_t* n_accepted, int64_t* counters);
int bi_sample_stretch_gauss(bi_ctx* ctx, int64_t E, int W, int F, const int32_t* var_kind, const int32_t* var_index,
                            const double* z0, const double* scale0, const double* unit, const int64_t* dataset, const double* x0,
                            const double* lo, const double* hi, int64_t n_steps, double a, uint64_t seed, int64_t first_ensemble,
                            const double* prior_mean, const double* prior_sigma, const double* prior_const, double* chain,
                            double* ll, int64_t* n_accepted, int64_t* counters);

int bi_grid_reduce(bi_ctx* ctx, int64_t E, const int64_t* dataset , int F, int n_keep, const int32_t* var_kind,
                   const int32_t* var_index, const double* z0 , const double* scale0 ,
                   const double* unit , const int32_t* n_nodes , const double* nodes, const double* term,
                   const double* logw, int64_t chunk, double* log_marginal , double* profile ,
                   int64_t* argmax , int64_t* counters );

int bi_eval_datasets(bi_ctx* ctx, const double* z, const double* rate_scale, int64_t t0, int64_t t1,
                     double* out, int32_t* status );
int bi_eval_datasets_device(bi_ctx* ctx, const double* z, const double* rate_scale, int64_t t0, int64_t t1,
                            double* out_dev, int32_t* status );

int bi_eval_datasets_points(bi_ctx* ctx, int64_t P, const double* z, const double* rate_scale, int64_t t0, int64_t t1,
                            double* out, int32_t* status );
int bi_eval_datasets_points_device(bi_ctx* ctx, int64_t P, const double* z, const double* rate_scale, int64_t t0, int64_t t1,
                                   double* out_dev, int32_t* status );

int bi_interpolate(bi_ctx* ctx, int which, const double* z, double* out);
int bi_eval_full(bi_ctx* ctx, const double* z, const double* rate_scale, int64_t dataset, double* ll,
                 double* mus_out, double* ps_out, int32_t* status);

typedef struct bi_plan bi_plan;
int bi_plan_points(bi_ctx* ctx, int64_t P, const double* z, const double* rate_scale, const int64_t* dataset,
                   bi_plan** out);
int bi_run_plan(bi_ctx* ctx, bi_plan* plan, double* out_dev );
int bi_plan_points_share(bi_ctx* ctx, int64_t P, const double* z, const double* rate_scale, const int64_t* dataset,
                         int share_rank, int share_world, bi_plan** out);
int bi_plan_share_info(const bi_plan* plan, int64_t* n_valid, int64_t* lo, int64_t* hi);
int bi_plan_points_resident(bi_ctx* ctx, int64_t P, const double* z_dev, const double* rate_scale_dev,
                            const int64_t* dataset_dev, int share_rank, int share_world, bi_plan** out);
int bi_plan_unsort(bi_ctx* ctx, bi_plan* plan, const double* gathered_dev, int64_t stride, double* full_dev);
int bi_plan_read(bi_ctx* ctx, bi_plan* plan, double* out , int32_t* status );
int bi_plan_status(bi_ctx* ctx, bi_plan* plan, int32_t* status_or);
int64_t bi_plan_bytes(const bi_plan* plan);
int64_t bi_plan_launches(const bi_plan* plan);
void bi_plan_destroy(bi_ctx* ctx, bi_plan* plan);
int bi_sync(bi_ctx* ctx);
void* bi_stream(bi_ctx* ctx);

int bi_device_alloc(bi_ctx* ctx, int64_t bytes, void** out);
int bi_device_free(bi_ctx* ctx, void* p);
int bi_memcpy_to_host(bi_ctx* ctx, void* dst_host, const void* src_dev, int64_t bytes);
int bi_memcpy_to_device(bi_ctx* ctx, void* dst_dev, const void* src_host, int64_t bytes);

int bi_selftest_log(bi_ctx* ctx, int64_t n, const double* x, double* out);

int bi_selftest_sort(bi_ctx* ctx, int kind, int64_t n, const void* keys, const void* vals, int begin_bit, int end_bit, void* keys_out,
                     void* vals_out);
int bi_selftest_scan(bi_ctx* ctx, int kind, int64_t n, const void* in, int64_t init, void* out);
int bi_selftest_grid_reduce(bi_ctx* ctx, int64_t cells, int64_t R, int64_t chunk, const double* t, const double* q,
                            double* log_marginal, double* profile, int64_t* argmax);

int bi_measure_read_bandwidth(bi_ctx* ctx, int nontemporal, int blocks_per_cu, int reps, double* gb_per_s);
int bi_measure_copy_bandwidth(bi_ctx* ctx, int64_t bytes, int reps, double* gb_per_s);
int bi_measure_stream_bandwidth(bi_ctx* ctx, int items, int rows, int nontemporal, int blocks_per_cu, int reps, double* gb_per_s);
int bi_profile_enable(bi_ctx* ctx, int on);
int bi_profile_read(bi_ctx* ctx, int64_t* n_launches, double* total_ms);
int bi_set_param(bi_ctx* ctx, const char* name, int64_t value);
int64_t bi_get_param(bi_ctx* ctx, const char* name);
int bi_list_params(char* buf, int len);

#if defined(__GNUC__)
#pragma GCC visibility pop
#endif
#ifdef __cplusplus
}
#endif
#endif
```

Baseline: 26790 evals/s.

## Stream anchor rows from a lossless 7-byte packed shadow with shared per-tile exponent

At model upload, a packing kernel builds a shadow copy of the anchor-row tensor. Each f64 is stored as 56 bits (low 32 bits, 16 mid bits, and 4 mantissa bits plus a 4-bit exponent offset from a per-512-bin tile base exponent). The packing is rejected if any tile is lossy. The dense morph kernels then decode rows from this shadow using buffer loads and byte permutes, which cuts HBM bytes per row by about an eighth, and raise waves-per-EU to hide the extra decode latency. In exchange the extra buffer costs memory, and the decode ALU work could limit throughput if the kernel is not purely bandwidth bound.

```diff
diff --git a/blueice_amd/_capi.py b/blueice_amd/_capi.py
--- a/blueice_amd/_capi.py
+++ b/blueice_amd/_capi.py
@@ -110,6 +110,7 @@
     'bi_memcpy_to_host': (C.c_int, [_p, _p, _p, _i64]),
     'bi_memcpy_to_device': (C.c_int, [_p, _p, _p, _i64]),
     'bi_selftest_log': (C.c_int, [_p, _i64, _p, _p]),
+    'bi_unpack_rows': (C.c_int, [_p, _p]),
     'bi_selftest_sort': (C.c_int, [_p, C.c_int, _i64, _p, _p, C.c_int, C.c_int, _p, _p]),
     'bi_selftest_scan': (C.c_int, [_p, C.c_int, _i64, _p, _i64, _p]),
     'bi_selftest_grid_reduce': (C.c_int, [_p, _i64, _i64, _i64, _p, _p, _p, _p, _p]),
diff --git a/blueice_amd/csrc/bi_context.h b/blueice_amd/csrc/bi_context.h
--- a/blueice_amd/csrc/bi_context.h
+++ b/blueice_amd/csrc/bi_context.h
@@ -108,6 +108,12 @@
     int64_t narrow_counts = 1;
     int64_t last_streamed_bytes = 0;
     int64_t n_narrow_launches = 0;
+    DevBuf pk, pk_base, pk_bad;
+    bool pk_valid = false;
+    bool pk_skip = false;
+    int64_t packed_rows = 1;
+    int64_t n_packed_launches = 0;
+    int64_t last_packed_saved = 0;
     int64_t last_morph_nbx = 0, last_morph_items = 0, last_morph_fused = 0;
 
     DevBuf real_counts;
diff --git a/blueice_amd/csrc/bi_dev_common.h b/blueice_amd/csrc/bi_dev_common.h
--- a/blueice_amd/csrc/bi_dev_common.h
+++ b/blueice_amd/csrc/bi_dev_common.h
@@ -30,7 +30,14 @@
     long long mail_timeout = 2000 * kMailTicksPerMs;
     int skip_post = -1, late_post = -1;
     const uint8_t* cnt8 = nullptr;
-};
+    const uint8_t* pk = nullptr;
+    const uint32_t* pk_base = nullptr;
+};
+
+constexpr int kPkChunk = 3584;
+constexpr int kPkMidOff = 2048;
+constexpr int kPkTopOff = 3072;
+constexpr int kPkSpan = 15;
 
 constexpr int kMaxSingleStreams = 128;
 
@@ -425,6 +432,41 @@
     }
 }
 
+struct PkRaw {
+    unsigned lo0, lo1;
+    unsigned mid;
+    unsigned top;
+};
+
+template <bool NT>
+__device__ __forceinline__ PkRaw pk_load(const uint8_t* __restrict__ pk, int64_t chunk) {
+    const __amdgpu_buffer_rsrc_t rsrc = __builtin_amdgcn_make_buffer_rsrc(const_cast<uint8_t*>(pk + chunk * kPkChunk), 0, kPkChunk, 0x00020000);
+    constexpr int aux = NT ? 2 : 0;
+    const auto lo = __builtin_amdgcn_raw_buffer_load_b64(rsrc, (int)threadIdx.x * 8, 0, aux);
+    PkRaw r;
+    r.lo0 = lo[0];
+    r.lo1 = lo[1];
+    r.mid = __builtin_amdgcn_raw_buffer_load_b32(rsrc, (int)threadIdx.x * 4, kPkMidOff, aux);
+    r.top = __builtin_amdgcn_raw_buffer_load_b16(rsrc, (int)threadIdx.x * 2, kPkTopOff, aux);
+    return r;
+}
+
+__device__ __forceinline__ unsigned pk_base_word(const uint32_t* __restrict__ pk_base, int64_t chunk) { return pk_base[chunk >> 1]; }
+__device__ __forceinline__ unsigned pk_exp_add(unsigned word, int64_t chunk) {
+    return (((word >> (((unsigned)chunk & 1u) * 16u)) & 0xffffu) - 1u) << 20;
+}
+
+__device__ __forceinline__ double2 pk_decode(const PkRaw& r, unsigned add) {
+    unsigned hx = __builtin_amdgcn_perm(r.top, r.mid, 0x0c040100u);
+    unsigned hy = __builtin_amdgcn_perm(r.top, r.mid, 0x0c050302u);
+    hx = hx ? hx + add : 0u;
+    hy = hy ? hy + add : 0u;
+    double2 v;
+    v.x = __longlong_as_double(((unsigned long long)hx << 32) | r.lo0);
+    v.y = __longlong_as_double(((unsigned long long)hy << 32) | r.lo1);
+    return v;
+}
+
 __device__ __forceinline__ double poisson_term(double n, double mu) {
     double t;
     if (n > 0.0) {
diff --git a/blueice_amd/csrc/bi_events.h b/blueice_amd/csrc/bi_events.h
--- a/blueice_amd/csrc/bi_events.h
+++ b/blueice_amd/csrc/bi_events.h
@@ -141,7 +141,10 @@
     }
     c->h_mus = tp->h_mus;
     std::fill(c->anchor_set.begin(), c->anchor_set.end(), 1);
-    if ((rc = bi_model_end(c))) return rc;
+    c->pk_skip = true;
+    rc = bi_model_end(c);
+    c->pk_skip = false;
+    if (rc) return rc;
     c->allow_neg = tp->allow_neg;
     return bi_set_unbinned(c, outlier_likelihood);
 }
diff --git a/blueice_amd/csrc/bi_k_misc.h b/blueice_amd/csrc/bi_k_misc.h
--- a/blueice_amd/csrc/bi_k_misc.h
+++ b/blueice_amd/csrc/bi_k_misc.h
@@ -189,6 +189,57 @@
     if (__ballot(lossy) != 0ull && (threadIdx.x & 63) == 0) atomicOr(bad + t, 1u);
 }
 
+__global__ __launch_bounds__(kThreads) void k_pack_rows(const double* __restrict__ ps, int64_t chunk0, uint8_t* __restrict__ pk,
+                                                        uint16_t* __restrict__ pk_base, unsigned* __restrict__ bad) {
+    const int64_t q = chunk0 + blockIdx.x;
+    const double2 v = *reinterpret_cast<const double2*>(ps + q * kTile + threadIdx.x * kBinsPerThread);
+    const unsigned long long u[2] = {(unsigned long long)__double_as_longlong(v.x), (unsigned long long)__double_as_longlong(v.y)};
+    unsigned emin = 0xFFFFu, emax = 0u;
+    bool lossy = false;
+#pragma unroll
+    for (int j = 0; j < 2; ++j) {
+        if (u[j] == 0ull) continue;
+        const unsigned e = (unsigned)(u[j] >> 52);
+        lossy |= e < 1u || e > 2046u;
+        emin = min(emin, e);
+        emax = max(emax, e);
+    }
+#pragma unroll
+    for (int off = 32; off > 0; off >>= 1) {
+        emin = min(emin, (unsigned)__shfl_xor((int)emin, off, 64));
+        emax = max(emax, (unsigned)__shfl_xor((int)emax, off, 64));
+    }
+    __shared__ unsigned s_min[kThreads / 64], s_max[kThreads / 64];
+    if ((threadIdx.x & 63) == 0) { s_min[threadIdx.x >> 6] = emin; s_max[threadIdx.x >> 6] = emax; }
+    __syncthreads();
+#pragma unroll
+    for (int w = 0; w < kThreads / 64; ++w) { emin = min(emin, s_min[w]); emax = max(emax, s_max[w]); }
+    const unsigned base = emax == 0u ? 0u : emin;
+    lossy |= emax > emin && emax - emin > (unsigned)(kPkSpan - 1);
+    unsigned long long lo = 0ull;
+    unsigned mid = 0u, top = 0u;
+#pragma unroll
+    for (int j = 0; j < 2; ++j) {
+        if (u[j] == 0ull) continue;
+        const unsigned code = ((unsigned)(u[j] >> 52) - base + 1u) & 15u;
+        lo |= (u[j] & 0xFFFFFFFFull) << (32 * j);
+        mid |= (unsigned)((u[j] >> 32) & 0xFFFFull) << (16 * j);
+        top |= ((unsigned)((u[j] >> 48) & 0xFull) | (code << 4)) << (8 * j);
+    }
+    uint8_t* __restrict__ p = pk + q * kPkChunk;
+    reinterpret_cast<unsigned long long*>(p)[threadIdx.x] = lo;
+    reinterpret_cast<unsigned*>(p + kPkMidOff)[threadIdx.x] = mid;
+    reinterpret_cast<uint16_t*>(p + kPkTopOff)[threadIdx.x] = (uint16_t)top;
+    if (threadIdx.x == 0) pk_base[q] = (uint16_t)base;
+    if (__ballot(lossy) != 0ull && (threadIdx.x & 63) == 0) atomicOr(bad, 1u);
+}
+
+__global__ __launch_bounds__(kThreads) void k_unpack_rows(const uint8_t* __restrict__ pk, const uint32_t* __restrict__ pk_base,
+                                                          int64_t chunk0, double* __restrict__ out) {
+    const int64_t q = chunk0 + blockIdx.x;
+    *reinterpret_cast<double2*>(out + q * kTile + threadIdx.x * kBinsPerThread) = pk_decode(pk_load<false>(pk, q), pk_exp_add(pk_base_word(pk_base, q), q));
+}
+
 __global__ void k_rows_sum(const double* __restrict__ partial, int nblk, double* __restrict__ out, int64_t T) {
     const int64_t t = (int64_t)blockIdx.x * blockDim.x + threadIdx.x;
     if (t >= T) return;
diff --git a/blueice_amd/csrc/bi_k_morph.h b/blueice_amd/csrc/bi_k_morph.h
--- a/blueice_amd/csrc/bi_k_morph.h
+++ b/blueice_amd/csrc/bi_k_morph.h
@@ -7,7 +7,44 @@
 namespace {
 
 
-template <int G, bool BB, bool NT, int MODE, bool CNT8 = false>
+
+template <int G, bool NT>
+__device__ __forceinline__ void packed_rows_fma(const LaunchArgs& a, const int64_t* __restrict__ rowoff, const double* __restrict__ coef,
+                                                int tile, int k_lo, int k_hi, double (&acc)[G][2]) {
+    static_assert(kTile == 512, "a chunk of the packed shadow is one 512-bin tile");
+    int k = k_lo;
+    for (; k + 8 <= k_hi; k += 8) {
+        PkRaw raw[8];
+        unsigned word[8];
+#pragma unroll
+        for (int u = 0; u < 8; ++u) word[u] = pk_base_word(a.pk_base, (rowoff[k + u] >> 9) + tile);
+#pragma unroll
+        for (int u = 0; u < 8; ++u) raw[u] = pk_load<NT>(a.pk, (rowoff[k + u] >> 9) + tile);
+        __builtin_amdgcn_sched_barrier(0);
+#pragma unroll
+        for (int u = 0; u < 8; ++u) {
+            const double2 v = pk_decode(raw[u], pk_exp_add(word[u], (rowoff[k + u] >> 9) + tile));
+#pragma unroll
+            for (int g = 0; g < G; ++g) {
+                const double c = coef[(k + u) * G + g];
+                acc[g][0] = fma(c, v.x, acc[g][0]);
+                acc[g][1] = fma(c, v.y, acc[g][1]);
+            }
+        }
+    }
+    for (; k < k_hi; ++k) {
+        const int64_t chunk = (rowoff[k] >> 9) + tile;
+        const double2 v = pk_decode(pk_load<NT>(a.pk, chunk), pk_exp_add(pk_base_word(a.pk_base, chunk), chunk));
+#pragma unroll
+        for (int g = 0; g < G; ++g) {
+            const double c = coef[k * G + g];
+            acc[g][0] = fma(c, v.x, acc[g][0]);
+            acc[g][1] = fma(c, v.y, acc[g][1]);
+        }
+    }
+}
+
+template <int G, bool BB, bool NT, int MODE, bool CNT8 = false, bool PACKED = false>
 __device__ __forceinline__ void morph_tiles(const LaunchArgs& a, const int64_t* __restrict__ rowoff,
                                             const double* __restrict__ coef, const double* __restrict__ aux_base,
                                             const double* __restrict__ cnt, const uint8_t* __restrict__ cnt8, int n_tiles, int tile0,
@@ -39,12 +76,16 @@
         int k0 = 0;
         if constexpr (NT && G == 1 && MODE != 2 && MODE != 3) {
             k0 = a.n_keep;
+            if constexpr (PACKED) {
+                packed_rows_fma<G, false>(a, rowoff, coef, tile, 0, k0, acc);
+            } else {
 #pragma unroll 8
-            for (int k = 0; k < k0; ++k) {
-                const double2 v = stream_load<false>(a.ps + rowoff[k] + bin0);
-                const double c = coef[k];
-                acc[0][0] = fma(c, v.x, acc[0][0]);
-                acc[0][1] = fma(c, v.y, acc[0][1]);
+                for (int k = 0; k < k0; ++k) {
+                    const double2 v = stream_load<false>(a.ps + rowoff[k] + bin0);
+                    const double c = coef[k];
+                    acc[0][0] = fma(c, v.x, acc[0][0]);
+                    acc[0][1] = fma(c, v.y, acc[0][1]);
+                }
             }
         }
         if constexpr (MODE == 2 || MODE == 3) if (a.nan_S > 0) {
@@ -80,14 +121,18 @@
             }
             k0 = a.n0;
         }
+        if constexpr (PACKED) {
+            packed_rows_fma<G, NT>(a, rowoff, coef, tile, k0, a.n0, acc);
+        } else {
 #pragma unroll 8
-        for (int k = k0; k < a.n0; ++k) {
-            const double2 v = stream_load<NT>(a.ps + rowoff[k] + bin0);
-#pragma unroll
-            for (int g = 0; g < G; ++g) {
-                const double c = coef[k * G + g];
-                acc[g][0] = fma(c, v.x, acc[g][0]);
-                acc[g][1] = fma(c, v.y, acc[g][1]);
+            for (int k = k0; k < a.n0; ++k) {
+                const double2 v = stream_load<NT>(a.ps + rowoff[k] + bin0);
+#pragma unroll
+                for (int g = 0; g < G; ++g) {
+                    const double c = coef[k * G + g];
+                    acc[g][0] = fma(c, v.x, acc[g][0]);
+                    acc[g][1] = fma(c, v.y, acc[g][1]);
+                }
             }
         }
         if (tab_pending) {
@@ -204,8 +249,12 @@
 
 }
 
-template <int G, bool BB, bool NT, int MODE = 0, bool CNT8 = false>
-__global__ __launch_bounds__(kThreads) void k_morph_reduce(LaunchArgs a) {
+constexpr int packed_min_waves(int G) { return G == 1 ? 7 : G == 2 ? 6 : G == 4 ? 5 : G == 8 ? 4 : 2; }
+
+template <int G, bool BB, bool NT, int MODE = 0, bool CNT8 = false, bool PACKED = false>
+__global__ __launch_bounds__(kThreads) __attribute__((amdgpu_waves_per_eu(PACKED ? packed_min_waves(G) : 1)))
+void k_morph_reduce(LaunchArgs a) {
+    static_assert(!PACKED || (MODE == 0 && !BB), "the packed rows serve the dense value kernels only");
     const int item = blockIdx.y;
     const int NS = a.n0 + a.n1 + a.n2;
     const int64_t* __restrict__ rowoff = a.rowoff + (int64_t)item * NS;
@@ -220,7 +269,7 @@
 #pragma unroll
     for (int g = 0; g < G; ++g) { sum[g] = 0.0; flg[g] = 0u; }
 
-    morph_tiles<G, BB, NT, MODE, CNT8>(a, rowoff, coef, a.aux + (int64_t)item * G * 2, cnt, cnt8, n_tiles, (int)blockIdx.x, (int)gridDim.x, sum, flg);
+    morph_tiles<G, BB, NT, MODE, CNT8, PACKED>(a, rowoff, coef, a.aux + (int64_t)item * G * 2, cnt, cnt8, n_tiles, (int)blockIdx.x, (int)gridDim.x, sum, flg);
 
     __shared__ double s_sum[kThreads / 64][G];
     __shared__ unsigned s_flg[kThreads / 64][G];
@@ -305,11 +354,13 @@
     }
 }
 
-template <bool BB, bool NT, int MODE, bool FUSE, bool CNT8 = false>
-__global__ __launch_bounds__(kThreads) void k_morph_single(LaunchArgs a, SingleDesc d) {
+template <bool BB, bool NT, int MODE, bool FUSE, bool CNT8 = false, bool PACKED = false>
+__global__ __launch_bounds__(kThreads) __attribute__((amdgpu_waves_per_eu(PACKED ? packed_min_waves(1) : 1)))
+void k_morph_single(LaunchArgs a, SingleDesc d) {
+    static_assert(!PACKED || (MODE == 0 && !BB), "the packed rows serve the dense value kernels only");
     double sum[1] = {0.0};
     unsigned flg[1] = {0u};
-    morph_tiles<1, BB, NT, MODE, CNT8>(a, d.rowoff, d.coef, d.aux, a.counts, a.cnt8, a.n_tiles, (int)blockIdx.x, (int)gridDim.x, sum, flg);
+    morph_tiles<1, BB, NT, MODE, CNT8, PACKED>(a, d.rowoff, d.coef, d.aux, a.counts, a.cnt8, a.n_tiles, (int)blockIdx.x, (int)gridDim.x, sum, flg);
 
     __shared__ double s_sum[kThreads / 64];
     __shared__ unsigned s_flg[kThreads / 64];
diff --git a/blueice_amd/csrc/bi_launch.h b/blueice_amd/csrc/bi_launch.h
--- a/blueice_amd/csrc/bi_launch.h
+++ b/blueice_amd/csrc/bi_launch.h
@@ -83,6 +83,51 @@
     return c->cnt8_all == 1;
 }
 
+void drop_packed_rows(bi_ctx* c, bool release) {
+    c->pk_valid = false;
+    if (release) { dev_free(c->pk); dev_free(c->pk_base); }
+}
+
+void build_packed_rows(bi_ctx* c) {
+    c->pk_valid = false;
+    if (!c->packed_rows || c->pk_skip || c->unbinned || c->bb_source >= 0 || !c->ps.p || c->B < 1) { drop_packed_rows(c, true); return; }
+    const int64_t n_chunks = c->A * c->S * (c->Bp / kTile);
+    const size_t pk_bytes = (size_t)n_chunks * kPkChunk;
+    const size_t base_bytes = ((size_t)n_chunks + 2) / 2 * sizeof(uint32_t);
+    size_t free_b = 0, total_b = 0;
+    if (hipMemGetInfo(&free_b, &total_b) != hipSuccess) { (void)hipGetLastError(); drop_packed_rows(c, true); return; }
+    if (!(c->pk.p && c->pk.bytes >= pk_bytes) && pk_bytes > free_b / 4) { drop_packed_rows(c, true); return; }
+    const std::string keep = c->err;
+    if (dev_alloc(c, c->pk, pk_bytes) || dev_alloc(c, c->pk_base, base_bytes) || dev_alloc(c, c->pk_bad, sizeof(unsigned))) {
+        (void)hipGetLastError();
+        c->err = keep;
+        drop_packed_rows(c, true);
+        return;
+    }
+    unsigned bad = 1u;
+    hipError_t e = hipMemsetAsync(c->pk_bad.p, 0, sizeof(unsigned), c->stream);
+    if (e == hipSuccess) e = hipMemsetAsync(c->pk_base.p, 0, base_bytes, c->stream);
+    const int64_t per_launch = (int64_t)1 << 30;
+    for (int64_t q0 = 0; q0 < n_chunks && e == hipSuccess; q0 += per_launch) {
+        hipLaunchKernelGGL(k_pack_rows, dim3((unsigned)std::min(per_launch, n_chunks - q0)), dim3(kThreads), 0, c->stream,
+                           (const double*)c->ps.p, q0, (uint8_t*)c->pk.p, (uint16_t*)c->pk_base.p, (unsigned*)c->pk_bad.p);
+        e = hipGetLastError();
+    }
+    if (e == hipSuccess) e = hipMemcpyAsync(&bad, c->pk_bad.p, sizeof(unsigned), hipMemcpyDeviceToHost, c->stream);
+    if (e == hipSuccess) e = hipStreamSynchronize(c->stream);
+    if (e != hipSuccess) { (void)hipGetLastError(); drop_packed_rows(c, true); return; }
+    if (bad != 0u) { drop_packed_rows(c, true); return; }
+    c->pk_valid = true;
+}
+
+bool packed_on(const bi_ctx* c) { return c->packed_rows && c->pk_valid && !c->unbinned && c->bb_source < 0 && c->pk.p; }
+
+void use_packed_rows(bi_ctx* c, LaunchArgs& a) {
+    a.pk = (const uint8_t*)c->pk.p;
+    a.pk_base = (const uint32_t*)c->pk_base.p;
+    ++c->n_packed_launches;
+}
+
 void launch_finish(bi_ctx* c, const double* partial, const unsigned* pflags, int nbx, int G, int64_t n_slots, const int64_t* perm,
                    const double* slot_lg, double* out, int32_t* status) {
     const int lanes = nbx > 64 ? kThreads : 64;
diff --git a/blueice_amd/csrc/bi_params.h b/blueice_amd/csrc/bi_params.h
--- a/blueice_amd/csrc/bi_params.h
+++ b/blueice_amd/csrc/bi_params.h
@@ -86,6 +86,7 @@
     {"compact_budget", kParamRW, BI_P_GET(c->compact_budget), BI_P_SET(c->compact_budget = v)},
     {"toy_offset", kParamRW, BI_P_GET(c->toy_offset), BI_P_RANGE(0, INT64_MAX, toy_offset, "toy_offset >= 0")},
     {"narrow_counts", kParamRW, BI_P_GET(c->narrow_counts), BI_P_FLAG(narrow_counts)},
+    {"packed_rows", kParamRW, BI_P_GET(c->packed_rows), BI_P_FLAG(packed_rows)},
     {"mail_timeout_ms", kParamRW, BI_P_GET(c->mail_timeout_ms),
      BI_P_RANGE(1, 60000, mail_timeout_ms, "mail_timeout_ms in [1, 60000]")},
     {"single_timing_reset", kParamWrite, nullptr,
@@ -112,6 +113,9 @@
     BI_P_RO("n_mail_resets", c->n_mail_resets),
     BI_P_RO("last_streamed_bytes", c->last_streamed_bytes),
     BI_P_RO("n_narrow_launches", c->n_narrow_launches),
+    BI_P_RO("n_packed_launches", c->n_packed_launches),
+    BI_P_RO("packed_rows_valid", c->pk_valid ? 1 : 0),
+    BI_P_RO("last_packed_saved_bytes", c->last_packed_saved),
     BI_P_RO("last_morph_nbx", c->last_morph_nbx),
     BI_P_RO("last_morph_items", c->last_morph_items),
     BI_P_RO("last_morph_fused", c->last_morph_fused),
diff --git a/blueice_amd/csrc/bi_single.h b/blueice_amd/csrc/bi_single.h
--- a/blueice_amd/csrc/bi_single.h
+++ b/blueice_amd/csrc/bi_single.h
@@ -246,6 +246,7 @@
         a.cnt8 = (const uint8_t*)c->cnt8.p + ds * c->Bp;
         ++c->n_narrow_launches;
     }
+    if (!sparse && !bb && packed_on(c)) use_packed_rows(c, a);
     const bool nt = !sparse && c->nt_loads != 0;
     a.n_keep = 0;
     if (nt && !bb && c->keep_rows != 0) {
@@ -400,6 +401,7 @@
         a.cnt8 = (const uint8_t*)c->cnt8.p;
         ++c->n_narrow_launches;
     }
+    if (!sparse && !bb && packed_on(c)) use_packed_rows(c, a);
     launch_morph_g(c, 1, a, dim3((unsigned)nbx, 1), bb, !sparse && c->nt_loads != 0);
     c->last_morph_nbx = nbx; c->last_morph_items = 1; c->last_morph_fused = 0;
     launch_finish(c, a.partial, a.pflags, nbx, 1, 1, (const int64_t*)(dev + (o + 2) * 8), (const double*)(dev + (o + 3) * 8),
diff --git a/blueice_amd/csrc/blueice_hip.hip b/blueice_amd/csrc/blueice_hip.hip
--- a/blueice_amd/csrc/blueice_hip.hip
+++ b/blueice_amd/csrc/blueice_hip.hip
@@ -76,6 +76,7 @@
     (void)hipSetDevice(c->device);
     (void)hipStreamSynchronize(c->stream);
     dev_free(c->ps); dev_free(c->nm); dev_free(c->nm_tot); dev_free(c->counts); dev_free(c->lgsum); dev_free(c->cnt8); dev_free(c->cnt8_bad);
+    dev_free(c->pk); dev_free(c->pk_base); dev_free(c->pk_bad);
     dev_free(c->scratch); dev_free(c->scratch2); dev_free(c->logmu); dev_free(c->toy_blocks_done); dev_free(c->ev_perm);
     dev_free(c->slot_dev); dev_free(c->slot_partial); dev_free(c->slot_pflags); dev_free(c->slot_counter); dev_free(c->space_edges);
     dev_free(c->mail); dev_free(c->mail_flags);
@@ -165,6 +166,7 @@
     c->model_ready = false;
     c->data_ready = false;
     c->cnt8_valid = false;
+    c->pk_valid = false;
     dev_free(c->real_counts);
     c->real_T = 0;
     release_coarse(c);
@@ -266,6 +268,7 @@
         }
     }
     HIP_TRY(c, hipStreamSynchronize(c->stream));
+    build_packed_rows(c);
     c->model_open = false;
     c->model_ready = true;
     return BI_OK;
@@ -534,6 +537,8 @@
     const int NS = a.n0 + a.n1 + a.n2;
     c->last_streamed_bytes = plan->bytes;
     const bool narrow = plan->narrow && !plan->sparse && narrow_on(c);
+    const bool packed = !plan->sparse && !bb && packed_on(c);
+    c->last_packed_saved = 0;
     if (plan->use_scan) {
         bi_plan::Class& k = plan->classes[0];
         ScanArgs sa{};
@@ -617,6 +622,10 @@
                 c->last_streamed_bytes -= 7 * c->Bp * ni;
                 ++c->n_narrow_launches;
             }
+            if (packed) {
+                use_packed_rows(c, b);
+                c->last_packed_saved += c->Bp * (int64_t)a.n0 * ni;
+            }
             launch_morph_g(c, k.G, b, dim3((unsigned)k.nbx, (unsigned)ni), bb, nt);
             c->last_morph_nbx = k.nbx; c->last_morph_items = ni; c->last_morph_fused = fuse ? 1 : 0;
             if (fuse) continue;
@@ -1101,6 +1110,7 @@
     ++c->epoch;
     c->unbinned = true;
     c->cnt8_valid = false;
+    drop_packed_rows(c, true);
     c->outlier = outlier_likelihood;
     c->csr_ready = c->compact_ready = false;
     if ((rc = dev_alloc(c, c->counts, (size_t)c->Bp * sizeof(double)))) return rc;
@@ -1307,6 +1317,21 @@
     if (e == hipSuccess && n) e = hipMemcpyAsync(out, dy.p, (size_t)n * sizeof(double), hipMemcpyDeviceToHost, c->stream);
     if (e == hipSuccess) e = hipStreamSynchronize(c->stream);
     if (e != hipSuccess) return fail(c, BI_ERR_HIP, "bi_selftest_log: %s", hipGetErrorString(e));
+    return BI_OK;
+}
+
+int bi_unpack_rows(bi_ctx* c, double* out_dev) {
+    int rc = check_ready(c, false);
+    if (rc) return rc;
+    if (!out_dev) return fail(c, BI_ERR_INVALID, "bi_unpack_rows: out_dev is NULL");
+    if (!c->pk_valid || !c->pk.p) return fail(c, BI_ERR_STATE, "bi_unpack_rows: the model has no packed rows (packed_rows_valid = 0)");
+    HIP_TRY(c, hipSetDevice(c->device));
+    const int64_t n_chunks = c->A * c->S * (c->Bp / kTile), per_launch = (int64_t)1 << 30;
+    for (int64_t q0 = 0; q0 < n_chunks; q0 += per_launch)
+        hipLaunchKernelGGL(k_unpack_rows, dim3((unsigned)std::min(per_launch, n_chunks - q0)), dim3(kThreads), 0, c->stream,
+                           (const uint8_t*)c->pk.p, (const uint32_t*)c->pk_base.p, q0, out_dev);
+    HIP_TRY(c, hipGetLastError());
+    HIP_TRY(c, hipStreamSynchronize(c->stream));
     return BI_OK;
 }
 
diff --git a/blueice_amd/csrc/tu_morph.hip b/blueice_amd/csrc/tu_morph.hip
--- a/blueice_amd/csrc/tu_morph.hip
+++ b/blueice_amd/csrc/tu_morph.hip
@@ -9,6 +9,13 @@
     if (c->unbinned) {
         if (nt) hipLaunchKernelGGL((k_morph_reduce<G, false, true, 2>), grid, dim3(kThreads), 0, c->stream, a);
         else hipLaunchKernelGGL((k_morph_reduce<G, false, false, 2>), grid, dim3(kThreads), 0, c->stream, a);
+        return;
+    }
+    if (a.pk && !bb) {
+        if (a.cnt8 && nt) hipLaunchKernelGGL((k_morph_reduce<G, false, true, 0, true, true>), grid, dim3(kThreads), 0, c->stream, a);
+        else if (a.cnt8) hipLaunchKernelGGL((k_morph_reduce<G, false, false, 0, true, true>), grid, dim3(kThreads), 0, c->stream, a);
+        else if (nt) hipLaunchKernelGGL((k_morph_reduce<G, false, true, 0, false, true>), grid, dim3(kThreads), 0, c->stream, a);
+        else hipLaunchKernelGGL((k_morph_reduce<G, false, false, 0, false, true>), grid, dim3(kThreads), 0, c->stream, a);
         return;
     }
     if (a.cnt8) {
@@ -60,18 +67,20 @@
 
 void launch_morph_single(bi_ctx* c, bool bb, bool nt, bool fuse, dim3 grid, const LaunchArgs& a, const SingleDesc& d) {
     const dim3 block(kThreads);
-#define BI_SINGLE(BBv, MODEv, C8v)                                                                                          \
+#define BI_SINGLE(BBv, MODEv, C8v, PKv)                                                                                        \
     do {                                                                                                               \
-        if (nt && fuse) hipLaunchKernelGGL((k_morph_single<BBv, true, MODEv, true, C8v>), grid, block, 0, c->stream, a, d);    \
-        else if (nt) hipLaunchKernelGGL((k_morph_single<BBv, true, MODEv, false, C8v>), grid, block, 0, c->stream, a, d);      \
-        else if (fuse) hipLaunchKernelGGL((k_morph_single<BBv, false, MODEv, true, C8v>), grid, block, 0, c->stream, a, d);    \
-        else hipLaunchKernelGGL((k_morph_single<BBv, false, MODEv, false, C8v>), grid, block, 0, c->stream, a, d);             \
+        if (nt && fuse) hipLaunchKernelGGL((k_morph_single<BBv, true, MODEv, true, C8v, PKv>), grid, block, 0, c->stream, a, d);    \
+        else if (nt) hipLaunchKernelGGL((k_morph_single<BBv, true, MODEv, false, C8v, PKv>), grid, block, 0, c->stream, a, d);      \
+        else if (fuse) hipLaunchKernelGGL((k_morph_single<BBv, false, MODEv, true, C8v, PKv>), grid, block, 0, c->stream, a, d);    \
+        else hipLaunchKernelGGL((k_morph_single<BBv, false, MODEv, false, C8v, PKv>), grid, block, 0, c->stream, a, d);             \
     } while (0)
-    if (c->unbinned) BI_SINGLE(false, 2, false);
-    else if (a.cnt8 && bb) BI_SINGLE(true, 0, true);
-    else if (a.cnt8) BI_SINGLE(false, 0, true);
-    else if (bb) BI_SINGLE(true, 0, false);
-    else BI_SINGLE(false, 0, false);
+    if (c->unbinned) BI_SINGLE(false, 2, false, false);
+    else if (a.pk && !bb && a.cnt8) BI_SINGLE(false, 0, true, true);
+    else if (a.pk && !bb) BI_SINGLE(false, 0, false, true);
+    else if (a.cnt8 && bb) BI_SINGLE(true, 0, true, false);
+    else if (a.cnt8) BI_SINGLE(false, 0, true, false);
+    else if (bb) BI_SINGLE(true, 0, false, false);
+    else BI_SINGLE(false, 0, false, false);
 #undef BI_SINGLE
 }
 
diff --git a/blueice_amd/device.py b/blueice_amd/device.py
--- a/blueice_amd/device.py
+++ b/blueice_amd/device.py
@@ -296,6 +296,16 @@
         out = np.empty(self.B, dtype=np.float64)
         self._check(self._lib.bi_download_counts(self._h, int(t), ptr(out)))
         return out
+
+    def unpack_rows(self):
+        rows = (int(np.prod([len(g) for g in self.anchor_z], dtype=np.int64)) if self.anchor_z else 1) * self.S
+        Bp = self.get_param('padded_bins')
+        buf = self.device_alloc(rows * Bp * 8)
+        try:
+            self._check(self._lib.bi_unpack_rows(self._h, C.c_void_p(buf.ptr)))
+            return buf.to_host(np.float64).reshape(rows, Bp)
+        finally:
+            buf.free()
 
     def _point_args(self, z, rate_scale, dataset):
         if self.d:
diff --git a/include/blueice_hip.h b/include/blueice_hip.h
--- a/include/blueice_hip.h
+++ b/include/blueice_hip.h
@@ -214,6 +214,8 @@
 
 int bi_selftest_log(bi_ctx* ctx, int64_t n, const double* x, double* out);
 
+int bi_unpack_rows(bi_ctx* ctx, double* out_dev);
+
 int bi_selftest_sort(bi_ctx* ctx, int kind, int64_t n, const void* keys, const void* vals, int begin_bit, int end_bit, void* keys_out,
                      void* vals_out);
 int bi_selftest_scan(bi_ctx* ctx, int kind, int64_t n, const void* in, int64_t init, void* out);
```

Result: faster. 30420 evals/s, median of 6 (+13.5%).
